# skhu101/TDNN-F_NAS

Measured on AMD Instinct MI355X. Metric: LF-MMI training frames/sec per node (SWBD 7q TDNN-F), higher is better.
Workload: dtype f32

## Files before the change

include/tdnnf_hip.h:

```cpp
#ifndef TDNNF_HIP_H_
#define TDNNF_HIP_H_

#include <stddef.h>
#include <stdint.h>

#ifdef __cplusplus
extern "C" {
#endif

#define TDNNF_OK 0
#define TDNNF_EINVAL 1
#define TDNNF_EHIP 2

#define TDNNF_MAX_OFFSETS 16

typedef struct {
  float *data;
  int rows, cols, stride;
} tdnnf_mat;

typedef void *tdnnf_stream;
typedef struct tdnnf_ng tdnnf_ng;

const char *tdnnf_last_error(void);
// ... 2 lines not shown
int tdnnf_get_option(const char *name, int *value_out);
int tdnnf_gemm_launch_forms(long long *counts, int capacity, int reset);
const char *tdnnf_gemm_launch_form_name(int index);

#define TDNNF_DARTS_USE_GUMBEL 1
#define TDNNF_DARTS_FREE_SELECT 2
#define TDNNF_DARTS_UNIFORM_SAMPLE 4
#define TDNNF_DARTS_USE_ENTROPY 8
#define TDNNF_DARTS_UPDATE_ALPHA 16

typedef struct {
  int row_stride;
  int num_offsets;
  int row_offsets[TDNNF_MAX_OFFSETS];
} tdnnf_tdnn_indexes;


int tdnnf_tdnn_darts_coef(const float *log_alpha_dev, int K, int flags, float temp_proportion,
                          const float *gumbel_u_dev, const float *sample_u_dev, int share_index,
                          float *coef_memo_dev, float *eff_coef_dev, tdnnf_stream stream);

int tdnnf_tdnn_propagate(const tdnnf_tdnn_indexes *indexes, const tdnnf_mat *in,
                         const float *linear_params_dev, int ldw, int Do, int Di,
                         const float *bias_dev, const float *eff_coef_dev, int init_mode,
                         tdnnf_mat *out, tdnnf_stream stream);

int tdnnf_tdnn_backprop_data(const tdnnf_tdnn_indexes *indexes, const tdnnf_mat *out_deriv,
                             const float *linear_params_dev, int ldw, int Do, int Di,
                             const float *eff_coef_dev, tdnnf_mat *in_deriv, tdnnf_stream stream);

size_t tdnnf_tdnn_update_workspace_bytes(int Do, int Di, int K, int num_rows);
int tdnnf_tdnn_update_simple(const tdnnf_tdnn_indexes *indexes, const tdnnf_mat *in_value,
                             const tdnnf_mat *out_deriv, int Do, int Di,
                             const float *eff_coef_dev, float lr, float *W_acc_dev, int ldw,
                             float *bias_acc_dev, void *workspace_dev, size_t workspace_bytes,
                             tdnnf_stream stream);

#define TDNNF_TAP_DOTS_SLABS 64
#define TDNNF_TAP_DOTS_DOUBLES(K) ((K) * (1 + TDNNF_TAP_DOTS_SLABS))

int tdnnf_tdnn_darts_alpha_update(const float *tap_grad_dev, int ldg, const float *linear_params_dev,
                                  int ldw, int Do, int Di, int K, const float *coef_memo_dev,
                                  int flags, int share_index, float temp_proportion, float lr,
                                  float *alpha_acc_dev, double *tap_dots_dev ,
                                  tdnnf_stream stream);

size_t tdnnf_tdnn_update_natural_gradient_workspace_bytes(int Do, int Di, int K, int num_rows, int has_bias);
int tdnnf_tdnn_update_natural_gradient(const tdnnf_tdnn_indexes *indexes, const tdnnf_mat *in_value,
                                       const tdnnf_mat *out_deriv, int Do, int Di,
                                       const float *linear_params_dev, int ldw_params,
                                       const float *coef_memo_dev, const float *eff_coef_dev, int flags,
                                       int share_index, float temp_proportion,
                                       tdnnf_ng *preconditioner_in, tdnnf_ng *preconditioner_out,
                                       float learning_rate, float *W_acc_dev, int ldw, float *bias_acc_dev,
                                       float *alpha_acc_dev, void *workspace_dev, size_t workspace_bytes,
                                       tdnnf_stream stream);


size_t tdnnf_colreduce_workspace_bytes(int rows, int cols);

int tdnnf_batchnorm_propagate(const tdnnf_mat *in, float epsilon, float target_rms, tdnnf_mat *out,
                              float *memo_dev, void *workspace_dev, size_t workspace_bytes, tdnnf_stream stream);
int tdnnf_batchnorm_backprop(const tdnnf_mat *out_value, const tdnnf_mat *out_deriv, float target_rms,
                             float *memo_dev, tdnnf_mat *in_deriv, void *workspace_dev, size_t workspace_bytes,
                             tdnnf_stream stream);
int tdnnf_batchnorm_store_stats(const float *memo_dev, int D, int num_frames, double *stats_dev,
                                tdnnf_stream stream);
int tdnnf_batchnorm_compute_derived(const double *stats_dev, int D, float epsilon, float target_rms,
                                    float *scale_dev, float *offset_dev, tdnnf_stream stream);
int tdnnf_batchnorm_test_propagate(const tdnnf_mat *in, const float *scale_dev, const float *offset_dev,
                                   tdnnf_mat *out, tdnnf_stream stream);
int tdnnf_batchnorm_test_backprop(const tdnnf_mat *out_deriv, const float *scale_dev, tdnnf_mat *in_deriv,
                                  tdnnf_stream stream);


int tdnnf_softmax_flops_propagate(const tdnnf_mat *in, const float *gumbel_u_dev, float temp_proportion,
                                  tdnnf_mat *out, tdnnf_stream stream);
int tdnnf_softmax_flops_backprop(const tdnnf_mat *out_value, tdnnf_mat *out_deriv, float scale,
                                 const float *flops_dev, int dim, float temp_proportion,
                                 tdnnf_mat *in_deriv, tdnnf_stream stream);
int tdnnf_onehot_propagate(const float *sample_u_dev, tdnnf_mat *out, tdnnf_stream stream);
int tdnnf_onehot_backprop(const tdnnf_mat *out_deriv, float lr, float *output_acc_dev, void *workspace_dev,
                          size_t workspace_bytes, tdnnf_stream stream);
int tdnnf_copyn_propagate(const tdnnf_mat *in, float scale, tdnnf_mat *out, tdnnf_stream stream);
int tdnnf_copyn_backprop(const tdnnf_mat *out_deriv, float scale, tdnnf_mat *in_deriv, tdnnf_stream stream);
int tdnnf_constant_function_propagate(const float *output_dev, tdnnf_mat *out, tdnnf_stream stream);
int tdnnf_constant_function_backprop(const tdnnf_mat *out_deriv, float lr, float *output_acc_dev,
                                     void *workspace_dev, size_t workspace_bytes, tdnnf_stream stream);
int tdnnf_flops_constraint_backprop(const float *flops_dev, float scale, int rows_in, int cols_in,
                                    tdnnf_mat *in_deriv, tdnnf_stream stream);

int tdnnf_elementwise_product_propagate(const tdnnf_mat *in, int output_dim, tdnnf_mat *out, tdnnf_stream);
int tdnnf_elementwise_product_backprop(const tdnnf_mat *in_value, const tdnnf_mat *out_deriv, int output_dim,
                                       tdnnf_mat *in_deriv, tdnnf_stream);
int tdnnf_relu_propagate(const tdnnf_mat *in, tdnnf_mat *out, tdnnf_stream);
int tdnnf_relu_backprop(const tdnnf_mat *out_value, const tdnnf_mat *out_deriv, tdnnf_mat *in_deriv, tdnnf_stream);
int tdnnf_relu_repair(const double *stats_dev, int dim, float self_repair_scale, float lower, float upper,
                      tdnnf_mat *in_deriv, tdnnf_stream);
int tdnnf_relu_store_stats(const tdnnf_mat *out_value, double *stats_dev, void *workspace_dev,
                           size_t workspace_bytes, tdnnf_stream);
int tdnnf_affine_propagate(const tdnnf_mat *in, const float *W_dev, int ldw, const float *bias_dev, int Do,
                           tdnnf_mat *out, tdnnf_stream);
int tdnnf_affine_backprop(const tdnnf_mat *out_deriv, const float *W_dev, int ldw, int Di, tdnnf_mat *in_deriv,
                          tdnnf_stream);
int tdnnf_affine_update_simple(const tdnnf_mat *in_value, const tdnnf_mat *out_deriv, float lr, float *W_acc_dev,
                               int ldw, float *bias_acc_dev, void *workspace_dev, size_t workspace_bytes,
                               tdnnf_stream);
size_t tdnnf_affine_update_natural_gradient_workspace_bytes(int Do, int Di, int num_rows, int has_bias);
int tdnnf_affine_update_natural_gradient(const tdnnf_mat *in_value, const tdnnf_mat *out_deriv,
                                         tdnnf_ng *preconditioner_in, tdnnf_ng *preconditioner_out,
                                         float learning_rate, float *W_acc_dev, int ldw, float *bias_acc_dev,
                                         void *workspace_dev, size_t workspace_bytes, tdnnf_stream);
int tdnnf_log_softmax_propagate(const tdnnf_mat *in, tdnnf_mat *out, tdnnf_stream);
int tdnnf_log_softmax_backprop(const tdnnf_mat *out_value, const tdnnf_mat *out_deriv, tdnnf_mat *in_deriv,
                               tdnnf_stream);
int tdnnf_sum_scaled(const tdnnf_mat *a, float sa, const tdnnf_mat *b, float sb, tdnnf_mat *out, tdnnf_stream);
int tdnnf_add_scaled(const tdnnf_mat *a, float s, tdnnf_mat *out, tdnnf_stream);
int tdnnf_general_dropout(const tdnnf_mat *in, const float *mask_dev, int num_seq, tdnnf_mat *out, tdnnf_stream);
int tdnnf_general_dropout_mask(const float *uniform_dev, long long n, float proportion, int continuous, float *mask_dev, tdnnf_stream);

typedef struct tdnnf_den_graph tdnnf_den_graph;
typedef struct tdnnf_supervision tdnnf_supervision;

int tdnnf_den_graph_create(int num_states, int num_arcs, int num_pdfs, const int *arc_src, const int *arc_dst,
                           const int *arc_pdf, const float *arc_prob, const float *initial_probs, int start_state,
                           tdnnf_den_graph **out);
void tdnnf_den_graph_destroy(tdnnf_den_graph *);
int tdnnf_supervision_create(int num_sequences, int frames_per_sequence, const int *seq_state_begin,
                             const int *seq_arc_begin, const int *state_time, const float *final_logprob,
                             const int *arc_src, const int *arc_dst, const int *arc_pdf, const float *arc_logprob,
                             float weight, tdnnf_supervision **out);
void tdnnf_supervision_destroy(tdnnf_supervision *);
int tdnnf_supervision_info(const tdnnf_supervision *, int *num_states, int *num_arcs, int *max_states_per_frame, int *wide);

int tdnnf_chain_set_denominator_mode(int mode);
int tdnnf_chain_den_mw_status(int *fallbacks, int *disabled, int reset);
size_t tdnnf_chain_workspace_bytes(const tdnnf_den_graph *, int num_sequences, int frames_per_sequence);
int tdnnf_chain_objf_and_deriv(const tdnnf_den_graph *, const tdnnf_supervision *, const tdnnf_mat *nnet_output,
                               const tdnnf_mat *xent_output , float leaky_hmm_coefficient,
                               float l2_regularize, float xent_regularize, double *results_dev,
                               tdnnf_mat *nnet_output_deriv, tdnnf_mat *xent_deriv, void *workspace_dev,
                               size_t workspace_bytes, tdnnf_stream);
int tdnnf_chain_numerator_part(const tdnnf_den_graph *, const tdnnf_supervision *, const tdnnf_mat *nnet_output, int part, double *results_dev,
                               tdnnf_mat *nnet_output_deriv, tdnnf_mat *xent_deriv, void *workspace_dev, size_t workspace_bytes, tdnnf_stream);

int tdnnf_ng_create(int rank, int update_period, float num_samples_history, float alpha, tdnnf_ng **out);
void tdnnf_ng_destroy(tdnnf_ng *);
int tdnnf_ng_freeze(tdnnf_ng *, int freeze);
int tdnnf_ng_precondition(tdnnf_ng *, tdnnf_mat *X, float *scale_host, tdnnf_stream);
size_t tdnnf_ng_stats_pass_workspace_bytes(int rank, int Di, int num_taps, int N);
int tdnnf_ng_stats_pass(const tdnnf_tdnn_indexes *ix, const tdnnf_mat *X, int Di, const float *eff_dev, const float *WT_dev,
                        const float *W_dev, int ldw, const float *bias_dev, tdnnf_mat *H, double *sumsq_dev, int sumsq_cap, int form,
                        void *workspace_dev, size_t workspace_bytes, tdnnf_stream);
const float *tdnnf_ng_scale_dev(const tdnnf_ng *);

size_t tdnnf_constrain_orthonormal_workspace_bytes(int rows, int cols);
int tdnnf_constrain_orthonormal(float scale, float *M_dev, int rows, int cols, int ld, void *workspace_dev,
                                size_t workspace_bytes, tdnnf_stream);
int tdnnf_axpy(const float *x_dev, float a, float *y_dev, size_t n, tdnnf_stream);
int tdnnf_dot(const float *x_dev, const float *y_dev, size_t n, double *result_host, tdnnf_stream);
size_t tdnnf_max_change_workspace_bytes(int num_comp);
int tdnnf_update_with_max_change(float *params_dev, float *delta_dev, int num_comp, const long long *comp_begin_host,
                                 const float *max_change_host, float max_param_change, float max_change_scale,
                                 float scale, int zero_delta, void *workspace_dev, size_t workspace_bytes,
                                 float *info_dev, tdnnf_stream);

int tdnnf_splice_input(const tdnnf_mat *feats, const tdnnf_mat *ivectors, int num_seq, int num_splice,
                       tdnnf_mat *out, tdnnf_stream);
int tdnnf_reorder_rows(const tdnnf_mat *in, int num_seq, int rho, int to_rho, tdnnf_mat *out, tdnnf_stream);

#define TDNNF_NET_MAX_LAYERS 32
typedef struct {
  int feat_dim, ivector_dim, num_pdfs;
  int hidden_dim, prefinal_small_dim;
  int num_layers;
  int bottleneck_dim[TDNNF_NET_MAX_LAYERS];
  int time_stride[TDNNF_NET_MAX_LAYERS];
  float bypass_scale;
  int frames_per_chunk, num_sequences;
  int frame_subsampling;
  float leaky_hmm, xent_regularize, chain_l2_regularize;
  float l2_hidden, l2_output;
  float max_change_hidden, max_change_output, max_param_change;
  float relu_self_repair_scale;
  float batchnorm_stats_scale;
  int darts_num_offsets;
  int darts_flags;
  float darts_temp_proportion;
  int use_natural_gradient;
  int bn_num_choices;
  int bn_choice_dims[8];
  int bn_mode;
  float bn_flops_scale;
  float bn_temp_proportion;
  int cv_update;
  int gemm_precision;
  int use_layer_offsets;
  int offset_left[TDNNF_NET_MAX_LAYERS];
  int offset_right[TDNNF_NET_MAX_LAYERS];
  int use_dropout;
} tdnnf_net_config;
typedef struct tdnnf_net tdnnf_net;

typedef struct tdnnf_egs_reader tdnnf_egs_reader;
typedef struct tdnnf_egs_writer tdnnf_egs_writer;
typedef struct tdnnf_eg tdnnf_eg;
int tdnnf_egs_reader_open(const char *path, tdnnf_egs_reader **out);
void tdnnf_egs_reader_close(tdnnf_egs_reader *);
int tdnnf_egs_reader_next(tdnnf_egs_reader *, tdnnf_eg **out);
void tdnnf_eg_destroy(tdnnf_eg *);
const char *tdnnf_eg_key(const tdnnf_eg *);
int tdnnf_eg_input_info(const tdnnf_eg *, const char *name, int *rows, int *cols, int *first_t);
int tdnnf_eg_input_copy(const tdnnf_eg *, const char *name, float *out);
int tdnnf_eg_supervision_info(const tdnnf_eg *, float *weight, int *num_sequences, int *frames_per_seq, int *label_dim, int *num_states,
                              int *num_arcs, int *first_t, int *t_step);
int tdnnf_egs_merge_sizes(const tdnnf_eg *const *egs, int n, int *num_states, int *num_arcs, int *frames_per_seq, int *feat_dim, int *ivector_dim);
int tdnnf_egs_merge(const tdnnf_eg *const *egs, int n, int first_t, int num_t, int frame_shift, float *feats, float *ivectors, int *seq_state_begin,
                    int *seq_arc_begin, int *state_time, float *final_logprob, int *arc_src, int *arc_dst, int *arc_pdf, float *arc_logprob,
                    float *weight_out);
int tdnnf_egs_writer_open(const char *path, tdnnf_egs_writer **out);
int tdnnf_egs_writer_close(tdnnf_egs_writer *);
int tdnnf_egs_writer_write(tdnnf_egs_writer *, const char *key, const float *feats, int rows, int feat_dim, int first_t, const float *ivector,
                           int ivector_dim, int compress, float weight, int frames, int t_step, int label_dim, int num_states, int num_arcs,
                           const float *final_logprob, const int *arc_src, const int *arc_dst, const int *arc_pdf, const float *arc_logprob);

int tdnnf_net_create(const tdnnf_net_config *cfg, tdnnf_net **out);
int tdnnf_net_create_shared(const tdnnf_net_config *cfg, const tdnnf_net *primary, tdnnf_net **out);
void tdnnf_net_destroy(tdnnf_net *);
long long tdnnf_net_num_params(const tdnnf_net *);
int tdnnf_net_num_components(const tdnnf_net *);
int tdnnf_net_component_info(const tdnnf_net *, int index, char *name_out, long long *begin, int *rows, int *cols,
                             int *has_bias, float *lr_factor, float *l2, float *max_change, float *orthonormal);
int tdnnf_net_component_num_alpha(const tdnnf_net *, int index);
int tdnnf_net_num_random_draws(const tdnnf_net *);
int tdnnf_net_set_random_draws(tdnnf_net *, const float *draws_dev);
int tdnnf_net_input_frames(const tdnnf_net *, int *num_t_in, int *first_t);
int tdnnf_net_set_buffers(tdnnf_net *, float *params_dev, float *grads_dev);
int tdnnf_net_forward_backward(tdnnf_net *, const tdnnf_mat *feats, const tdnnf_mat *ivectors, const tdnnf_den_graph *,
                               const tdnnf_supervision *, double *results_dev, long long step, tdnnf_stream);
int tdnnf_net_num_grad_buckets(const tdnnf_net *);
int tdnnf_net_grad_bucket(const tdnnf_net *, int index, long long *begin, long long *end);
int tdnnf_net_wait_grad_bucket(const tdnnf_net *, int index, tdnnf_stream stream);
int tdnnf_net_update(tdnnf_net *, float learning_rate, float l2_regularize_scale, long long step, tdnnf_stream);
int tdnnf_net_set_dropout_proportion(tdnnf_net *, float proportion);
int tdnnf_net_set_temperature_proportion(tdnnf_net *, float proportion);
size_t tdnnf_planes_bytes(int num_planes, long long rows_total, long long k_blocks);
size_t tdnnf_planes_split_workspace_bytes(void);
void tdnnf_planes_routed(long long *rows_gemms, long long *weight_gradients);
void tdnnf_planes_bound_checks(long long *checks, long long *violations);
int tdnnf_planes_split(int num_planes, const tdnnf_mat *x, int lead_rows, long long rows_total, void *planes, long long t_rows_total, void *planes_t,
                       float *scale_dev, void *workspace_dev, tdnnf_stream);
int tdnnf_planes_gemm(int num_planes, const void *a_planes, long long a_rows_total, const float *a_scale_dev, const void *b_planes, long long b_rows_total,
                      const float *b_scale_dev, int num_segments, const long long *a_row, const long long *b_row, const int *a_first_col,
                      const int *b_first_col, const int *seg_cols, const float *bias, int init_mode, int relu, tdnnf_mat *c, tdnnf_stream);
int tdnnf_planes_gemm_epilogue(int num_planes, const void *a_planes, long long a_rows_total, const float *a_scale_dev, const void *b_planes, long long b_rows_total,
                               const float *b_scale_dev, int num_segments, const long long *a_row, const long long *b_row, const int *a_first_col,
                               const int *b_first_col, const int *seg_cols, const float *bias, int init_mode, int relu, const tdnnf_mat *add, float add_scale,
                               int add_first_row, float *colstats, int *colstats_rows, tdnnf_mat *c, tdnnf_stream stream);
typedef int TDNNF_ALLREDUCE_FN(void *ctx, double *buf, long long count, tdnnf_stream stream);
int tdnnf_net_set_batchnorm_sync(tdnnf_net *, TDNNF_ALLREDUCE_FN *allreduce, void *ctx, int world_size);

int tdnnf_rccl_available(void);
int tdnnf_rccl_library_path(char *out, int out_bytes);
int tdnnf_rccl_unique_id(void *out_128_bytes);
int tdnnf_rccl_comm_create(const void *id_128_bytes, int world_size, int rank, void **comm_out);
void tdnnf_rccl_comm_destroy(void *comm);
int tdnnf_rccl_allreduce_sum(void *comm, void *buf_dev, long long count, int is_double, tdnnf_stream stream);
int tdnnf_net_set_batchnorm_sync_rccl(tdnnf_net *, void *comm, int world_size);
int tdnnf_net_allreduce_grads_rccl(tdnnf_net *, void *comm, tdnnf_stream comm_stream, tdnnf_stream stream);
int tdnnf_net_set_learning_rate_factor(tdnnf_net *, const char *name_pattern, float factor, int *num_set);
long long tdnnf_net_stats_size(const tdnnf_net *);
int tdnnf_net_get_stats(const tdnnf_net *, double *stats_host, tdnnf_stream);
int tdnnf_net_set_stats(tdnnf_net *, const double *stats_host, tdnnf_stream);
int tdnnf_net_write_model(const tdnnf_net *, const char *path, int binary, float learning_rate, tdnnf_stream);
int tdnnf_net_read_model(tdnnf_net *, const char *path, tdnnf_stream);
int tdnnf_net_config_from_model(const char *path, int frames_per_chunk, int num_sequences, tdnnf_net_config *out);
int tdnnf_net_config_text(const tdnnf_net_config *cfg, char *out, size_t capacity, size_t *needed);
int tdnnf_net_phase_times(tdnnf_net *, double *ms_out, int capacity, int *count);
int tdnnf_net_set_capture(tdnnf_net *, int on);
int tdnnf_net_get_activation(const tdnnf_net *, const char *name, tdnnf_mat *out, tdnnf_stream);
int tdnnf_net_activation_dims(const tdnnf_net *, const char *name, int *rows, int *cols);

typedef struct tdnnf_infer tdnnf_infer;
int tdnnf_infer_create(const tdnnf_net *model, int frames_per_chunk, int max_chunks, int which_output, tdnnf_infer **out);
void tdnnf_infer_destroy(tdnnf_infer *);
int tdnnf_infer_plan(const tdnnf_infer *, int num_utts, const int *frames_host, const int *ivector_rows_host, int ivector_period,
                     int *chunks_out, int capacity, int *num_chunks);
int tdnnf_chunk_plan(int frames_per_chunk, int frame_subsampling, int num_utts, const int *frames_host, const int *ivector_rows_host,
                     int ivector_period, int *chunks_out, int capacity, int *num_chunks);
int tdnnf_infer_compute(tdnnf_infer *, int num_utts, const int *frames_host, const tdnnf_mat *feats, const int *ivector_rows_host,
                        const tdnnf_mat *ivectors, int ivector_period, tdnnf_mat *out, tdnnf_stream);
int tdnnf_infer_counts(const tdnnf_infer *, int *fused_layers, int *fallback_passes);

int tdnnf_profile_enable(int on);
int tdnnf_profile_read(int kernel_class, double *launches, double *total_ms, double *total_flops);
int tdnnf_profile_read_bytes(int kernel_class, double *algorithmic_bytes);
const char *tdnnf_profile_class_name(int kernel_class);

#ifdef __cplusplus
}
#endif
#endif
```

tdnn-f_nas_amd/csrc/abi_ng.hip:

```cpp
#include <stdint.h>
#include <string.h>

#include <algorithm>

#include "gemm_f32.h"
#include "ng.h"

using namespace tdnnf;

extern "C" {

const float *tdnnf_ng_scale_dev(const tdnnf_ng *ng) { return ng && ng->dev ? ng->scale_f : nullptr; }

size_t tdnnf_ng_stats_pass_workspace_bytes(int rank, int Di, int num_taps, int N) { return ng_pform_ws_bytes(pad4(rank), Di, num_taps, N) + 64; }

int tdnnf_ng_stats_pass(const tdnnf_tdnn_indexes *ix, const tdnnf_mat *X, int Di, const float *eff, const float *WT, const float *W, int ldw,
                        const float *bias, tdnnf_mat *H, double *sumsq, int sumsq_cap, int use_valu, void *workspace, size_t workspace_bytes,
                        tdnnf_stream stream) {
  TDNNF_REQUIRE(ix && X && X->data && H && H->data && Di > 0 && ix->num_offsets >= 1 && ix->num_offsets <= kMaxSeg && ix->row_stride >= 1,
                "ng_stats_pass: bad arguments");
  const int K = ix->num_offsets, N = H->rows, Rp = H->cols;
  for (int i = 0; i < K; i++)
    TDNNF_REQUIRE(ix->row_offsets[i] >= 0 && (long long)(N - 1) * ix->row_stride + ix->row_offsets[i] < X->rows && Di <= X->cols,
                  "ng_stats_pass: tap %d reads outside X (%d x %d)", i, X->rows, X->cols);
  TDNNF_REQUIRE(!sumsq || sumsq_cap >= rows_gemm_sumsq_blocks(N), "ng_stats_pass: sumsq needs %d entries", rows_gemm_sumsq_blocks(N));
  hipStream_t s = (hipStream_t)stream;
  NgInput in;
  memset(&in, 0, sizeof(in));
  in.x = view(X); in.ix = *ix; in.Di = Di; in.ones = bias ? 1 : 0; in.N = N; in.eff = eff;
  if (use_valu == 2) {
    TDNNF_REQUIRE(W && ldw >= K * Di && sumsq && H->stride == Rp && workspace && ng_pform_ok(Rp, in, workspace_bytes),
                  "ng_stats_pass: the one-pass form takes >= 2 taps of one matrix whole 128-row tiles apart, N %% 128 == 0, N >= 32768, taps x rank <= 64, no coefficients");
    return ng_pform_pass(W, Rp, ldw, bias, in, H->data, sumsq, workspace, s);
  }
  if (use_valu) {
    const NgRowdotArgs v = ng_pass_rowdot_args(WT, Rp, bias, in, H->data, H->stride, sumsq, sumsq_cap);
    TDNNF_REQUIRE(WT && ng_rowdot_ok(v), "ng_stats_pass: the vector-ALU kernel takes rank 20 / 40 / 80 and 16-byte aligned rows");
    TDNNF_HIP(ng_rowdot(v, s));
    return TDNNF_OK;
  }
  TDNNF_REQUIRE(W && ldw >= K * Di, "ng_stats_pass: the MFMA form needs W (rank x ldw)");
  GemmPrecisionScope exact_f32(2);
  TDNNF_HIP(rows_gemm(ng_pass_gemm_args(W, ldw, Rp, bias, in, H->data, H->stride, sumsq), true, s));
  return TDNNF_OK;
}

int tdnnf_ng_create(int rank, int update_period, float num_samples_history, float alpha, tdnnf_ng **out) {
  TDNNF_REQUIRE(out && rank >= 0 && update_period >= 1 && num_samples_history > 0 && alpha >= 0, "ng_create: bad configuration");
  tdnnf_ng *ng = new tdnnf_ng();
  ng->rank = rank;
  ng->Rp = 0;
  ng->update_period = update_period;
  ng->t = 0;
  ng->D = ng->Dp = 0;
  ng->frozen = 0;
  ng->num_samples_history = num_samples_history;
  ng->alpha = alpha;
  ng->epsilon = 1.0e-10f;
  ng->delta = 5.0e-04f;
  ng->rho = 0;
  ng->dev = nullptr;
  ng->pin = nullptr;
  ng->scratch = nullptr;
  ng->scratch_floats = 0;
  ng->pending = 0;
  ng->job_done = 0;
  ng->ev_job = nullptr;
  ng->ev_wait = nullptr;
  ng->must_reorth = false;
  *out = ng;
  return TDNNF_OK;
}

int tdnnf_ng_freeze(tdnnf_ng *ng, int freeze) {
  TDNNF_REQUIRE(ng, "ng_freeze: null object");
  ng->frozen = freeze ? 1 : 0;
  return TDNNF_OK;
}

void tdnnf_ng_destroy(tdnnf_ng *ng) {
  if (!ng) return;
  if (ng->pending) ng_pool_wait(ng);
  hipFree(ng->dev);
  hipHostFree(ng->pin);
  hipFree(ng->scratch);
  if (ng->ev_job) hipEventDestroy(ng->ev_job);
  delete ng;
}

int tdnnf_ng_precondition(tdnnf_ng *ng, tdnnf_mat *X, float *scale_host, tdnnf_stream stream) {
  TDNNF_REQUIRE(ng && mat_ok(X) && X->rows > 0 && X->cols > 0, "ng_precondition: bad arguments");
  hipStream_t s = (hipStream_t)stream;
  NgCallScope scope;
  if (X->cols == 1) {
    if (scale_host) *scale_host = 1.0f;
    return TDNNF_OK;
  }
  const int N = X->rows, D = X->cols;
  const int Rp = pad4(std::max(1, std::min(ng->rank, D - 1)));
  const size_t ws_bytes = ng_stats_workspace_bytes(ng->rank, D, 1, N);
  const size_t need = (size_t)N * Rp + ws_bytes / sizeof(float) + 64;
  if (ng->scratch_floats < need) {
    if (ng->scratch) hipFree(ng->scratch);
    ng->scratch = nullptr;
    ng->scratch_floats = 0;
    TDNNF_HIP(hipMalloc((void **)&ng->scratch, sizeof(float) * need));
    ng->scratch_floats = need;
  }
  float *H = ng->scratch;
  void *ws = (void *)(((uintptr_t)(H + (size_t)N * Rp) + 63) & ~(uintptr_t)63);
  NgInput in;
  memset(&in, 0, sizeof(in));
  in.x = view(X);
  in.ix.row_stride = 1;
  in.ix.num_offsets = 1;
  in.Di = D;
  in.N = N;
  int rc = ng_stats_step(ng, in, H, ws, ws_bytes - 64, s);
  if (rc) return rc;
  if (ng->rank == 0) {
    if (scale_host) *scale_host = 1.0f;
    return TDNNF_OK;
  }
  TDNNF_HIP(rows_gemm_1seg(H, ng->Rp, ng->W, ng->Dp, false, X->data, X->stride, N, D, ng->Rp, 0, ng->neg_one, nullptr, s));
  if (scale_host) {
    TDNNF_HIP(hipMemcpyAsync(ng->h_scale, ng->scale_f, sizeof(float), hipMemcpyDeviceToHost, s));
    TDNNF_HIP(hipStreamSynchronize(s));
    *scale_host = *ng->h_scale;
  }
  return TDNNF_OK;
}

}
```

tdnn-f_nas_amd/csrc/abi_tdnn.hip:

```cpp
#include <dlfcn.h>
#include <stdlib.h>
#include <string.h>

#include <string>

#include "common.h"
#include "gemm_f32.h"
#include "planes_gemm.h"

namespace tdnnf {

static thread_local std::string g_last_error;

void set_error(const char *fmt, ...) {
  char buf[1024];
  va_list ap;
  va_start(ap, fmt);
  vsnprintf(buf, sizeof(buf), fmt, ap);
  va_end(ap);
  g_last_error = buf;
}
int hip_status(hipError_t e, const char *what) {
  set_error("HIP error %d (%s) in %s", (int)e, hipGetErrorString(e), what);
  return TDNNF_EHIP;
}

Options &options() {
  static Options o;
  return o;
}

namespace {
typedef int (*roctx_push_t)(const char *);
typedef int (*roctx_pop_t)();
roctx_push_t g_roctx_push = nullptr;
roctx_pop_t g_roctx_pop = nullptr;
bool roctx_ready() {
  static const bool ok = [] {
    const char *e = getenv("TDNNF_ROCTX");
    if (e && atoi(e) == 0) return false;
    for (const char *lib : {"librocprofiler-sdk-roctx.so", "librocprofiler-sdk-roctx.so.1", "libroctx64.so", "libroctx64.so.4"}) {
      void *h = dlopen(lib, RTLD_NOW | RTLD_GLOBAL);
      if (!h) continue;
      g_roctx_push = (roctx_push_t)dlsym(h, "roctxRangePushA");
      g_roctx_pop = (roctx_pop_t)dlsym(h, "roctxRangePop");
      if (g_roctx_push && g_roctx_pop) return true;
    }
    return false;
  }();
  return ok;
}
}
TraceRange::TraceRange(const char *name) : on(roctx_ready()) {
  if (on) g_roctx_push(name);
}
TraceRange::~TraceRange() {
  if (on) g_roctx_pop();
}

static bool tdnn_rows_ok(const tdnnf_tdnn_indexes *ix, int rows_in, int N) {
  if (!ix || ix->num_offsets < 1 || ix->num_offsets > TDNNF_MAX_OFFSETS || ix->row_stride < 1) return false;
  for (int i = 0; i < ix->num_offsets; i++) {
    const long long need = (long long)ix->row_offsets[i] + (long long)ix->row_stride * N - (ix->row_stride - 1);
    if (ix->row_offsets[i] < 0 || (N > 0 && rows_in < need)) return false;
  }
  return true;
}

}

using namespace tdnnf;

extern "C" {

const char *tdnnf_last_error(void) { return g_last_error.c_str(); }
int tdnnf_abi_version(void) { return 1; }

static int *option_slot(const char *name) {
  Options &o = options();
  if (!name) return nullptr;
  const struct { const char *n; int *p; } table[] = {{"ng_grouped", &o.ng_grouped}, {"ng_fuse", &o.ng_fuse}, {"ng_early_in", &o.ng_early_in},
                                                     {"wgrad_stream", &o.wgrad_stream}, {"gemm_ring", &o.gemm_ring}, {"planes", &o.planes}, {"den_split", &o.den_split}, {"phase_events", &o.phase_events}, {"wgrad_lag", &o.wgrad_lag}, {"ng_bk", &o.ng_bk}, {"ng_valu", &o.ng_valu}, {"ng_pform", &o.ng_pform}, {"planes_group", &o.planes_group}, {"xent_behind_den", &o.xent_behind_den}, {"ng_early_fork", &o.ng_early_fork}, {"ng_diag_skip", &o.ng_diag_skip}, {"wgrad_small", &o.wgrad_small}, {"splitk_per_cu", &o.splitk_per_cu}, {"gemm_alt_taps", &o.gemm_alt_taps}, {"reverse_passes", &o.reverse_passes}, {"splitk_partial_round", &o.splitk_partial_round}, {"wgrad_on_caller", &o.wgrad_on_caller}, {"den_mw_test_abort", &o.den_mw_test_abort}, {"planes_check_bound", &o.planes_check_bound}, {"den_gamma_pairs", &o.den_gamma_pairs}, {"num_form", &o.num_form}, {"num_frontier_cap", &o.num_frontier_cap}, {"gemm_arith_test", &o.gemm_arith_test}};
  for (auto &e : table)
    if (strcmp(e.n, name) == 0) return e.p;
  return nullptr;
}
int tdnnf_set_option(const char *name, int value) {
  int *p = option_slot(name);
  TDNNF_REQUIRE(p, "set_option: unknown option '%s' (ng_grouped, ng_fuse, ng_early_in, wgrad_stream, gemm_ring, planes, den_split)", name ? name : "(null)");
  *p = value;
  return TDNNF_OK;
}
int tdnnf_get_option(const char *name, int *value) {
  int *p = option_slot(name);
  TDNNF_REQUIRE(p && value, "get_option: unknown option '%s'", name ? name : "(null)");
  *value = *p;
  return TDNNF_OK;
}

}

namespace tdnnf {
int tdnn_propagate_impl(const tdnnf_tdnn_indexes *ix, const tdnnf_mat *in, const float *W, int ldw, int Do, int Di,
                        const float *bias, const float *eff_coef, int init_mode, int relu, tdnnf_mat *out, tdnnf_stream stream,
                        float *colstats, int *colstats_rows) {
  TDNNF_REQUIRE(mat_ok(in) && mat_ok(out) && W, "tdnn_propagate: bad matrices");
  TDNNF_REQUIRE(Do > 0 && Di > 0 && in->cols == Di && out->cols == Do, "tdnn_propagate: dims: in.cols=%d Di=%d out.cols=%d Do=%d",
                in ? in->cols : -1, Di, out ? out->cols : -1, Do);
  TDNNF_REQUIRE(tdnn_rows_ok(ix, in->rows, out->rows), "tdnn_propagate: input has too few rows for the time offsets");
  TDNNF_REQUIRE(ldw >= ix->num_offsets * Di, "tdnn_propagate: ldw < K*Di");
  TDNNF_REQUIRE(init_mode >= 0 && init_mode <= 2 && (init_mode != 1 || bias), "tdnn_propagate: init_mode 1 needs a bias");
  RowsGemmArgs a;
  memset(&a, 0, sizeof(a));
  a.A = in->data;
  a.lda = (long long)in->stride * ix->row_stride;
  a.B = W;
  a.ldb = ldw;
  a.C = out->data;
  a.ldc = out->stride;
  a.M = out->rows;
  a.N = Do;
  a.bias = bias;
  a.coef = eff_coef;
  a.init_mode = init_mode;
  a.relu = relu;
  a.colstats = colstats;
  a.colstats_rows = colstats_rows;
  a.nseg = ix->num_offsets;
  for (int i = 0; i < a.nseg; i++) {
    a.seg[i].a_off = (long long)ix->row_offsets[i] * in->stride;
    a.seg[i].b_off = (long long)i * Di;
    a.seg[i].klen = Di;
    a.seg[i].m_lo = 0;
    a.seg[i].m_hi = out->rows;
  }
  TDNNF_HIP(rows_gemm(a, true, (hipStream_t)stream));
  return TDNNF_OK;
}
}

extern "C" {

int tdnnf_tdnn_propagate(const tdnnf_tdnn_indexes *ix, const tdnnf_mat *in, const float *W, int ldw, int Do, int Di,
                         const float *bias, const float *eff_coef, int init_mode, tdnnf_mat *out, tdnnf_stream stream) {
  return tdnn_propagate_impl(ix, in, W, ldw, Do, Di, bias, eff_coef, init_mode, 0, out, stream);
}

}

namespace tdnnf {
int tdnn_backprop_data_impl(const tdnnf_tdnn_indexes *ix, const tdnnf_mat *out_deriv, const float *W, int ldw, int Do,
                            int Di, const float *eff_coef, int overwrite, const tdnnf_mat *add, float add_scale, int add_lo,
                            tdnnf_mat *in_deriv, tdnnf_stream stream) {
  TDNNF_REQUIRE(mat_ok(in_deriv) && mat_ok(out_deriv) && W, "tdnn_backprop_data: bad matrices");
  TDNNF_REQUIRE(Do > 0 && Di > 0 && in_deriv->cols == Di && out_deriv->cols == Do, "tdnn_backprop_data: bad dims");
  TDNNF_REQUIRE(tdnn_rows_ok(ix, in_deriv->rows, out_deriv->rows), "tdnn_backprop_data: in_deriv has too few rows for the time offsets");
  TDNNF_REQUIRE(ldw >= ix->num_offsets * Di, "tdnn_backprop_data: ldw < K*Di");
  const int rho = ix->row_stride, N = out_deriv->rows, K = ix->num_offsets;
  if (N == 0) return TDNNF_OK;
  for (int cls = 0; cls < rho; cls++) {
    RowsGemmArgs a;
    memset(&a, 0, sizeof(a));
    float cf_dummy = 0;
    (void)cf_dummy;
    int nseg = 0, u_max = 0;
    int seg_tap[kMaxSeg];
    for (int i = 0; i < K; i++) {
      if (ix->row_offsets[i] % rho != cls) continue;
      const int shift = (ix->row_offsets[i] - cls) / rho;
      a.seg[nseg].a_off = -(long long)shift * out_deriv->stride;
      a.seg[nseg].b_off = (long long)i * Di;
      a.seg[nseg].klen = Do;
      a.seg[nseg].m_lo = shift;
      a.seg[nseg].m_hi = shift + N;
      if (shift + N > u_max) u_max = shift + N;
      seg_tap[nseg] = i;
      nseg++;
    }
    if (nseg == 0) continue;
    bool contiguous = true;
    for (int s = 1; s < nseg; s++) contiguous = contiguous && seg_tap[s] == seg_tap[s - 1] + 1;
    a.A = out_deriv->data;
    a.lda = out_deriv->stride;
    a.B = W;
    a.ldb = ldw;
    const float *WT = (ldw == K * Di && !planes_hint_b()) ? transposed_weights(W) : nullptr;
    if (WT) {
      a.B = WT;
      a.ldb = Do;
      for (int sg = 0; sg < nseg; sg++) a.seg[sg].b_off = (long long)seg_tap[sg] * Di * Do;
    }
    a.C = in_deriv->data + (long long)cls * in_deriv->stride;
    a.ldc = (long long)in_deriv->stride * rho;
    a.M = u_max;
    a.N = Di;
    a.init_mode = 0;
    if (overwrite) {
      TDNNF_REQUIRE(rho == 1 && u_max == in_deriv->rows, "tdnn_backprop_data: overwrite needs row_stride 1 and full row coverage");
      a.init_mode = 2;
    }
    if (add) {
      TDNNF_REQUIRE(rho == 1 && add->cols == Di && add_lo >= 0 && add_lo + add->rows <= in_deriv->rows, "tdnn_backprop_data: bad addend");
      a.add = add->data;
      a.ldadd = add->stride;
      a.add_scale = add_scale;
      a.add_lo = add_lo;
      a.add_hi = add_lo + add->rows;
    }
    TDNNF_REQUIRE(!(overwrite || add) || !eff_coef || contiguous, "tdnn_backprop_data: fused overwrite/addend needs a single launch");
    if (!eff_coef || contiguous) {
      a.coef = eff_coef ? eff_coef + seg_tap[0] : nullptr;
      a.nseg = nseg;
      TDNNF_HIP(rows_gemm(a, WT != nullptr, (hipStream_t)stream));
    } else {
      for (int s = 0; s < nseg; s++) {
        RowsGemmArgs b = a;
        b.seg[0] = a.seg[s];
        b.nseg = 1;
        b.coef = eff_coef + seg_tap[s];
        b.M = a.seg[s].m_hi;
        TDNNF_HIP(rows_gemm(b, WT != nullptr, (hipStream_t)stream));
      }
    }
  }
  return TDNNF_OK;
}
}

extern "C" {

int tdnnf_tdnn_backprop_data(const tdnnf_tdnn_indexes *ix, const tdnnf_mat *out_deriv, const float *W, int ldw, int Do,
                             int Di, const float *eff_coef, tdnnf_mat *in_deriv, tdnnf_stream stream) {
  return tdnn_backprop_data_impl(ix, out_deriv, W, ldw, Do, Di, eff_coef, 0, nullptr, 0.f, 0, in_deriv, stream);
}

size_t tdnnf_tdnn_update_workspace_bytes(int Do, int Di, int K, int num_rows) {
  return wgrad_workspace_bytes(Do, Di, K, num_rows);
}

}

namespace tdnnf {
int tdnn_update_simple_impl(const tdnnf_tdnn_indexes *ix, const tdnnf_mat *in_value, const tdnnf_mat *out_deriv, int Do,
                            int Di, const float *eff_coef, float lr, float *W_acc, int ldw, float *bias_acc, void *ws,
                            size_t ws_bytes, const int *active_dev, int max_active, tdnnf_stream stream, bool overwrite) {
  TDNNF_REQUIRE(mat_ok(in_value) && mat_ok(out_deriv) && W_acc, "tdnn_update_simple: bad matrices");
  TDNNF_REQUIRE(Do > 0 && Di > 0 && in_value->cols == Di && out_deriv->cols == Do, "tdnn_update_simple: bad dims");
  TDNNF_REQUIRE(tdnn_rows_ok(ix, in_value->rows, out_deriv->rows), "tdnn_update_simple: in_value has too few rows for the time offsets");
  TDNNF_REQUIRE(ldw >= ix->num_offsets * Di, "tdnn_update_simple: ldw < K*Di");
  if (out_deriv->rows == 0) return TDNNF_OK;
  TDNNF_REQUIRE(ws && ws_bytes >= wgrad_workspace_bytes(Do, Di, ix->num_offsets, out_deriv->rows), "tdnn_update_simple: workspace too small");
  WgradArgs a;
  memset(&a, 0, sizeof(a));
  a.dY = out_deriv->data;
  a.lddy = out_deriv->stride;
  a.X = in_value->data;
  a.ldx = in_value->stride;
  a.Do = Do;
  a.Di = Di;
  a.K = ix->num_offsets;
  a.N = out_deriv->rows;
  a.row_stride = ix->row_stride;
  for (int i = 0; i < a.K; i++) a.row_offsets[i] = ix->row_offsets[i];
  a.coef = eff_coef;
  a.scale = lr;
  a.G = W_acc;
  a.ldg = ldw;
  a.accumulate = overwrite ? 0 : 1;
  a.bias_acc = bias_acc;
  a.active = active_dev;
  a.max_active = max_active;
  TDNNF_HIP(wgrad(a, ws, ws_bytes, (hipStream_t)stream));
  return TDNNF_OK;
}
}

extern "C" {

int tdnnf_tdnn_update_simple(const tdnnf_tdnn_indexes *ix, const tdnnf_mat *in_value, const tdnnf_mat *out_deriv, int Do,
                             int Di, const float *eff_coef, float lr, float *W_acc, int ldw, float *bias_acc, void *ws,
                             size_t ws_bytes, tdnnf_stream stream) {
  return tdnn_update_simple_impl(ix, in_value, out_deriv, Do, Di, eff_coef, lr, W_acc, ldw, bias_acc, ws, ws_bytes, nullptr, 0, stream);
}

int tdnnf_affine_propagate(const tdnnf_mat *in, const float *W, int ldw, const float *bias, int Do, tdnnf_mat *out,
                           tdnnf_stream stream) {
  TDNNF_REQUIRE(mat_ok(in) && mat_ok(out) && W && Do > 0 && out->cols == Do && in->rows == out->rows && ldw >= in->cols,
                "affine_propagate: bad arguments");
  tdnnf_tdnn_indexes ix;
  memset(&ix, 0, sizeof(ix));
  ix.row_stride = 1;
  ix.num_offsets = 1;
  return tdnnf_tdnn_propagate(&ix, in, W, ldw, Do, in->cols, bias, nullptr, bias ? 1 : 2, out, stream);
}

int tdnnf_affine_backprop(const tdnnf_mat *out_deriv, const float *W, int ldw, int Di, tdnnf_mat *in_deriv, tdnnf_stream stream) {
  TDNNF_REQUIRE(mat_ok(out_deriv) && mat_ok(in_deriv) && W && Di > 0 && in_deriv->cols == Di && in_deriv->rows == out_deriv->rows && ldw >= Di,
                "affine_backprop: bad arguments");
  if (out_deriv->rows == 0) return TDNNF_OK;
  RowsGemmArgs a;
  memset(&a, 0, sizeof(a));
  a.A = out_deriv->data;
  a.lda = out_deriv->stride;
  a.B = W;
  a.ldb = ldw;
  const float *WT = (ldw == Di && !planes_hint_b()) ? transposed_weights(W) : nullptr;
  if (WT) {
    a.B = WT;
    a.ldb = out_deriv->cols;
  }
  a.C = in_deriv->data;
  a.ldc = in_deriv->stride;
  a.M = out_deriv->rows;
  a.N = Di;
  a.init_mode = 2;
  a.nseg = 1;
  a.seg[0].klen = out_deriv->cols;
  a.seg[0].m_lo = 0;
  a.seg[0].m_hi = out_deriv->rows;
  TDNNF_HIP(rows_gemm(a, WT != nullptr, (hipStream_t)stream));
  return TDNNF_OK;
}

int tdnnf_affine_update_simple(const tdnnf_mat *in_value, const tdnnf_mat *out_deriv, float lr, float *W_acc, int ldw,
                               float *bias_acc, void *ws, size_t ws_bytes, tdnnf_stream stream) {
  TDNNF_REQUIRE(mat_ok(in_value) && mat_ok(out_deriv) && in_value->rows == out_deriv->rows, "affine_update_simple: bad matrices");
  tdnnf_tdnn_indexes ix;
  memset(&ix, 0, sizeof(ix));
  ix.row_stride = 1;
  ix.num_offsets = 1;
  return tdnnf_tdnn_update_simple(&ix, in_value, out_deriv, out_deriv->cols, in_value->cols, nullptr, lr, W_acc, ldw,
                                  bias_acc, ws, ws_bytes, stream);
}

}
```

tdnn-f_nas_amd/csrc/common.h:

```cpp
#pragma once
#include <hip/hip_runtime.h>
#include <stdarg.h>
#include <stdio.h>

#include "tdnnf_hip.h"

namespace tdnnf {

struct MatView {
  float *data;
  int rows, cols, stride;
};
inline MatView view(const tdnnf_mat *m) { return MatView{m->data, m->rows, m->cols, m->stride}; }

void set_error(const char *fmt, ...);
int hip_status(hipError_t e, const char *what);

inline bool mat_ok(const tdnnf_mat *m) {
  return m && m->rows >= 0 && m->cols >= 0 && m->stride >= m->cols && (m->data || m->rows * m->cols == 0);
}
inline bool same_dim(const tdnnf_mat *a, const tdnnf_mat *b) { return a->rows == b->rows && a->cols == b->cols; }

inline bool vec4_ok(const MatView &m) {
  return (reinterpret_cast<uintptr_t>(m.data) & 15) == 0 && m.stride % 4 == 0 && m.cols % 4 == 0;
}

#define TDNNF_REQUIRE(cond, ...)            \
  do {                                      \
    if (!(cond)) {                          \
      ::tdnnf::set_error(__VA_ARGS__);      \
      return TDNNF_EINVAL;                  \
    }                                       \
  } while (0)

#define TDNNF_HIP(expr)                                         \
  do {                                                          \
    hipError_t e__ = (expr);                                    \
    if (e__ != hipSuccess) return ::tdnnf::hip_status(e__, #expr); \
  } while (0)

#define TDNNF_LAUNCH_CHECK() TDNNF_HIP(hipGetLastError())

struct Options {
  int ng_grouped = 1;
  int ng_fuse = 1;
  int ng_early_in = 1;
  int wgrad_stream = -1;
  int gemm_ring = 1;
  int planes = 1;
  int den_mw_test_abort = 0;
  int planes_group = 1;
  int planes_check_bound = 0;
  int wgrad_lag = 3;
  int wgrad_on_caller = 0;
  int splitk_partial_round = 1;
  int reverse_passes = 0;
  int gemm_alt_taps = 1;
  int splitk_per_cu = 2;
  int wgrad_small = 0;
  int ng_bk = 0;
  int ng_early_fork = 1;
  int xent_behind_den = -1;
  int ng_pform = 1;
  int ng_valu = 0;
  int ng_diag_skip = 0;
  int phase_events = 0;
  int den_split = -1;
  int num_form = 0;
  int gemm_arith_test = 0;
  int num_frontier_cap = 0;
  int den_gamma_pairs = 0;
};
Options &options();

struct TraceRange {
  explicit TraceRange(const char *name);
  ~TraceRange();
  bool on;
};

__host__ __device__ inline float floor_keep_nan(float x, float f) { return x < f ? f : x; }

inline int grid_for(long long work, int block, int cap = 2048) {
  long long g = (work + block - 1) / block;
  if (g > cap) g = cap;
  if (g < 1) g = 1;
  return (int)g;
}
#ifdef __HIPCC__
template <class T>
struct as_given { typedef T type; };
template <class... P>
__attribute__((visibility("hidden"))) inline hipError_t launch_vec_or_scalar(bool vec, int rows, int cols, void (*k4)(P...), void (*k1)(P...), hipStream_t s, typename as_given<P>::type... args) {
  const long long work = (long long)rows * (vec ? cols / 4 : cols);
  void (*k)(P...) = vec ? k4 : k1;
  hipLaunchKernelGGL(k, dim3(grid_for(work, 256)), dim3(256), 0, s, args...);
  return hipGetLastError();
}
#endif

inline unsigned long long tdnnf_decision(unsigned long long step, unsigned long long k) {
  unsigned long long z = step * 0x9E3779B97F4A7C15ULL + k * 0xBF58476D1CE4E5B9ULL + 0x94D049BB133111EBULL;
  z = (z ^ (z >> 30)) * 0xBF58476D1CE4E5B9ULL;
  z = (z ^ (z >> 27)) * 0x94D049BB133111EBULL;
  return (z ^ (z >> 31)) >> 8;
}

bool log_softmax_propagate_with_aux(const tdnnf_mat *in, tdnnf_mat *out, tdnnf_mat *aux, float aux_scale, hipStream_t s);
float chain_supervision_weight(const tdnnf_supervision *sp);
size_t chain_split_region_bytes(const tdnnf_den_graph *g, int B, int T);
int chain_den(const tdnnf_den_graph *g, const tdnnf_supervision *sp, const tdnnf_mat *y, float leaky, tdnnf_mat *deriv, void *ws, hipStream_t s,
              bool beside_other_work = false, hipStream_t caller_aux = nullptr, hipEvent_t ev_recursions = nullptr, bool *ev_recorded = nullptr);
int chain_num_recursion(const tdnnf_supervision *sp, const tdnnf_den_graph *g, const tdnnf_mat *y, void *ws, hipStream_t s);
int chain_num_xent(const tdnnf_den_graph *g, const tdnnf_supervision *sp, const tdnnf_mat *y, const tdnnf_mat *xent_output, float xent_regularize,
                   tdnnf_mat *xent_deriv, void *ws, hipStream_t s, bool xent_deriv_initialised = false);
int chain_num(const tdnnf_den_graph *g, const tdnnf_supervision *sp, const tdnnf_mat *y, const tdnnf_mat *xent_output,
              float xent_regularize, tdnnf_mat *xent_deriv, void *ws, hipStream_t s, bool xent_deriv_initialised = false);
int chain_finish(const tdnnf_den_graph *g, const tdnnf_supervision *sp, const tdnnf_mat *y, float l2_regularize, double *results,
                 tdnnf_mat *deriv, tdnnf_mat *xent_deriv, void *ws, hipStream_t s);

int tdnn_propagate_impl(const tdnnf_tdnn_indexes *ix, const tdnnf_mat *in, const float *W, int ldw, int Do, int Di,
                        const float *bias, const float *eff_coef, int init_mode, int relu, tdnnf_mat *out, tdnnf_stream stream,
                        float *colstats = nullptr, int *colstats_rows = nullptr);
int tdnn_update_simple_impl(const tdnnf_tdnn_indexes *ix, const tdnnf_mat *in_value, const tdnnf_mat *out_deriv, int Do, int Di,
                            const float *eff_coef, float lr, float *W_acc, int ldw, float *bias_acc, void *ws, size_t ws_bytes,
                            const int *active_dev, int max_active, tdnnf_stream stream, bool overwrite = false);
int tdnn_backprop_data_impl(const tdnnf_tdnn_indexes *ix, const tdnnf_mat *out_deriv, const float *W, int ldw, int Do, int Di,
                            const float *eff_coef, int overwrite, const tdnnf_mat *add, float add_scale, int add_lo,
                            tdnnf_mat *in_deriv, tdnnf_stream stream);

}
```

tdnn-f_nas_amd/csrc/gemm_f32.h:

```cpp
#pragma once
#include <hip/hip_runtime.h>
#include <stddef.h>
#include <stdint.h>
#include <string.h>

#include <vector>

#include "prof.h"

namespace tdnnf {

constexpr int kMaxSeg = 16;

struct GemmSeg {
  long long a_off;
  long long b_off;
  int klen;
  int m_lo, m_hi;
};

struct RowsGemmArgs {
  const float *A;
  long long lda;
  const float *B;
  long long ldb;
  float *C;
  long long ldc;
  int M, N;
  const float *bias;
  const float *coef;
  int init_mode;
  int relu;
  int c_vec;
  const float *add;
  long long ldadd;
  float add_scale;
  int add_lo, add_hi;
  int ksplit;
  int kchunk;
  float *partial;
  double *sumsq;
  int sumsq_cap;
  float *colstats;
  int *colstats_rows;
  int colstats_stride;
  int prec;
  int serial_epilogue;
  int alt_seg_order;
  int nseg;
  GemmSeg seg[kMaxSeg];
  const float *col_scale;
  const float *col_offset;
  int post_add;
  const int *row_map;
};
inline bool rows_gemm_has_post(const RowsGemmArgs &a) { return a.col_scale || a.col_offset || a.post_add || a.row_map; }

struct SplitKScratchOverride {
  float *prev_buf;
  size_t prev_bytes;
  SplitKScratchOverride(float *buf, size_t bytes);
  ~SplitKScratchOverride();
};

struct GemmPrecisionScope {
  int prev;
  explicit GemmPrecisionScope(int prec);
  ~GemmPrecisionScope();
};
int gemm_precision_default();
struct TransposedWeightsScope {
  const float *prev_w, *prev_wt;
  long long prev_n;
  TransposedWeightsScope(const float *w_base, const float *wt_base, long long n);
  ~TransposedWeightsScope();
};
const float *transposed_weights(const float *W);

inline bool aligned16(const void *p) { return (reinterpret_cast<uintptr_t>(p) & 15) == 0; }

inline int rows_gemm_colstats_cap(int M) { return (M + 63) / 64 + 64; }
inline int rows_gemm_sumsq_blocks(int M) { return (M + 127) / 128 > 1024 ? (M + 127) / 128 : 1024; }

hipError_t rows_gemm(const RowsGemmArgs &args, bool b_kcontig, hipStream_t stream);
inline hipError_t rows_gemm_1seg(const float *A, long long lda, const float *B, long long ldb, bool b_kcontig, float *C, long long ldc, int M, int N, int K,
                                 int init_mode, const float *coef, double *sumsq, hipStream_t stream) {
  RowsGemmArgs a;
  memset(&a, 0, sizeof(a));
  a.A = A; a.lda = lda; a.B = B; a.ldb = ldb; a.C = C; a.ldc = ldc; a.M = M; a.N = N;
  a.init_mode = init_mode; a.coef = coef; a.sumsq = sumsq; a.nseg = 1;
  a.seg[0].klen = K; a.seg[0].m_lo = 0; a.seg[0].m_hi = M;
  return rows_gemm(a, b_kcontig, stream);
}

struct RowsGemmGroup;
bool rows_gemm_group_ok(const RowsGemmArgs &a);
hipError_t rows_gemm_group(const std::vector<RowsGemmArgs> &calls, RowsGemmGroup **cache, hipStream_t stream);
void rows_gemm_group_destroy(RowsGemmGroup *g);

struct WgradArgs {
  const float *dY;
  long long lddy;
  const float *X;
  long long ldx;
  int Do, Di, K, N;
  int row_stride;
  int row_offsets[kMaxSeg];
  const float *coef;
  float scale;
  float *G;
  long long ldg;
  int accumulate;
  float *bias_acc;
  const int *active;
  int max_active;
  int prec;
  int xcd_order;
};
size_t wgrad_workspace_bytes(int Do, int Di, int K, int N);
hipError_t wgrad(const WgradArgs &args, void *workspace, size_t workspace_bytes, hipStream_t stream);

}
```

tdnn-f_nas_amd/csrc/launch_forms.h:

```cpp
#pragma once
#include <atomic>

namespace tdnnf {

enum RowsForm {
  kFormPlain,
  kFormRing,
  kFormSplitK,
  kFormPartialS2,
  kFormPartialS8 = kFormPartialS2 + 6,
  kFormMainSplitTail,
  kFormMainPlainTail,
  kFormSumsqPlain,
  kFormSumsqSplitK,
  kFormPost,
  kFormGrouped,
  kRowsForms
};
constexpr int kRowsTiles = 9, kRowsAriths = 3;

template <int WM, int WN, int TM, int TN, int BK>
constexpr int rows_tile_index() {
  constexpr int BM = WM * TM * 32, BN = WN * TN * 32;
  constexpr int t = (BM == 128 && BN == 32 && BK == 32) ? 0 : (BM == 128 && BN == 32 && BK == 64) ? 1 : (BM == 128 && BN == 64 && BK == 32) ? 2
                  : (BM == 128 && BN == 96 && BK == 16) ? 3 : (BM == 128 && BN == 96 && BK == 32) ? 4 : (BM == 128 && BN == 160 && BK == 16) ? 5
                  : (BM == 64 && BN == 128 && BK == 16) ? 6 : (BM == 128 && BN == 128 && BK == 16) ? 7 : (BM == 128 && BN == 128 && BK == 32) ? 8 : -1;
  static_assert(t >= 0, "a rows GEMM tile without a counter: add it here and to kRowsTileNames (launch_forms.hip)");
  return t;
}
constexpr int rows_form_index(int tile, int arith, int form) { return (tile * kRowsAriths + arith) * kRowsForms + form; }

enum {
  kPlanesPlain = kRowsTiles * kRowsAriths * kRowsForms,
  kPlanesMainSplitTail,
  kPlanesMainPlainTail,
  kWgradFirst,
  kWgradPlanes = kWgradFirst + 5 * kRowsAriths,
  kWgradLastSlabs,
  kRowsLastSlices,
  kRowsVec4Launches,
  kRowsScalarLaunches,
  kPlanesAltChunked,
  kLaunchFormCounters
};

std::atomic<long long> *launch_form_counters();
inline void count_form(int index) { launch_form_counters()[index].fetch_add(1, std::memory_order_relaxed); }
inline void note_rows_slices(int ksplit) { launch_form_counters()[kRowsLastSlices].store(ksplit, std::memory_order_relaxed); }
inline void note_wgrad_slabs(int splits) { launch_form_counters()[kWgradLastSlabs].store(splits, std::memory_order_relaxed); }

}
```

tdnn-f_nas_amd/csrc/launch_forms.hip:

```cpp
#include "launch_forms.h"

#include <stdio.h>

#include "common.h"

namespace tdnnf {

std::atomic<long long> *launch_form_counters() {
  static std::atomic<long long> counters[kLaunchFormCounters];
  return counters;
}

namespace {
const char *const kRowsTileNames[kRowsTiles] = {"128x32k32", "128x32k64", "128x64k32", "128x96k16", "128x96k32", "128x160k16", "64x128k16", "128x128k16", "128x128k32"};
const char *const kArithNames[kRowsAriths] = {"f32", "bf16x3", "bf16x6"};
const char *const kRowsFormNames[kRowsForms] = {"plain", "ring", "splitk", "partial_s2", "partial_s3", "partial_s4", "partial_s5", "partial_s6", "partial_s7", "partial_s8",
                                                "main_split_tail", "main_plain_tail", "sumsq_plain", "sumsq_splitk", "post", "grouped"};
const char *const kWgradTileNames[5] = {"128x128", "160x128", "128x160", "32x128", "64x64"};
}

}

using namespace tdnnf;

extern "C" {

const char *tdnnf_gemm_launch_form_name(int index) {
  static thread_local char buf[64];
  if (index < 0 || index >= kLaunchFormCounters) return nullptr;
  if (index < kPlanesPlain) {
    const int form = index % kRowsForms, arith = (index / kRowsForms) % kRowsAriths, tile = index / (kRowsForms * kRowsAriths);
    snprintf(buf, sizeof(buf), "rows.%s.%s.%s", kRowsTileNames[tile], kArithNames[arith], kRowsFormNames[form]);
  } else if (index == kPlanesPlain) {
    snprintf(buf, sizeof(buf), "planes.plain");
  } else if (index == kPlanesMainSplitTail) {
    snprintf(buf, sizeof(buf), "planes.main_split_tail");
  } else if (index == kPlanesMainPlainTail) {
    snprintf(buf, sizeof(buf), "planes.main_plain_tail");
  } else if (index < kWgradPlanes) {
    const int i = index - kWgradFirst;
    snprintf(buf, sizeof(buf), "wgrad.%s.%s", kWgradTileNames[i / kRowsAriths], kArithNames[i % kRowsAriths]);
  } else if (index == kWgradPlanes) {
    snprintf(buf, sizeof(buf), "wgrad.planes");
  } else if (index == kWgradLastSlabs) {
    snprintf(buf, sizeof(buf), "wgrad.last_slabs");
  } else if (index == kRowsLastSlices) {
    snprintf(buf, sizeof(buf), "rows.last_slices");
  } else if (index == kRowsVec4Launches) {
    snprintf(buf, sizeof(buf), "rows.launches_vec4");
  } else if (index == kRowsScalarLaunches) {
    snprintf(buf, sizeof(buf), "rows.launches_scalar");
  } else {
    snprintf(buf, sizeof(buf), "planes.alt_chunked");
  }
  return buf;
}

int tdnnf_gemm_launch_forms(long long *counts, int capacity, int reset) {
  std::atomic<long long> *c = launch_form_counters();
  for (int i = 0; i < kLaunchFormCounters; i++) {
    if (counts && i < capacity) counts[i] = c[i].load(std::memory_order_relaxed);
    if (reset) c[i].store(0, std::memory_order_relaxed);
  }
  return kLaunchFormCounters;
}

}
```

tdnn-f_nas_amd/csrc/net_step.hip:

```cpp
#include <math.h>
#include <string.h>

#include <string>
#include <vector>

#include "batchnorm.h"
#include "common.h"
#include "fused.h"
#include "gemm_f32.h"
#include "net_model.h"
#include "ng.h"

namespace tdnnf {
namespace {

__global__ void add_scaled_taps_kernel(const float *G, const float *coef, float *acc, int Do, int KDi, int Di) {
  const long long total = (long long)Do * KDi;
  for (long long e = blockIdx.x * 256LL + threadIdx.x; e < total; e += gridDim.x * 256LL) acc[e] += coef[(e % KDi) / Di] * G[e];
}
__global__ void scaled_taps_to_kernel(const float *G, const float *coef, int Do, int KDi, int Di, float *T, int ldT) {
  const long long total = (long long)Do * KDi;
  for (long long e = blockIdx.x * 256LL + threadIdx.x; e < total; e += gridDim.x * 256LL) {
    const int o = (int)(e / KDi), c = (int)(e % KDi);
    T[(size_t)o * ldT + c] = (coef ? coef[c / Di] : 1.0f) * G[e];
// ... 551 lines not shown
        if (did) {
          TDNNF_HIP(hipEventRecord(n->ev_fin, n->s3));
          early_refresh = true;
        }
      }
    }
    if (early_refresh) TDNNF_HIP(hipStreamWaitEvent(s, n->ev_fin, 0));
    return TDNNF_OK;
  }
  bool is_head_comp(int comp) const {
    return comp == n->c_prefinal_l || comp == n->head[0].c_affine || comp == n->head[0].c_linear || comp == n->head[0].c_output ||
           comp == n->head[1].c_affine || comp == n->head[1].c_linear || comp == n->head[1].c_output;
  }
  bool early_eligible(int comp, int which) const {
    const auto &E = n->early[comp];
    if (E.done == n->fb_count || (which == 0 && is_head_comp(comp))) return false;
    if (E.recorded != n->fb_count - 1 || !n->ng_in[comp] || !n->ng_out[comp] || ng_dim(n->ng_in[comp]) == 0 || ng_dim(n->ng_out[comp]) == 0) return false;
    return n->comps[comp].lr_factor != 0.f && n->ngc[comp].H_in;
  }
  int launch_early_in(int which) {
    if (!(use_ng && n->early_on)) return TDNNF_OK;
    std::vector<int> who;
    for (int comp = (int)n->comps.size() - 1; comp >= 0; comp--)
      if (early_eligible(comp, which)) who.push_back(comp);
    if (who.empty()) return TDNNF_OK;
    TDNNF_HIP(hipEventRecord(n->ev_early_in, s));
    TDNNF_HIP(hipStreamWaitEvent(n->s4, n->ev_early_in, 0));
    if (early_refresh) TDNNF_HIP(hipStreamWaitEvent(n->s4, n->ev_fin, 0));
    NgInput xin;
    if (n->early_group) {
      std::vector<RowsGemmArgs> calls;
      std::vector<int> grouped;
      for (int comp : who) {
        memcpy(&xin, n->early[comp].xin, sizeof(xin));
        RowsGemmArgs a;
        CK(ng_stats_main_prepare(n->ng_in[comp], xin, n->ngc[comp].H_in, n->ngc[comp].part_in, n->s4, &a));
        if (!rows_gemm_group_ok(a)) continue;
        calls.push_back(a);
        grouped.push_back(comp);
      }
      if (calls.empty()) return TDNNF_OK;
      TDNNF_HIP(rows_gemm_group(calls, &n->early_launch, n->s4));
      for (int comp : grouped) n->early[comp].done = n->fb_count;
    } else {
      SplitKScratchOverride early_scratch(n->s4_scratch, n->s4_scratch_bytes);
      for (int comp : who) {
        memcpy(&xin, n->early[comp].xin, sizeof(xin));
        CK(ng_stats_main(n->ng_in[comp], xin, n->ngc[comp].H_in, n->ngc[comp].part_in, n->ws4, n->ws_bytes, n->s4));
        n->early[comp].done = n->fb_count;
      }
    }
    TDNNF_HIP(hipEventRecord(n->ev_early, n->s4));
    n->early_any = true;
    return TDNNF_OK;
  }

  int forward_heads_and_objective() {
    if (early_at_fork) {
      CK(finish_refreshes());
      CK(launch_early_in(0));
    }
    top = M(prev, No, Hd);
    if (po_next.base == top.data && po_next.rows == top.rows) po_top = po_next;
    else CK(split(top, 0, kP | kT, &po_top, s, fb_next));
    {
      PlanesHintScope ph(hint_of(po_top), wplanes(n->c_prefinal_l));
      CK(tdnnf_affine_propagate(&top, net_W(n, n->c_prefinal_l), Hd, nullptr, S, &pl, s));
    }
    CK(split(pl, 0, kP | kT, &po_pl, s));
    for (int h = 0; h < 2; h++) {
      CK(forward_head(h));
      if (h == 0) CK(fork_objective());
    }
    tdnnf_mat yx = M(n->head[1].y, No, P);
    const bool dense_first = log_softmax_propagate_with_aux(&yx, &lsm, &dx, -c.xent_regularize * chain_supervision_weight(sup), s);
    if (!dense_first) CK(tdnnf_log_softmax_propagate(&yx, &lsm, s));
    TDNNF_HIP(hipStreamWaitEvent(s, n->ev_num, 0));
    CK(chain_num_xent(den, sup, &y, &lsm, c.xent_regularize, &dx, n->chain_ws, s, dense_first));
    if (!dense_first) CK(tdnnf_log_softmax_backprop(&lsm, &dx, &dx, s));
    return phase_mark(n, 2, s);
  }
  int forward_head(int h) {
    auto &H = n->head[h];
    tdnnf_mat ar = M(H.aff_relu, No, Hd), lo = M(H.lin_out, No, S), b1 = M(H.bn1_out, No, Hd), b2 = M(H.bn2_out, No, S), yh = M(H.y, No, P);
    FroBound fb_b1;
    {
      PlanesHintScope ph(hint_of(po_pl), wplanes(H.c_affine));
      FroBoundScope fbs(pl_on ? n->fro_buf : nullptr, &fb_b1.blocks);
      CK(affine_relu_bn_stats(n, &ix1, &pl, net_W(n, H.c_affine), S, Hd, S, net_bias(n, H.c_affine), nullptr, &ar, H.bn1_memo, H.bn1_stats, s));
    }
    CK(bn_apply_planes(ar, H.bn1_memo, none, 0.f, b1, nullptr, fb_b1, &po_b1[h]));
    if (!po_b1[h].base) CK(split(b1, 0, kP | kT, &po_b1[h], s, fb_b1));
    {
      PlanesHintScope ph(hint_of(po_b1[h]), wplanes(H.c_linear));
      CK(tdnnf_affine_propagate(&b1, net_W(n, H.c_linear), Hd, nullptr, S, &lo, s));
    }
    CK(bn_fwd(n, H.lin_out, H.bn2_out, No, S, H.bn2_memo, H.bn2_stats, s));
    CK(split(b2, 0, kP | kT, &po_b2[h], s));
    PlanesHintScope ph(hint_of(po_b2[h]), wplanes(H.c_output));
    return tdnnf_affine_propagate(&b2, net_W(n, H.c_output), S, net_bias(n, H.c_output), P, &yh, s);
  }
  int fork_objective() {
    TraceRange trace_den("chain denominator forward-backward (second stream)");
    TDNNF_HIP(hipEventRecord(n->ev_fork, s));
    TDNNF_HIP(hipStreamWaitEvent(n->s2, n->ev_fork, 0));
    const bool den_split = n->den_split;
    TDNNF_HIP(hipStreamWaitEvent(n->s3, n->ev_fork, 0));
    const int xbd = options().xent_behind_den;
    const bool behind = den_split && (xbd > 0 || (xbd < 0 && !n->wg_on));
    if (behind && !n->ev_den_rec) TDNNF_HIP(hipEventCreateWithFlags(&n->ev_den_rec, hipEventDisableTiming));
    bool rec = false;
    CK(chain_den(den, sup, &y, c.leaky_hmm, &dy, n->chain_ws, n->s2, !den_split, n->s3, behind ? n->ev_den_rec : nullptr, &rec));
    if (rec) TDNNF_HIP(hipStreamWaitEvent(s, n->ev_den_rec, 0));
    TDNNF_HIP(hipEventRecord(n->ev_den, n->s2));
    hipStream_t sn = n->s3;
    if (n->wg_on && den_split) {
      sn = n->s4;
      TDNNF_HIP(hipStreamWaitEvent(sn, n->ev_fork, 0));
    }
    CK(chain_num_recursion(sup, den, &y, n->chain_ws, sn));
    TDNNF_HIP(hipEventRecord(n->ev_num, sn));
    return TDNNF_OK;
  }

  int capture(const std::string &name, const tdnnf_mat &m) {
    if (!n->capture_on) return TDNNF_OK;
    tdnnf_mat *dst = nullptr;
    for (auto &kv : n->named)
      if (kv.first == name) dst = &kv.second;
    if (!dst) {
      float *p = nullptr;
      TDNNF_HIP(hipMalloc((void **)&p, sizeof(float) * (size_t)std::max(1, m.rows) * ldpad(m.cols)));
      n->captured.push_back(p);
      n->named.push_back({name, M(p, m.rows, m.cols)});
      dst = &n->named.back().second;
    }
    TDNNF_REQUIRE(dst->rows == m.rows && dst->cols == m.cols, "net_forward_backward: captured %s changed shape", name.c_str());
    return tdnnf_sum_scaled(&m, 1.0f, nullptr, 0.f, dst, s);
  }
  int out_stats_fuse(int comp, MatView xv, MatView dzv, MatView dv, NgFuse &f) {
    fused_comp = -1;
    if (!c.use_natural_gradient || n->ng_out.empty() || !n->ng_out[comp] || n->comps[comp].lr_factor == 0.f) return 0;
    if (options().ng_fuse == 0) return 0;
    const bool fuse_always = options().ng_fuse == 2;
    auto &C = n->ngc[comp];
    const float *W = nullptr;
    int Rp = 0, ldw = 0;
    CK(ng_external_begin(n->ng_out[comp], dv.cols, &W, &Rp, &ldw, s));
    if (!W || !bn_relu_bwd_ng_ok(xv, dzv, dv, Rp) || !(fuse_always || bn_relu_bwd_ng_pays(dv.rows))) return 0;
    f.W = W; f.Rp = Rp; f.ldw = ldw; f.H = C.H_out; f.part = C.part_out; f.part_cap = rows_gemm_sumsq_blocks(dv.rows);
    fused_comp = comp;
    return 1;
  }
  double *oderiv_of(double *relu_stats, int relu_index) {
    std::vector<char> &nz = *n->oderiv_nonzero;
    if ((int)nz.size() < c.num_layers + 3) nz.resize(c.num_layers + 3, 0);
    const bool skip = nz[relu_index] && ::tdnnf::tdnnf_decision((unsigned long long)step, 2 * (4096 + relu_k)) % 4 == 0;
    relu_k++;
    if (!skip) nz[relu_index] = 1;
    return skip ? nullptr : relu_stats + relu_oderiv_at(Hd);
  }
  int bn_relu_backward(float *relu_out, const tdnnf_mat &d_in, const tdnnf_mat &d_out, int lead, float *memo, double *relu_stats, float *bias_acc, int comp,
                       int relu_index, const float *mask, FroBound *fb, PlanesOperand *po) {
    const bool store = coin() || step == 0;
    const bool repair = c.relu_self_repair_scale > 0.f && coin();
    tdnnf_mat x = M(relu_out, d_in.rows, Hd);
    NgFuse f;
    const int fuse = out_stats_fuse(comp, view(&x), view(&d_in), view(&d_out), f);
    if (fuse < 0) return TDNNF_EINVAL;
    FroBoundScope fbs(pl_on ? n->fro_buf : nullptr, &fb->blocks);
    BwdPlanes bp{nullptr, 0, 0, nullptr};
    PlanesOperand tmp;
    CK(bwd_planes(d_out, lead, &bp, &tmp));
    TDNNF_HIP(bn_relu_bwd(view(&x), view(&d_in), memo, 1.0f, cv, relu_stats, store, repair, c.relu_self_repair_scale, view(&d_out), bias_acc, 1.0f,
                          n->ws, n->ws_bytes, s, mask, B, fuse ? &f : nullptr, oderiv_of(relu_stats, relu_index), bp.P ? &bp : nullptr));
    if (bp.P) *po = tmp;
    if (bp.P && options().planes_check_bound) TDNNF_HIP(planes_check_bound(view(&d_out), bp.rec, n->planes_ws, s));
    return TDNNF_OK;
  }
  int close_bucket(int key) {
    if (use_ng) CK(ng_close(key));
    for (auto &gb : n->buckets) {
      if (gb.close_key != key) continue;
      hipStream_t cs = s;
      if (!use_ng && n->wg_on && n->pg_count > 0) CK(wait_last_wgrads(s, side_streams()));
      if (use_ng) {
        TDNNF_HIP(hipEventRecord(gb.handoff, s));
        TDNNF_HIP(hipStreamWaitEvent(n->s3, gb.handoff, 0));
        cs = n->s3;
      }
      const long long cnt = gb.end - gb.begin;
      if (cnt > 0)
        hipLaunchKernelGGL(commit_grads_kernel, dim3(grid_for(cnt, 256)), dim3(256), 0, cs, n->grads + gb.begin, n->gtmp + gb.begin, cnt, results);
      TDNNF_HIP(hipEventRecord(gb.ready, cs));
    }
    return TDNNF_OK;
  }
  float *bias_target(int comp) const {
    if (n->comps[comp].lr_factor == 0.f) return nullptr;
    if (!use_ng) return net_Bg(n, comp);
    return n->ngc[comp].bsum;
  }
  int handed_off(hipStream_t sw, bool on_caller) {
    if (!n->wg_on || on_caller) return TDNNF_OK;
    TDNNF_HIP(hipEventRecord(n->ev_pg[n->pg_count & 3], sw));
    const unsigned lag = lag3 ? 3u : 1u;
    if (n->pg_count >= lag) TDNNF_HIP(hipStreamWaitEvent(s, n->ev_pg[(n->pg_count - lag) & 3], 0));
    n->pg_count++;
    return TDNNF_OK;
  }
  int param_grad(int comp, const tdnnf_tdnn_indexes &ix, int K, int Di, int Do, tdnnf_mat *x, tdnnf_mat *dyv, const float *eff, bool bias_done,
                 const int *active, int max_active, bool from_tapgrad) {
    const int ldw = K * Di;
    float *bias_acc = net_Bg(n, comp);
    if (n->comps[comp].lr_factor == 0.f) return TDNNF_OK;
    hipStream_t sw = s;
    void *wsw = n->ws;
    const bool on_caller = n->wg_on && options().wgrad_on_caller != 0 && n->early_any && !den_joined;
    if (on_caller) caller_used = true;
    float *scr = nullptr;
    if (n->wg_on && !on_caller) {
      const int ns = (n->wg_two ? 2 : 1) + (n->s5 ? 1 : 0), k = (int)(n->pg_count % (unsigned)ns);
      const int which = k == 0 ? 0 : (k == 1 && n->wg_two) ? 1 : 2;
      sw = which == 0 ? n->s4 : which == 1 ? n->s2 : n->s5;
      wsw = which == 0 ? n->ws4 : which == 1 ? n->ws2 : n->ws5;
      scr = which == 0 ? n->s4_scratch : which == 1 ? n->s2_scratch : n->s5_scratch;
      TDNNF_HIP(hipEventRecord(n->ev_pg_in, s));
      TDNNF_HIP(hipStreamWaitEvent(sw, n->ev_pg_in, 0));
    }
    SplitKScratchOverride sw_scratch(scr, scr ? n->s4_scratch_bytes : 0);
    if (!use_ng) {
      CK(tdnn_update_simple_impl(&ix, x, dyv, Do, Di, eff, 1.0f, net_Wg(n, comp), ldw, bias_done ? nullptr : bias_acc, wsw, n->ws_bytes, active, max_active, sw));
      return handed_off(sw, on_caller);
    }
    const int N = dyv->rows, ones = bias_acc ? 1 : 0, Dx = ldw + ones, ldT = (Dx + 3) & ~3;
    auto &C = n->ngc[comp];
    TDNNF_REQUIRE(C.T && C.N == N, "net_forward_backward: component %s has no natural-gradient buffers for %d rows", n->comps[comp].name.c_str(), N);
    float *T = C.T;
    const bool grouped = n->ng_grouped && ng_dim(n->ng_in[comp]) != 0 && ng_dim(n->ng_out[comp]) != 0;
    const bool overwrite = !from_tapgrad && !active && eff == nullptr && (ones || ldT == ldw);
    if (!overwrite) TDNNF_HIP(hipMemsetAsync(T, 0, sizeof(float) * (size_t)Do * ldT, sw));
    if (from_tapgrad)
      hipLaunchKernelGGL(scaled_taps_to_kernel, dim3(grid_for((long long)Do * ldw, 256)), dim3(256), 0, sw, n->tapgrad, eff, Do, ldw, Di, T, ldT);
    else
      CK(tdnn_update_simple_impl(&ix, x, dyv, Do, Di, eff, 1.0f, T, ldT, nullptr, wsw, n->ws_bytes, active, max_active, sw, overwrite));
    if (ones) {
      if (!bias_done) TDNNF_HIP(colsum_add(view(dyv), 1.0f, C.bsum, wsw, sw));
      if (!grouped) ng_set_column(C.bsum, Do, T, ldT, ldw, sw);
    }
    NgInput xin;
    memset(&xin, 0, sizeof(xin));
    xin.x = view(x); xin.ix = ix; xin.Di = Di; xin.ones = ones; xin.N = N; xin.eff = eff; xin.active = active; xin.max_active = max_active;
    static_assert(sizeof(NgInput) <= sizeof(tdnnf_net::EarlyIn::xin), "EarlyIn::xin too small");
    if (n->early_on && n->early[comp].done == n->fb_count) {
      TDNNF_REQUIRE(memcmp(n->early[comp].xin, &xin, sizeof(xin)) == 0, "net_forward_backward: the input of component %s moved between minibatches",
                    n->comps[comp].name.c_str());
      if (n->early_group) {
        TDNNF_HIP(hipStreamWaitEvent(sw, n->ev_early, 0));
        CK(ng_stats_main_finish(n->ng_in[comp], xin, C.H_in, wsw, n->ws_bytes, sw));
      }
    } else {
      CK(ng_stats_main(n->ng_in[comp], xin, C.H_in, C.part_in, wsw, n->ws_bytes, sw));
    }
    if (n->early_on) {
      memcpy(n->early[comp].xin, &xin, sizeof(xin));
      n->early[comp].recorded = n->fb_count;
    }
    NgInput yin;
    memset(&yin, 0, sizeof(yin));
    yin.x = view(dyv); yin.ix.row_stride = 1; yin.ix.num_offsets = 1; yin.Di = Do; yin.N = N;
    if (fused_comp == comp) {
      fused_comp = -1;
      CK(ng_stats_main_finish(n->ng_out[comp], yin, C.H_out, wsw, n->ws_bytes, sw));
    } else {
      CK(ng_stats_main(n->ng_out[comp], yin, C.H_out, C.part_out, wsw, n->ws_bytes, sw));
    }
    if (grouped) {
      n->ng_cur.push_back(comp);
      CK(handed_off(sw, on_caller));
      if (from_tapgrad && n->wg_on) TDNNF_HIP(hipStreamWaitEvent(s, n->ev_pg[(n->pg_count - 1) & 3], 0));
      return TDNNF_OK;
    }
    TDNNF_HIP(hipEventRecord(n->ev_ngc, sw));
    TDNNF_HIP(hipStreamWaitEvent(n->s3, n->ev_ngc, 0));
    {
      SplitKScratchOverride side_scratch(n->s3_scratch, n->s3_scratch_bytes);
      CK(ng_chain_one(n->ng_in[comp], n->ng_out[comp], C.H_in, C.part_in, C.H_out, C.part_out, T, Do, Dx, ldT, ldw, net_Wg(n, comp), bias_acc,
                      n->ng_side_ws, n->ngset_ws_bytes, n->ngTmp, n->s3));
    }
    CK(handed_off(sw, on_caller));
    if (from_tapgrad && n->wg_on) TDNNF_HIP(hipStreamWaitEvent(s, n->ev_pg[(n->pg_count - 1) & 3], 0));
    return TDNNF_OK;
  }
  int ng_close(int key) {
    if (n->ng_cur.empty()) return TDNNF_OK;
    bool closes = false;
    for (auto &gb : n->buckets) closes = closes || gb.close_key == key;
    if (!closes) return TDNNF_OK;
    tdnnf_net::NgBucket *nb = nullptr;
    for (auto &b : n->ng_buckets)
      if (b.key == key) nb = &b;
    if (!nb) {
      std::vector<NgGroupComp> gc;
      for (int comp : n->ng_cur) {
        const CompDesc &cd = n->comps[comp];
        auto &C = n->ngc[comp];
        NgGroupComp g;
        g.in = n->ng_in[comp]; g.out = n->ng_out[comp];
        g.T = C.T; g.Do = cd.rows; g.ldw = cd.cols; g.Dx = cd.cols + (cd.has_bias ? 1 : 0); g.ldT = (g.Dx + 3) & ~3;
        g.bsum = cd.has_bias ? C.bsum : nullptr;
        g.H_in = C.H_in; g.H_out = C.H_out; g.part_in = C.part_in; g.part_out = C.part_out; g.N = C.N;
        g.W_acc = net_Wg(n, comp); g.bias_acc = net_Bg(n, comp);
        gc.push_back(g);
      }
      NgGroup *grp = nullptr;
      CK(ng_group_create(gc, &grp));
      n->ng_buckets.push_back(tdnnf_net::NgBucket{key, n->ng_cur, grp});
      nb = &n->ng_buckets.back();
    }
    TDNNF_REQUIRE(nb->comps == n->ng_cur, "net_forward_backward: the components of gradient bucket %d changed between minibatches", key);
    if (n->wg_on && n->pg_count > 0) {
      CK(wait_last_wgrads(n->s3, side_streams()));
      if (caller_used) {
        TDNNF_HIP(hipEventRecord(n->ev_ngc, s));
        TDNNF_HIP(hipStreamWaitEvent(n->s3, n->ev_ngc, 0));
        caller_used = false;
      }
    } else {
      TDNNF_HIP(hipEventRecord(n->ev_ngc, s));
      TDNNF_HIP(hipStreamWaitEvent(n->s3, n->ev_ngc, 0));
    }
    if (n->early_any) TDNNF_HIP(hipStreamWaitEvent(n->s3, n->ev_early, 0));
    CK(ng_group_run(nb->group, n->s3));
    n->ng_cur.clear();
    return TDNNF_OK;
  }
  int tdnn_wgrad(Tdnn &td, tdnnf_mat *x, tdnnf_mat *dyv, const float *eff, bool bias_done) {
    const int ldw = td.K * td.Di;
    bool tap_ready = false;
    if (td.darts && !(c.darts_flags & TDNNF_DARTS_UNIFORM_SAMPLE)) {
      tap_ready = true;
      TDNNF_HIP(hipMemsetAsync(n->tapgrad, 0, sizeof(float) * (size_t)td.Do * ldw, s));
      CK(tdnnf_tdnn_update_simple(&td.ix, x, dyv, td.Do, td.Di, nullptr, 1.0f, n->tapgrad, ldw, nullptr, n->ws, n->ws_bytes, s));
      CK(tdnnf_tdnn_darts_alpha_update(n->tapgrad, ldw, net_W(n, td.comp), ldw, td.Do, td.Di, td.K, td.memo, c.darts_flags, td.share,
                                       c.darts_temp_proportion, 1.0f, net_Ag(n, td.comp), n->tapdots, s));
      if (!use_ng) {
        hipLaunchKernelGGL(add_scaled_taps_kernel, dim3(grid_for((long long)td.Do * ldw, 256)), dim3(256), 0, s, n->tapgrad, eff,
                           net_Wg(n, td.comp), td.Do, ldw, td.Di);
        if (!bias_done) TDNNF_HIP(colsum_add(view(dyv), 1.0f, net_Bg(n, td.comp), n->ws, s));
        return TDNNF_OK;
      }
    }
    const bool compact = td.darts && (c.darts_flags & TDNNF_DARTS_UNIFORM_SAMPLE) && td.K > 2;
    return param_grad(td.comp, td.ix, td.K, td.Di, td.Do, x, dyv, eff, bias_done, compact ? td.active : nullptr, compact ? 2 : 0, tap_ready);
  }

  int backward_heads() {
    if (!early_at_fork) CK(finish_refreshes());
    if (n->wg_on) CK(launch_early_in(2));
    for (int h = 1; h >= 0; h--) CK(backward_head(h));
    CK(capture("prefinal-l.deriv", d_pl));
    CK(split(d_pl, 0, kP | kT, &po_dpl, s));
    {
      PlanesHintScope ph(hint_of(po_dpl), hint_of(po_top));
      CK(param_grad(n->c_prefinal_l, ix1, 1, Hd, S, &top, &d_pl, nullptr, false, nullptr, 0, false));
    }
    CK(close_bucket(-2));
    return phase_mark(n, 3, s);
  }
  int backward_head(int h) {
    auto &H = n->head[h];
    TraceRange trace_head(h == 0 ? "backward prefinal-chain / output" : "backward prefinal-xent / output-xent");
    if (h == 0) {
      TDNNF_HIP(hipStreamWaitEvent(s, n->ev_den, 0));
      den_joined = true;
      n->wg_two = n->wg_on && n->ws2 != nullptr;
      CK(chain_finish(den, sup, &y, c.chain_l2_regularize, results, &dy, nullptr, n->chain_ws, s));
    }
    tdnnf_mat dout = h == 0 ? dy : dx;
    tdnnf_mat b2 = M(H.bn2_out, No, S), b1 = M(H.bn1_out, No, Hd);
    float *d_b1_buf = !lag3 ? n->dA : dC_of(h == 1 ? Ltop : Ltop - 1), *d_b2_buf = !lag3 ? n->d_small2 : n->dS[h == 1 ? 0 : 1];
    tdnnf_mat d_b2 = M(d_b2_buf, No, S), d_b1 = M(d_b1_buf, No, Hd);
    const std::string hname = h == 0 ? "prefinal-chain" : "prefinal-xent";
    if (h == 1) CK(capture("output-xent.deriv", dout));
    PlanesOperand po_d;
    CK(split(dout, 0, kP | kT, &po_d, s));
    {
      PlanesHintScope ph(hint_of(po_d), hint_of(po_b2[h]));
      CK(param_grad(H.c_output, ix1, 1, S, P, &b2, &dout, nullptr, false, nullptr, 0, false));
    }
    {
      PlanesHintScope ph(hint_of(po_d), wplanes(H.c_output));
      CK(tdnnf_affine_backprop(&dout, net_W(n, H.c_output), S, S, &d_b2, s));
    }
    CK(capture(hname + ".batchnorm2.deriv", d_b2));
    if (cv) CK(tdnnf_batchnorm_test_backprop(&d_b2, H.bn2_memo + 2 * S, &d_b2, s));
    else CK(tdnnf_batchnorm_backprop(&b2, &d_b2, 1.0f, H.bn2_memo, &d_b2, n->ws, n->ws_bytes, s));
    CK(capture(hname + ".linear.deriv", d_b2));
    CK(split(d_b2, 0, kP | kT, &po_d, s));
    {
      PlanesHintScope ph(hint_of(po_d), hint_of(po_b1[h]));
      CK(param_grad(H.c_linear, ix1, 1, Hd, S, &b1, &d_b2, nullptr, false, nullptr, 0, false));
    }
    {
      PlanesHintScope ph(hint_of(po_d), wplanes(H.c_linear));
      CK(tdnnf_affine_backprop(&d_b2, net_W(n, H.c_linear), Hd, Hd, &d_b1, s));
    }
    CK(capture(hname + ".batchnorm1.deriv", d_b1));
    FroBound fb_d;
    CK(bn_relu_backward(H.aff_relu, d_b1, d_b1, 0, H.bn1_memo, H.relu_stats, bias_target(H.c_affine), H.c_affine, c.num_layers + 1 + h, nullptr, &fb_d,
                        &po_d));
    CK(capture(hname + ".affine.deriv", d_b1));
    if (!po_d.base || po_d.base != d_b1.data) CK(split(d_b1, 0, kP | kT, &po_d, s, fb_d));
    {
      PlanesHintScope ph(hint_of(po_d), hint_of(po_pl));
      CK(param_grad(H.c_affine, ix1, 1, S, Hd, &pl, &d_b1, nullptr, true, nullptr, 0, false));
    }
    PlanesHintScope ph_bp(hint_of(po_d), wplanes(H.c_affine));
    if (h == 1) {
      CK(tdnnf_affine_backprop(&d_b1, net_W(n, H.c_affine), S, S, &d_pl, s));
      if (!n->wg_on) CK(launch_early_in(early_at_fork ? 1 : 2));
    } else {
      tdnnf_mat tmp = M(!lag3 ? n->d_small2 : n->dS[0], No, S);
      CK(tdnnf_affine_backprop(&d_b1, net_W(n, H.c_affine), S, S, &tmp, s));
      CK(tdnnf_add_scaled(&tmp, 1.0f, &d_pl, s));
    }
    return TDNNF_OK;
  }
  int backward_trunk() {
    {
      tdnnf_mat d_top = M(d_cur, No, Hd);
      PlanesHintScope ph(hint_of(po_dpl), wplanes(n->c_prefinal_l));
      CK(tdnnf_affine_backprop(&d_pl, net_W(n, n->c_prefinal_l), Hd, Hd, &d_top, s));
    }
    for (int l = c.num_layers - 1; l >= 0; l--) CK(backward_layer(l));
    {
      FroBound fb_d;
      PlanesOperand po_d;
      tdnnf_mat d_aff = M(d_cur, N0, Hd);
      CK(bn_relu_backward(n->t1_relu, d_aff, d_aff, 0, n->t1_bn_memo, n->t1_relu_stats, bias_target(n->tdnn1.comp), n->tdnn1.comp, 0, mask_of(0), &fb_d, &po_d));
      if (!po_d.base) CK(split(d_aff, 0, kT, &po_d, s, fb_d));
      PlanesHintScope ph(hint_of(po_d), hint_of(po_lda));
      CK(param_grad(n->tdnn1.comp, ix1, 1, lda_dim, Hd, &lda_out, &d_aff, nullptr, true, nullptr, 0, false));
    }
    CK(close_bucket(-1));
    return phase_mark(n, 4, s);
  }
  int backward_layer(int l) {
    TdnnfLayer &L = n->layers[l];
    float *in_act = l > 0 ? n->layers[l - 1].noop_out : n->t1_bn;
    const int no = L.aff.rows_out, nl = L.lin.rows_out, ni = N_of(L.gin, B);
    tdnnf_mat d_out = M(d_cur, no, Hd), d_aff = M(dC_of(l), no, Hd);
    const std::string lname = "tdnnf" + std::to_string(l + 2);
    TraceRange trace_layer(("backward " + lname).c_str());
    CK(capture(lname + ".noop.deriv", d_out));
    FroBound fb_daff;
    PlanesOperand po_daff, po_dlin;
    CK(bn_relu_backward(L.relu_out, d_out, d_aff, max_off(L.aff), L.bn_memo, L.relu_stats, bias_target(L.aff.comp), L.aff.comp, 1 + l, mask_of(l + 1), &fb_daff,
                        &po_daff));
    CK(capture(lname + ".affine.deriv", d_aff));
    tdnnf_mat lin = M(L.lin_out, nl, L.bn);
    tdnnf_mat aff_in = L.perm ? M(L.lin_perm, nl, L.bn) : (L.c_arch >= 0 ? M(L.lin_masked, nl, L.bn) : lin);
    const float *lin_eff = L.lin.darts ? L.lin.memo + TDNNF_MAX_OFFSETS : nullptr;
    const float *aff_eff = L.aff.darts ? L.aff.memo + TDNNF_MAX_OFFSETS : nullptr;
    ProfFlopsScale taps_active(L.lin.darts && (c.darts_flags & TDNNF_DARTS_UNIFORM_SAMPLE) && L.lin.K > 2 ? 2.0 / L.lin.K : 1.0);
    if (pl_on && !po_daff.base) CK(split(d_aff, max_off(L.aff), kP | kT, &po_daff, s, fb_daff));
    {
      PlanesHintScope ph(hint_of(po_daff), hint_of(po_lin[l]));
      CK(tdnn_wgrad(L.aff, &aff_in, &d_aff, aff_eff, true));
    }
    PlanesHintScope ph_aff_bp(hint_of(po_daff), wplanes(L.aff.comp));
    tdnnf_mat d_lin = M(lag3 ? (L.perm ? n->d_small2 : dS_of(l)) : n->d_small, nl, L.bn);
    if (L.perm) {
      TDNNF_HIP(hipMemsetAsync(d_lin.data, 0, sizeof(float) * (size_t)nl * d_lin.stride, s));
      CK(tdnnf_tdnn_backprop_data(&L.aff.ix, &d_aff, net_W(n, L.aff.comp), L.aff.K * L.bn, Hd, L.bn, aff_eff, &d_lin, s));
      tdnnf_mat un = M(lag3 ? dS_of(l) : n->d_small2, nl, L.bn);
      CK(tdnnf_reorder_rows(&d_lin, B, L.aff.ix.row_stride, 0, &un, s));
      d_lin = un;
    } else {
      CK(tdnn_backprop_data_impl(&L.aff.ix, &d_aff, net_W(n, L.aff.comp), L.aff.K * L.bn, Hd, L.bn, aff_eff, 1, nullptr, 0.f, 0, &d_lin, s));
    }
    if (L.c_arch >= 0) {
      const int chunks = (nl + 511) / 512;
      hipLaunchKernelGGL(colsum_prod_partial_kernel, dim3((L.bn + 255) / 256, chunks), dim3(256), 0, s, view(&lin), view(&d_lin), 512, (float *)n->ws);
      hipLaunchKernelGGL(bn_choice_backward_kernel, dim3(1), dim3(256), 0, s, bn_choice(c), (const float *)n->ws, chunks, L.arch_p, net_Wg(n, L.c_arch));
      hipLaunchKernelGGL(col_scale_kernel, dim3(grid_for((long long)nl * L.bn, 256)), dim3(256), 0, s, view(&d_lin), L.arch_mask, view(&d_lin));
    }
    CK(capture(lname + ".linear.deriv", d_lin));
    tdnnf_mat in = M(in_act, ni, Hd);
    if (pl_on) CK(split(d_lin, max_off(L.lin), kP | kT, &po_dlin, s));
    {
      PlanesHintScope ph(hint_of(po_dlin), hint_of(po_in[l]));
      CK(tdnn_wgrad(L.lin, &in, &d_lin, lin_eff, false));
    }
    CK(close_bucket(l));
    PlanesHintScope ph_lin_bp(hint_of(po_dlin), wplanes(L.lin.comp));
    tdnnf_mat d_in = M(d_next, ni, Hd);
    tdnnf_mat d_byp = sub_grid_view(d_next, L.gin, L.gout, B, Hd);
    if (d_byp.rows == d_out.rows) {
      const int row0 = (int)((d_byp.data - d_in.data) / d_in.stride);
      CK(tdnn_backprop_data_impl(&L.lin.ix, &d_lin, net_W(n, L.lin.comp), L.lin.K * Hd, L.bn, Hd, lin_eff, 1, &d_out, c.bypass_scale, row0,
                                 &d_in, s));
    } else {
      CK(tdnn_backprop_data_impl(&L.lin.ix, &d_lin, net_W(n, L.lin.comp), L.lin.K * Hd, L.bn, Hd, lin_eff, 1, nullptr, 0.f, 0, &d_in, s));
      tdnnf_mat d_o = tdnnf_mat{d_cur, L.gout.n, d_byp.cols, B * ldpad(Hd)};
      CK(tdnnf_add_scaled(&d_o, c.bypass_scale, &d_byp, s));
    }
    std::swap(d_cur, d_next);
    return TDNNF_OK;
  }
  int join() {
    if (n->wg_on) CK(wait_last_wgrads(s, 3));
    n->wg_two = false;
    if (use_ng) {
      TDNNF_HIP(hipEventRecord(n->ev_s3, n->s3));
      TDNNF_HIP(hipStreamWaitEvent(s, n->ev_s3, 0));
    }
    CK(phase_mark(n, 5, s));
    TDNNF_LAUNCH_CHECK();
    return TDNNF_OK;
  }

  int run() {
    CK(begin());
    BnSyncScope bn_sync_scope(n->bn_sync.fn && !c.cv_update ? &n->bn_sync : nullptr);
    GemmPrecisionScope gemm_arith(c.gemm_precision == 2 ? 3 : c.gemm_precision == 3 ? 4 : c.gemm_precision);
    CK(weight_planes());
    TransposedWeightsScope gemm_wt(n->params, n->paramsT, n->paramsT ? n->num_params : 0);
    CK(transpose_weights());
    TraceRange trace_step("tdnnf_net_forward_backward");
    CK(forward_trunk());
    CK(forward_heads_and_objective());
    CK(backward_heads());
    CK(backward_trunk());
    return join();
  }
};

}

extern "C" {

int tdnnf_net_forward_backward(tdnnf_net *n, const tdnnf_mat *feats, const tdnnf_mat *ivectors, const tdnnf_den_graph *den,
                               const tdnnf_supervision *sup, double *results, long long step, tdnnf_stream stream) {
// ... 27 lines not shown
```

tdnn-f_nas_amd/csrc/rows_gemm.hip:

```cpp
#include <algorithm>
#include <cstring>
#include <vector>

#include "colreduce.h"
#include "common.h"
#include "device.h"
#include "gemm_f32.h"
#include "gemm_ring.h"
#include "launch_forms.h"
#include "planes_gemm.h"
#include "rows_gemm_kernels.h"

namespace tdnnf {
namespace {

float *g_scratch_override = nullptr;
size_t g_scratch_override_bytes = 0;
int g_gemm_prec = 0;
const float *g_tw_w = nullptr, *g_tw_wt = nullptr;
long long g_tw_n = 0;

struct KRange {
  long long ktot;
  bool k4;
};
KRange k_range(const RowsGemmArgs &a) {
  KRange k{0, true};
  for (int i = 0; i < a.nseg; i++) {
    k.ktot += a.seg[i].klen;
    k.k4 = k.k4 && (a.seg[i].klen % 4 == 0 || a.nseg == 1);
  }
  return k;
}
bool is_two_tap_shift(const RowsGemmArgs &a) {
  return a.nseg == 2 && a.seg[0].klen == a.seg[1].klen && a.lda > 0 && a.seg[0].a_off != a.seg[1].a_off && (a.seg[1].a_off - a.seg[0].a_off) % a.lda == 0;
}
int usable_rows(const GemmSeg &sg, int M) {
  const int lo = sg.m_lo > 0 ? sg.m_lo : 0, hi = sg.m_hi < M ? sg.m_hi : M;
  return hi > lo ? hi - lo : 0;
}
bool operands_vec4(const RowsGemmArgs &a) {
  bool vec = aligned16(a.A) && aligned16(a.B) && a.lda % 4 == 0 && a.ldb % 4 == 0;
  for (int i = 0; i < a.nseg; i++) vec = vec && a.seg[i].a_off % 4 == 0 && a.seg[i].b_off % 4 == 0;
  return vec;
}

template <int BM, int BN, int BK>
constexpr size_t rows_lds_bytes(bool b_kc) {
  return sizeof(float) * 2 * (BM * (BK + 4) + (b_kc ? BN * (BK + 4) : BK * (BN + 4)));
}
template <int BM, int BN, int BK, int NP>
constexpr size_t rows_x3_lds_bytes() {
  return sizeof(__bf16) * 2 * NP * (size_t)(BM + BN) * (BK + 8);
}

thread_local int t_launched_arith = 0;
inline void note_launch(int arith, bool vec) {
  t_launched_arith = arith;
  count_form(vec ? kRowsVec4Launches : kRowsScalarLaunches);
}
template <int WM, int WN, int TM, int TN, int BK>
void count_rows_form(int form) {
  count_form(rows_form_index(rows_tile_index<WM, WN, TM, TN, BK>(), t_launched_arith, form));
}

template <int WM, int WN, int TM, int TN, int BK, int NP, int TAG>
void launch_rows_x3_tagged(dim3 grid, const RowsGemmArgs &a, int ntm, int ntn, hipStream_t s) {
  constexpr int D = 1;
  constexpr size_t lds = rows_x3_lds_bytes<WM * TM * 32, WN * TN * 32, BK, NP>();
  static const bool opted = opt_in_lds(rows_gemm_x3_kernel<WM, WN, TM, TN, BK, NP, D, TAG>, lds);
  (void)opted;
  note_launch(NP - 1, true);
  hipLaunchKernelGGL((rows_gemm_x3_kernel<WM, WN, TM, TN, BK, NP, D, TAG>), grid, dim3(256), lds, s, a, ntm, ntn);
}

template <int WM, int WN, int TM, int TN, int BK, int TAG>
void launch_rows_kernel_tagged(dim3 grid, const RowsGemmArgs &a, int ntm, int ntn, bool b_kc, bool vec, hipStream_t s) {
  constexpr int BM = WM * TM * 32, BN = WN * TN * 32;
  constexpr size_t lds_kc = rows_lds_bytes<BM, BN, BK>(true), lds_nc = rows_lds_bytes<BM, BN, BK>(false);
  static const bool opted = opt_in_lds(rows_gemm_kernel<WM, WN, TM, TN, BK, true, 4, TAG>, lds_kc) && opt_in_lds(rows_gemm_kernel<WM, WN, TM, TN, BK, true, 1, TAG>, lds_kc) &&
                            opt_in_lds(rows_gemm_kernel<WM, WN, TM, TN, BK, false, 4, TAG>, lds_nc) && opt_in_lds(rows_gemm_kernel<WM, WN, TM, TN, BK, false, 1, TAG>, lds_nc);
  (void)opted;
  const dim3 block(256);
  note_launch(0, vec);
  if (b_kc) {
    if (vec) hipLaunchKernelGGL((rows_gemm_kernel<WM, WN, TM, TN, BK, true, 4, TAG>), grid, block, lds_kc, s, a, ntm, ntn);
    else hipLaunchKernelGGL((rows_gemm_kernel<WM, WN, TM, TN, BK, true, 1, TAG>), grid, block, lds_kc, s, a, ntm, ntn);
  } else {
    if (vec) hipLaunchKernelGGL((rows_gemm_kernel<WM, WN, TM, TN, BK, false, 4, TAG>), grid, block, lds_nc, s, a, ntm, ntn);
    else hipLaunchKernelGGL((rows_gemm_kernel<WM, WN, TM, TN, BK, false, 1, TAG>), grid, block, lds_nc, s, a, ntm, ntn);
  }
}
template <int WM, int WN, int TM, int TN, int BK>
void launch_rows_kernel(dim3 grid, const RowsGemmArgs &a, int ntm, int ntn, bool b_kc, bool vec, hipStream_t s) {
  const bool ng = prof_class_override() == 3;
  if (a.prec == 1 && b_kc && vec) {
    if (ng) launch_rows_x3_tagged<WM, WN, TM, TN, BK, 2, 1>(grid, a, ntm, ntn, s);
    else launch_rows_x3_tagged<WM, WN, TM, TN, BK, 2, 0>(grid, a, ntm, ntn, s);
    return;
  }
  if (a.prec == 3 && b_kc && vec) {
    if constexpr (BK == 16) {
      if (ng) launch_rows_x3_tagged<WM, WN, TM, TN, BK, 3, 1>(grid, a, ntm, ntn, s);
      else launch_rows_x3_tagged<WM, WN, TM, TN, BK, 3, 0>(grid, a, ntm, ntn, s);
      return;
    }
  }
  if (ng) launch_rows_kernel_tagged<WM, WN, TM, TN, BK, 1>(grid, a, ntm, ntn, b_kc, vec, s);
  else launch_rows_kernel_tagged<WM, WN, TM, TN, BK, 0>(grid, a, ntm, ntn, b_kc, vec, s);
}

template <int WM, int WN, int TM, int TN>
constexpr bool kRingTile = (WM == 2 && WN == 2 && TM == 2 && TN == 2) || (WM == 4 && WN == 1 && TM == 1 && TN == 5);
inline bool ring_applies(const RowsGemmArgs &a, bool b_kc, bool vec, int tile_cols) {
  return prof_class_override() != 3 && (tile_cols == 128 || rows_gemm_ring_mode() >= 2) && rows_gemm_ring_ok(a, b_kc, vec);
}

template <int WM, int WN, int TM, int TN, int BK>
hipError_t launch_rows(const RowsGemmArgs &a, bool b_kc, bool vec, hipStream_t s, int form = kFormPlain) {
  constexpr int BM = WM * TM * 32, BN = WN * TN * 32;
  const int ntm = (a.M + BM - 1) / BM, ntn = (a.N + BN - 1) / BN;
  if constexpr (kRingTile<WM, WN, TM, TN>) {
    if (ring_applies(a, b_kc, vec, BN)) {
      note_launch(0, true);
      count_rows_form<WM, WN, TM, TN, BK>(kFormRing);
      return rows_gemm_ring(a, b_kc, BN, s);
    }
  }
  launch_rows_kernel<WM, WN, TM, TN, BK>(dim3(ntm * ntn), a, ntm, ntn, b_kc, vec, s);
  count_rows_form<WM, WN, TM, TN, BK>(form);
  return hipGetLastError();
}

template <int WM, int WN, int TM, int TN, int BK>
void launch_split_k(RowsGemmArgs at, int ntm, int ntn, int S, long long ktot, float *scratch, bool b_kc, bool vec, hipStream_t s) {
  const long long kt = (ktot + BK - 1) / BK;
  at.kchunk = (int)(((kt + S - 1) / S) * BK);
  at.ksplit = (int)((ktot + at.kchunk - 1) / at.kchunk);
  at.partial = scratch;
  note_rows_slices(at.ksplit);
  launch_rows_kernel<WM, WN, TM, TN, BK>(dim3(ntm * ntn * at.ksplit), at, ntm, ntn, b_kc, vec, s);
  const long long total = (long long)at.M * at.N;
  hipLaunchKernelGGL(splitk_reduce_kernel, dim3((unsigned)std::min<long long>((total + 255) / 256, 2048)), dim3(256), 0, s, at);
}

template <int WM, int WN, int TM, int TN, int BK>
int rows_slots_per_cu(int prec) {
  int per_cu = (WM * TM == 4 && WN * TN == 4 && BK == 16 && prec == 0) ? 3 : 2;
  if (prec == 3 && WN * TN == 5) per_cu = 1;
  if (WM * TM == 2 && prec == 0) per_cu = 4;
  return per_cu;
}
template <int WM, int WN, int TM, int TN, int BK>
int rows_slots(int prec) {
  return rows_slots_per_cu<WM, WN, TM, TN, BK>(prec) * device_cus();
}

constexpr size_t kScratchDefaultBytes = 64u << 20;
float *splitk_scratch(size_t *bytes) {
  if (g_scratch_override) {
    *bytes = g_scratch_override_bytes;
    return g_scratch_override;
  }
  static float *buf = nullptr;
  static bool tried = false;
  if (!tried) {
    tried = true;
    if (hipMalloc((void **)&buf, kScratchDefaultBytes) != hipSuccess) buf = nullptr;
    (void)hipGetLastError();
  }
  *bytes = kScratchDefaultBytes;
  return buf;
}

template <int WM, int WN, int TM, int TN, int BK>
hipError_t launch_rows_balanced(const RowsGemmArgs &a, bool b_kc, bool vec, int cls, double flops, hipStream_t s) {
  constexpr int BM = WM * TM * 32, BN = WN * TN * 32;
  const int ntm = (a.M + BM - 1) / BM, ntn = (a.N + BN - 1) / BN;
  int slots = rows_slots<WM, WN, TM, TN, BK>((b_kc && vec) ? a.prec : 0);
  if constexpr (kRingTile<WM, WN, TM, TN>) {
    if (ring_applies(a, b_kc, vec, BN)) slots = rows_gemm_ring_slots(BN);
  }
  const int tiles = ntm * ntn;
  const int q = tiles / slots, r = tiles % slots;
  const bool stats = a.colstats != nullptr;
  const auto [ktot, k4] = k_range(a);
  const int main_mt = (q * slots) / ntn;
  float *scratch = nullptr;
  size_t scratch_bytes = 0;
  int S_partial = 0;
  if (!stats && q == 0 && tiles * 4 > slots && k4 && options().splitk_partial_round) {
    const int cus = device_cus();
    const long long kt = (ktot + BK - 1) / BK;
    double best = (double)((tiles + cus - 1) / cus);
    for (int S = 2; S <= 8; S++) {
      if (kt / S < 24) break;
      const double cost = (double)(((long long)tiles * S + cus - 1) / cus) / S + 0.02 * S;
      if (cost < best - 1e-9) {
        best = cost;
        S_partial = S;
      }
    }
  }
  if (!stats && (tiles * 4 <= slots || S_partial >= 2) && k4 && ktot >= 16 * BK && (scratch = splitk_scratch(&scratch_bytes))) {
    const long long kt = (ktot + BK - 1) / BK;
    int S = S_partial >= 2 ? S_partial : slots / tiles;
    if (S_partial < 2 && options().splitk_per_cu == 1) S = std::max(2, device_cus() / tiles);
    if (S > kt / 4) S = (int)(kt / 4);
    const size_t need = sizeof(float) * (size_t)S * a.M * ((a.N + 3) & ~3);
    if (S >= 2 && need <= scratch_bytes) {
      ProfScope ps(cls, flops, s);
      launch_split_k<WM, WN, TM, TN, BK>(a, ntm, ntn, S, ktot, scratch, b_kc, vec, s);
      count_rows_form<WM, WN, TM, TN, BK>(S_partial >= 2 ? kFormPartialS2 + S_partial - 2 : kFormSplitK);
      return hipGetLastError();
    }
  }
  if (q >= 1 && r > 0 && 2 * r <= slots && main_mt > 0 && main_mt < ntm && k4 && ktot >= 8 * BK && (scratch = splitk_scratch(&scratch_bytes))) {
    const int m_main = main_mt * BM;
    RowsGemmArgs am = a;
    am.M = m_main;
    const int tail_rows = a.M - m_main;
    const long long kt_tail = (ktot + BK - 1) / BK;
    const int tail_tiles0 = ((tail_rows + BM - 1) / BM) * ntn;
    int S_tail = slots / tail_tiles0;
    if (S_tail > kt_tail / 2) S_tail = (int)(kt_tail / 2);
    const bool tail_split = S_tail >= 2 && sizeof(float) * (size_t)S_tail * tail_rows * ((a.N + 3) & ~3) <= scratch_bytes;
    ColReducePlan tail_plan = colreduce_plan(tail_rows, a.N);
    if (stats) {
      am.colstats_stride = main_mt + (tail_split ? tail_plan.chunks : (tail_rows + BM - 1) / BM);
      *a.colstats_rows = am.colstats_stride;
    }
    {
      ProfScope ps(cls, flops * m_main / a.M, s);
      hipError_t e = launch_rows<WM, WN, TM, TN, BK>(am, b_kc, vec, s);
      if (e != hipSuccess) return e;
    }
    RowsGemmArgs at = a;
    at.M = a.M - m_main;
    at.A = a.A + (long long)m_main * a.lda;
    at.C = a.C + (long long)m_main * a.ldc;
    for (int i = 0; i < at.nseg; i++) {
      at.seg[i].m_lo -= m_main;
      at.seg[i].m_hi -= m_main;
    }
    at.add_lo -= m_main;
    at.add_hi -= m_main;
    if (stats) {
      at.colstats = a.colstats + (long long)main_mt * a.N;
      at.colstats_stride = am.colstats_stride;
    }
    if (tail_split) {
      {
        ProfScope ps(cls, flops * at.M / a.M, s);
        launch_split_k<WM, WN, TM, TN, BK>(at, (at.M + BM - 1) / BM, ntn, S_tail, ktot, scratch, b_kc, vec, s);
        count_rows_form<WM, WN, TM, TN, BK>(kFormMainSplitTail);
      }
      if (stats) {
        MatView ct{at.C, at.M, at.N, (int)at.ldc};
        hipError_t e = colreduce_partial_into(1, ct, ct, tail_plan.chunks, tail_plan.rows_per_chunk, am.colstats_stride, at.colstats, s);
        if (e != hipSuccess) return e;
      }
      return hipGetLastError();
    }
    ProfScope ps(cls, flops * at.M / a.M, s);
    const hipError_t e = launch_rows<WM, WN, TM, TN, BK>(at, b_kc, vec, s);
    count_rows_form<WM, WN, TM, TN, BK>(kFormMainPlainTail);
    return e;
  }
  ProfScope ps(cls, flops, s);
  if (stats) {
    RowsGemmArgs as = a;
    as.colstats_stride = ntm;
    *a.colstats_rows = ntm;
    return launch_rows<WM, WN, TM, TN, BK>(as, b_kc, vec, s);
  }
  return launch_rows<WM, WN, TM, TN, BK>(a, b_kc, vec, s);
}

template <int WM, int WN, int TM, int TN, int BK>
hipError_t launch_rows_sumsq(const RowsGemmArgs &a, bool b_kc, bool vec, hipStream_t s) {
  constexpr int BM = WM * TM * 32;
  const int tiles = (a.M + BM - 1) / BM, slots = rows_slots<WM, WN, TM, TN, BK>(0);
  const auto [ktot, k4] = k_range(a);
  float *scratch = nullptr;
  size_t scratch_bytes = 0;
  if (tiles * 4 <= slots && k4 && ktot >= 16 * BK && (scratch = splitk_scratch(&scratch_bytes))) {
    const long long kt = (ktot + BK - 1) / BK;
    int S = slots / tiles;
    if (S > kt / 4) S = (int)(kt / 4);
    if (S > 16) S = 16;
    const size_t need = sizeof(float) * (size_t)S * a.M * ((a.N + 3) & ~3);
    if (S >= 2 && need <= scratch_bytes && tiles * S <= a.sumsq_cap) {
      launch_split_k<WM, WN, TM, TN, BK>(a, tiles, 1, S, ktot, scratch, b_kc, vec, s);
      count_rows_form<WM, WN, TM, TN, BK>(kFormSumsqSplitK);
      return hipGetLastError();
    }
  }
  return launch_rows<WM, WN, TM, TN, BK>(a, b_kc, vec, s, kFormSumsqPlain);
}

template <int WM, int WN, int TM, int TN, int BK>
hipError_t launch_rows_post(const RowsGemmArgs &a, bool vec, int cls, double flops, hipStream_t s) {
  constexpr int BM = WM * TM * 32, BN = WN * TN * 32;
  const int ntm = (a.M + BM - 1) / BM, ntn = (a.N + BN - 1) / BN;
  constexpr size_t lds = rows_lds_bytes<BM, BN, BK>(true);
  static const bool opted = opt_in_lds(rows_gemm_post_kernel<WM, WN, TM, TN, BK, 4>, lds) && opt_in_lds(rows_gemm_post_kernel<WM, WN, TM, TN, BK, 1>, lds);
  (void)opted;
  ProfScope ps(cls, flops, s);
  note_launch(0, vec);
  count_rows_form<WM, WN, TM, TN, BK>(kFormPost);
  if (vec) hipLaunchKernelGGL((rows_gemm_post_kernel<WM, WN, TM, TN, BK, 4>), dim3(ntm * ntn), dim3(256), lds, s, a, ntm, ntn);
  else hipLaunchKernelGGL((rows_gemm_post_kernel<WM, WN, TM, TN, BK, 1>), dim3(ntm * ntn), dim3(256), lds, s, a, ntm, ntn);
  return hipGetLastError();
}

inline long long floordiv(long long a, long long b) { return a >= 0 ? a / b : -((-a + b - 1) / b); }

bool planes_try_rows(const RowsGemmArgs &a, bool b_kc, int np, double flops, hipStream_t s, hipError_t *err) {
  const PlanesOperand *ha = planes_hint_a(), *hb = planes_hint_b();
  if (!ha || !hb || ha->np != np || hb->np != np || !ha->P || a.sumsq || a.ksplit > 1 || a.nseg > 16) return false;
  if (ha->coef || (a.coef == nullptr) != (hb->coef == nullptr)) return false;
  long long coef_t0 = 0;
  if (a.coef) {
    coef_t0 = a.coef - hb->coef;
    if (coef_t0 < 0 || coef_t0 >= 16 || hb->coef_period <= 0) return false;
  }
  if (a.lda != ha->ld || a.A < ha->base || (a.A - ha->base) % ha->ld != 0) return false;
  const long long arow0 = (a.A - ha->base) / ha->ld;
  const int BM = planes_gemm_tile_rows(a.N), BN = planes_gemm_tile_cols(a.N);
  const long long m_pad = (long long)((a.M + BM - 1) / BM) * BM, n_pad = (long long)((a.N + BN - 1) / BN) * BN;
  PlanesGemmArgs g;
  memset(&g, 0, sizeof(g));
  g.np = np;
  g.A = ha->P; g.RA = ha->R; g.scale_a = ha->scale; g.scale_b = hb->scale;
  if (a.ldb != hb->ld || a.B < hb->base) return false;
  const long long boff0 = a.B - hb->base;
  if (b_kc) {
    if (!hb->P) return false;
    g.B = hb->P; g.RB = hb->R;
  } else {
    if (!hb->PT) return false;
    g.B = hb->PT; g.RB = hb->Rt;
  }
  for (int i = 0; i < a.nseg; i++) {
    const GemmSeg &sg = a.seg[i];
    const long long shift = floordiv(sg.a_off, ha->ld), c0 = sg.a_off - shift * ha->ld;
    if (c0 % 16 != 0 || c0 + sg.klen > ha->cols || sg.klen <= 0) return false;
    const long long first = arow0 + shift;
    const int lo = sg.m_lo > 0 ? sg.m_lo : 0, hi = sg.m_hi < a.M ? sg.m_hi : a.M;
    if (hi <= lo) return false;
    if (first + lo < 0 || first + hi > ha->rows) return false;
    if (lo > 0 && first + lo != 0) return false;
    if (hi < a.M && first + hi != ha->rows) return false;
    if (ha->lead + first < 0 || ha->lead + first + m_pad > ha->R) return false;
    g.seg[i].a_row = ha->lead + first;
    g.seg[i].a_kb0 = (int)(c0 / 16);
    g.seg[i].nkb = (sg.klen + 15) / 16;
    if (sg.klen % 16 != 0 && c0 + sg.klen != ha->cols) return false;
    const long long bo = boff0 + sg.b_off;
    if (b_kc) {
      const long long brow = bo / hb->ld, bc0 = bo % hb->ld;
      if (bo < 0 || bc0 % 16 != 0 || bc0 + sg.klen > hb->cols || brow + a.N > hb->rows || brow + n_pad > hb->R) return false;
      if (sg.klen % 16 != 0 && bc0 + sg.klen != hb->cols) return false;
      if (a.coef && (bc0 % hb->coef_period != 0 || bc0 / hb->coef_period != coef_t0 + i || sg.klen > hb->coef_period)) return false;
      g.seg[i].b_row = brow;
      g.seg[i].b_kb0 = (int)(bc0 / 16);
    } else {
      const long long krow = bo / hb->ld, ncol = bo % hb->ld;
      if (bo < 0 || krow % 16 != 0 || krow + sg.klen > hb->rows || ncol + a.N > hb->cols || ncol + n_pad > hb->Rt) return false;
      if (sg.klen % 16 != 0 && krow + sg.klen != hb->rows) return false;
      if (a.coef && (ncol % hb->coef_period != 0 || ncol / hb->coef_period != coef_t0 + i || a.N > hb->coef_period)) return false;
      g.seg[i].b_row = ncol;
      g.seg[i].b_kb0 = (int)(krow / 16);
    }
  }
  g.nseg = a.nseg;
  g.alt_seg_order = a.alt_seg_order && a.nseg == 2 && g.seg[0].nkb == g.seg[1].nkb && g.seg[0].a_kb0 == g.seg[1].a_kb0 && g.seg[0].a_row != g.seg[1].a_row;
  if (g.alt_seg_order && options().gemm_alt_taps == 2 && g.seg[0].nkb >= 24 && !a.coef) {
    const PlanesSeg s0 = g.seg[0], s1 = g.seg[1];
    const int nchunk = std::min(16, s0.nkb / 6), per = (s0.nkb + nchunk - 1) / nchunk;
    int n = 0;
    for (int c = 0; c < nchunk; c++) {
      const int k0 = c * per, kn = std::min(per, s0.nkb - k0);
      if (kn <= 0) break;
      for (const PlanesSeg *sp : {&s0, &s1}) {
        PlanesSeg q = *sp;
        q.a_kb0 += k0;
        q.b_kb0 += k0;
        q.nkb = kn;
        g.seg[n++] = q;
      }
    }
    g.nseg = n;
    g.alt_seg_order = 0;
    count_form(kPlanesAltChunked);
  }
  g.skip_coef = a.coef;
  g.C = a.C; g.ldc = a.ldc; g.M = a.M; g.N = a.N;
  g.bias = a.bias; g.init_mode = a.init_mode; g.relu = a.relu;
  g.add = a.add; g.ldadd = a.ldadd; g.add_scale = a.add_scale; g.add_lo = a.add_lo; g.add_hi = a.add_hi;
  ProfScope ps(BN == 160 ? 1 : 0, flops, s);
  g_planes_routed_rows++;
  {
    const int cus = device_cus();
    g.M = a.M;
    g.N = a.N;
    const int BMl = planes_gemm_launch_tile_rows(g);
    const int ntm = (a.M + BMl - 1) / BMl, ntn = (a.N + BN - 1) / BN, tiles = ntm * ntn, slots = cus * (BMl == 128 ? 2 : 1), q = tiles / slots, r = tiles % slots;
    int nkb = 0;
    for (int i = 0; i < g.nseg; i++) nkb += g.seg[i].nkb;
    const int main_mt = (q * slots) / ntn;
    const bool stats = a.colstats && a.colstats_rows && g.init_mode != 0;
    if (stats) {
      g.colstats = a.colstats;
      g.colstats_stride = ntm;
      *a.colstats_rows = ntm;
    }
    size_t scratch_bytes = 0;
    float *scratch = nullptr;
    if (q >= 1 && r > 0 && 2 * r <= slots && main_mt > 0 && main_mt < ntm && nkb >= 48 && BMl == BM && (scratch = splitk_scratch(&scratch_bytes))) {
      const int m_main = main_mt * BM, tail_rows = a.M - m_main, tail_tiles = ((tail_rows + BM - 1) / BM) * ntn;
      int S = std::min(cus / tail_tiles, nkb / 4);
      const long long ldp = (a.N + 3) & ~3;
      if (S >= 2 && sizeof(float) * (size_t)S * tail_rows * ldp <= scratch_bytes) {
        PlanesGemmArgs gm = g;
        gm.M = m_main;
        const ColReducePlan tail_plan = colreduce_plan(tail_rows, a.N);
        if (stats) {
          gm.colstats_stride = main_mt + tail_plan.chunks;
          *a.colstats_rows = gm.colstats_stride;
        }
        *err = planes_gemm(gm, s);
        if (*err != hipSuccess) return true;
        PlanesGemmArgs gt = g;
        gt.colstats = nullptr;
        gt.M = tail_rows;
        gt.C = g.C + (long long)m_main * g.ldc;
        for (int i = 0; i < gt.nseg; i++) gt.seg[i].a_row += m_main;
        if (gt.add) {
          gt.add_lo = g.add_lo - m_main;
          gt.add_hi = g.add_hi - m_main;
          gt.add = g.add;
        }
        const int kbps = (nkb + S - 1) / S;
        gt.ksplit = (nkb + kbps - 1) / kbps;
        gt.kb_per_split = kbps;
        gt.partial = scratch;
        gt.partial_stride = (long long)tail_rows * ldp;
        gt.ldp_m = ldp;
        gt.ldp_n = 1;
        count_form(gt.ksplit >= 2 ? kPlanesMainSplitTail : kPlanesMainPlainTail);
        if (gt.ksplit >= 2) {
          *err = planes_gemm(gt, s);
          if (*err == hipSuccess) *err = planes_splitk_finish(gt, s);
        } else {
          gt.ksplit = 0;
          gt.partial = nullptr;
          *err = planes_gemm(gt, s);
        }
        if (stats && *err == hipSuccess) {
          MatView ct{gt.C, tail_rows, a.N, (int)gt.ldc};
          *err = colreduce_partial_into(1, ct, ct, tail_plan.chunks, tail_plan.rows_per_chunk, gm.colstats_stride, a.colstats + (long long)main_mt * a.N, s);
        }
        return true;
      }
    }
  }
  count_form(kPlanesPlain);
  *err = planes_gemm(g, s);
  return true;
}

}

SplitKScratchOverride::SplitKScratchOverride(float *buf, size_t bytes) : prev_buf(g_scratch_override), prev_bytes(g_scratch_override_bytes) {
  g_scratch_override = buf;
  g_scratch_override_bytes = bytes;
}
SplitKScratchOverride::~SplitKScratchOverride() {
  g_scratch_override = prev_buf;
  g_scratch_override_bytes = prev_bytes;
}
GemmPrecisionScope::GemmPrecisionScope(int prec) : prev(g_gemm_prec) { g_gemm_prec = prec; }
GemmPrecisionScope::~GemmPrecisionScope() { g_gemm_prec = prev; }
int gemm_precision_default() { return g_gemm_prec; }
TransposedWeightsScope::TransposedWeightsScope(const float *w_base, const float *wt_base, long long n) : prev_w(g_tw_w), prev_wt(g_tw_wt), prev_n(g_tw_n) {
  g_tw_w = w_base;
  g_tw_wt = wt_base;
  g_tw_n = n;
}
TransposedWeightsScope::~TransposedWeightsScope() {
  g_tw_w = prev_w;
  g_tw_wt = prev_wt;
  g_tw_n = prev_n;
}
const float *transposed_weights(const float *W) {
  if (!g_tw_w || !g_tw_wt || W < g_tw_w || W >= g_tw_w + g_tw_n) return nullptr;
  return g_tw_wt + (W - g_tw_w);
}

hipError_t rows_gemm(const RowsGemmArgs &a_in, bool b_kc, hipStream_t s) {
  if (a_in.M <= 0 || a_in.N <= 0 || a_in.nseg <= 0) return hipSuccess;
  RowsGemmArgs a = a_in;
  a.c_vec = aligned16(a.C) && a.ldc % 4 == 0 && (a.init_mode != 1 || aligned16(a.bias)) && (!a.add || (aligned16(a.add) && a.ldadd % 4 == 0));
  const bool vec = operands_vec4(a);
  const int waste128 = ((a.N + 127) / 128) * 128 - a.N, waste160 = ((a.N + 159) / 160) * 160 - a.N;
  const long long ktot = k_range(a).ktot;
  double flops = 0;
  for (int i = 0; i < a.nseg; i++) flops += 2.0 * usable_rows(a.seg[i], a.M) * a.N * a.seg[i].klen;
  if (prof_on()) {
    double a_elems = 0, b_elems = 0;
    bool taps = true;
    for (int i = 1; i < a.nseg; i++)
      taps = taps && a.seg[i].klen == a.seg[0].klen && a.lda > 0 && (a.seg[i].a_off - a.seg[0].a_off) % a.lda == 0;
    if (taps) {
      long long lo = a.seg[0].a_off, hi = a.seg[0].a_off;
      for (int i = 1; i < a.nseg; i++) {
        lo = std::min(lo, a.seg[i].a_off);
        hi = std::max(hi, a.seg[i].a_off);
      }
      a_elems = ((double)a.M + (double)(hi - lo) / (double)a.lda) * a.seg[0].klen;
    }
    for (int i = 0; i < a.nseg; i++) {
      if (!taps) a_elems += (double)usable_rows(a.seg[i], a.M) * a.seg[i].klen;
      b_elems += (double)a.seg[i].klen * a.N;
    }
    double c_elems = (double)a.M * a.N * (a.init_mode == 0 ? 2.0 : 1.0);
    if (a.add) c_elems += (double)(std::min(a.add_hi, a.M) - std::max(a.add_lo, 0)) * a.N;
    prof_next_gemm(flops, 4.0 * (a_elems + b_elems + c_elems));
  }
  a.serial_epilogue = 0;
  a.alt_seg_order = options().gemm_alt_taps && is_two_tap_shift(a);
  if (rows_gemm_has_post(a)) {
    if (!b_kc || a.init_mode == 0 || a.sumsq || a.ksplit > 1 || (a.init_mode == 1 && !a.bias)) return hipErrorInvalidValue;
    a.prec = 0;
    a.colstats = nullptr;
    if (a.colstats_rows) *a.colstats_rows = 0;
    a.c_vec = a.c_vec && (!a.col_scale || aligned16(a.col_scale)) && (!a.col_offset || aligned16(a.col_offset));
    if (waste160 < waste128) return launch_rows_post<4, 1, 1, 5, 16>(a, vec, 1, flops, s);
    if ((long long)((a.M + 127) / 128) * ((a.N + 127) / 128) < 768) return launch_rows_post<2, 2, 1, 2, 16>(a, vec, 0, flops, s);
    if (ktot <= 512) return launch_rows_post<2, 2, 2, 2, 16>(a, vec, 0, flops, s);
    return launch_rows_post<2, 2, 2, 2, 32>(a, vec, 0, flops, s);
  }
  if (a.prec == 0) {
    a.prec = g_gemm_prec;
    if (a.prec == 0 && (options().gemm_arith_test == 1 || options().gemm_arith_test == 3)) a.prec = options().gemm_arith_test;
  }
  if (a.prec == 2) a.prec = 0;
  if (a.prec == 4 || (a.prec == 3 && options().planes)) {
    hipError_t pe = hipSuccess;
    if (planes_try_rows(a, b_kc, a.prec == 4 ? 2 : 3, flops, s, &pe)) return pe;
    if (a.prec == 4) a.prec = 0;
  }
  if (!(b_kc && vec)) a.prec = 0;
  if (a.colstats_rows) *a.colstats_rows = 0;
  if (!a.colstats_rows || a.prec != 0 || a.sumsq || a.N <= 32 || waste160 < waste128 || a.ksplit > 1) a.colstats = nullptr;
  if (a.sumsq) {
    if (a.N > 128) return hipErrorInvalidValue;
    a.sumsq_cap = rows_gemm_sumsq_blocks(a.M);
    ProfScope ps(0, flops, s);
    if (a.N <= 32) return (options().ng_bk & 1) ? launch_rows_sumsq<4, 1, 1, 1, 64>(a, b_kc, vec, s) : launch_rows_sumsq<4, 1, 1, 1, 32>(a, b_kc, vec, s);
    if (a.N <= 64 && a.N > 32 && (options().ng_bk & 8) == 0) return launch_rows_sumsq<4, 1, 1, 2, 32>(a, b_kc, vec, s);
    if (a.N <= 96 && a.N > 64 && ((options().ng_bk & 4) || ktot >= 2048)) return launch_rows_sumsq<2, 2, 2, 2, 32>(a, b_kc, vec, s);
    if (a.N <= 96) return (options().ng_bk & 2) ? launch_rows_sumsq<4, 1, 1, 3, 32>(a, b_kc, vec, s) : launch_rows_sumsq<4, 1, 1, 3, 16>(a, b_kc, vec, s);
    return launch_rows_sumsq<2, 2, 2, 2, 32>(a, b_kc, vec, s);
  }
  if (a.N <= 32 && a.M >= 1024) {
    ProfScope ps(0, flops, s);
    return (options().ng_bk & 1) ? launch_rows<4, 1, 1, 1, 64>(a, b_kc, vec, s) : launch_rows<4, 1, 1, 1, 32>(a, b_kc, vec, s);
  }
  if (waste160 < waste128) return launch_rows_balanced<4, 1, 1, 5, 16>(a, b_kc, vec, 1, flops, s);
  {
    const long long tiles128 = (long long)((a.M + 127) / 128) * ((a.N + 127) / 128);
    const bool small = tiles128 < 768;
    if (small && a.prec == 0 && !a.sumsq) return launch_rows_balanced<2, 2, 1, 2, 16>(a, b_kc, vec, 0, flops, s);
    if ((ktot <= 512 && a.prec == 0) || a.prec == 3) return launch_rows_balanced<2, 2, 2, 2, 16>(a, b_kc, vec, 0, flops, s);
  }
  return launch_rows_balanced<2, 2, 2, 2, 32>(a, b_kc, vec, 0, flops, s);
}

struct RowsGemmGroup {
  std::vector<RowsGemmArgs> args;
  std::vector<int> first;
  RowsGemmArgs *d_args = nullptr;
  int *d_first = nullptr;
  int capacity = 0;
};
void rows_gemm_group_destroy(RowsGemmGroup *g) {
  if (!g) return;
  if (g->d_args) hipFree(g->d_args);
  if (g->d_first) hipFree(g->d_first);
  delete g;
}
bool rows_gemm_group_ok(const RowsGemmArgs &a) {
  if (a.M <= 0 || a.N <= 0 || a.N > 32 || !a.sumsq || a.nseg <= 0 || a.ksplit > 1 || a.colstats || a.add) return false;
  return operands_vec4(a);
}
hipError_t rows_gemm_group(const std::vector<RowsGemmArgs> &calls, RowsGemmGroup **cache, hipStream_t s) {
  if (calls.empty()) return hipSuccess;
  if (!*cache) *cache = new RowsGemmGroup();
  RowsGemmGroup &g = **cache;
  std::vector<RowsGemmArgs> prep(calls.size());
  std::vector<int> first(calls.size() + 1, 0);
  double flops = 0, bytes = 0;
  for (size_t i = 0; i < calls.size(); i++) {
    RowsGemmArgs a = calls[i];
    if (!rows_gemm_group_ok(a)) return hipErrorInvalidValue;
    a.c_vec = aligned16(a.C) && a.ldc % 4 == 0 && (a.init_mode != 1 || aligned16(a.bias));
    a.sumsq_cap = rows_gemm_sumsq_blocks(a.M);
    a.serial_epilogue = 0;
    a.ksplit = 0;
    a.partial = nullptr;
    a.prec = 0;
    a.colstats = nullptr;
    a.colstats_rows = nullptr;
    a.alt_seg_order = options().gemm_alt_taps && is_two_tap_shift(a);
    prep[i] = a;
    first[i + 1] = first[i] + (a.M + 127) / 128;
    const double kt = (double)k_range(a).ktot;
    flops += 2.0 * a.M * a.N * kt;
    bytes += 4.0 * ((double)a.M * kt + kt * a.N + (double)a.M * a.N);
  }
  const bool same = g.args.size() == prep.size() && memcmp(g.args.data(), prep.data(), sizeof(RowsGemmArgs) * prep.size()) == 0 && g.first == first;
  if (!same) {
    if (g.capacity < (int)prep.size()) {
      if (g.d_args) hipFree(g.d_args);
      if (g.d_first) hipFree(g.d_first);
      hipError_t e = hipMalloc((void **)&g.d_args, sizeof(RowsGemmArgs) * prep.size());
      if (e != hipSuccess) return e;
      e = hipMalloc((void **)&g.d_first, sizeof(int) * (prep.size() + 1));
      if (e != hipSuccess) return e;
      g.capacity = (int)prep.size();
    }
    g.args = prep;
    g.first = first;
    hipError_t e = hipMemcpyAsync(g.d_args, g.args.data(), sizeof(RowsGemmArgs) * prep.size(), hipMemcpyHostToDevice, s);
    if (e != hipSuccess) return e;
    e = hipMemcpyAsync(g.d_first, g.first.data(), sizeof(int) * first.size(), hipMemcpyHostToDevice, s);
    if (e != hipSuccess) return e;
  }
  constexpr size_t lds = rows_lds_bytes<128, 32, 32>(true);
  ProfGemmRange prof(3, flops, bytes, s);
  RowsGemmTasks t{g.d_args, g.d_first, (int)prep.size()};
  note_launch(0, true);
  count_rows_form<4, 1, 1, 1, 32>(kFormGrouped);
  hipLaunchKernelGGL((rows_gemm_group_kernel<4, 1, 1, 1, 32, true, 4>), dim3(first.back()), dim3(256), lds, s, t);
  return hipGetLastError();
}

}
```

tdnn-f_nas_amd/csrc/rows_gemm_kernels.h:

```cpp
#pragma once
#include "common.h"
#include "gemm_dev.h"
#include "gemm_f32.h"

namespace tdnnf {
namespace {

__device__ __forceinline__ void post_store4(const RowsGemmArgs &p, int m, int n, float4 v, float4 pre, float4 addv) {
  v.x += pre.x; v.y += pre.y; v.z += pre.z; v.w += pre.w;
  if (!p.post_add) { v.x += p.add_scale * addv.x; v.y += p.add_scale * addv.y; v.z += p.add_scale * addv.z; v.w += p.add_scale * addv.w; }
  if (p.relu) { v.x = floor_keep_nan(v.x, 0.f); v.y = floor_keep_nan(v.y, 0.f); v.z = floor_keep_nan(v.z, 0.f); v.w = floor_keep_nan(v.w, 0.f); }
  const float4 sc = p.col_scale ? *reinterpret_cast<const float4 *>(p.col_scale + n) : make_float4(1.f, 1.f, 1.f, 1.f);
  const float4 of = p.col_offset ? *reinterpret_cast<const float4 *>(p.col_offset + n) : make_float4(0.f, 0.f, 0.f, 0.f);
  const float as = p.post_add ? p.add_scale : 0.f;
  v.x = sc.x * v.x + of.x + as * addv.x;
  v.y = sc.y * v.y + of.y + as * addv.y;
  v.z = sc.z * v.z + of.z + as * addv.z;
  v.w = sc.w * v.w + of.w + as * addv.w;
  const int mo = p.row_map ? p.row_map[m] : m;
  if (mo >= 0) *reinterpret_cast<float4 *>(p.C + (long long)mo * p.ldc + n) = v;
}
__device__ __forceinline__ void post_store1(const RowsGemmArgs &p, int m, int n, float x) {
  if (p.init_mode == 1) x += p.bias[n];
  const float a = (p.add && m >= p.add_lo && m < p.add_hi) ? p.add[(long long)(m - p.add_lo) * p.ldadd + n] : 0.f;
  if (!p.post_add) x += p.add_scale * a;
  if (p.relu) x = floor_keep_nan(x, 0.f);
  x = (p.col_scale ? p.col_scale[n] : 1.f) * x + (p.col_offset ? p.col_offset[n] : 0.f) + (p.post_add ? p.add_scale * a : 0.f);
  const int mo = p.row_map ? p.row_map[m] : m;
  if (mo >= 0) p.C[(long long)mo * p.ldc + n] = x;
}

template <int WM, int WN, int TM, int TN, int BK, bool B_KC, int VEC, bool POST = false>
__device__ __forceinline__ void rows_gemm_block(const RowsGemmArgs &p, int ntm, int ntn, int bx, int gx) {
  constexpr int BM = WM * TM * 32, BN = WN * TN * 32;
  constexpr int LDAS = BK + 4;
  constexpr int LDBS = B_KC ? BK + 4 : BN + 4;
  constexpr int A_TILE = BM * LDAS;
  constexpr int B_TILE = B_KC ? BN * LDBS : BK * LDBS;
  constexpr int A_F4 = (BM * BK / 4 + 255) / 256;
  constexpr int B_F4 = (BN * BK / 4 + 255) / 256;
  constexpr int KF4 = BK / 4;
  extern __shared__ __attribute__((aligned(16))) float smem[];
  float *As = smem;
  float *Bs = smem + 2 * A_TILE;

  const int nblk = ntm * ntn;
  int bid = bx;
  {
    const int q = nblk / 8, r = nblk % 8, xcd = bid % 8, j = bid / 8;
    bid = (xcd < r ? xcd * (q + 1) : r * (q + 1) + (xcd - r) * q) + j;
  }
  int sp = 0;
  if (p.ksplit > 1) {
    sp = bx % p.ksplit;
    bid = bx / p.ksplit;
  }
  const long long k_begin = (long long)sp * p.kchunk, k_end = p.ksplit > 1 ? k_begin + p.kchunk : (1LL << 60);
  const int tile_m = bid / ntn, tile_n = bid % ntn;
  const int m0 = tile_m * BM, n0 = tile_n * BN;
  const int t = threadIdx.x, lane = t & 63, wave = t >> 6;
  const int wm = wave / WN, wn = wave % WN;
  const int li = lane & 31, lh = lane >> 5;

  f32x16 acc[TM][TN];
#pragma unroll
  for (int a = 0; a < TM; a++)
#pragma unroll
    for (int b = 0; b < TN; b++)
#pragma unroll
      for (int r = 0; r < 16; r++) acc[a][b][r] = 0.f;

  const bool rev_seg = p.alt_seg_order && (tile_m & 1);
  int seg = -1, sgi = 0, kc = 0, klen = 0;
  long long seg_kstart = 0, seg_knext = 0;
  float cf = 1.f;
  auto next_seg = [&]() {
    for (++seg; seg < p.nseg; ++seg) {
      sgi = rev_seg ? p.nseg - 1 - seg : seg;
      seg_kstart = seg_knext;
      seg_knext += p.seg[sgi].klen;
      cf = p.coef ? p.coef[sgi] : 1.f;
      const long long lo = k_begin > seg_kstart ? k_begin - seg_kstart : 0;
      const long long hi = k_end < seg_knext ? k_end - seg_kstart : p.seg[sgi].klen;
      if (cf != 0.f && hi > lo) {
        kc = (int)lo;
        klen = (int)hi;
        return;
      }
    }
    kc = 0;
    klen = 0;
  };
  next_seg();

  float4 ra[A_F4], rb[B_F4];
  float cf_tile = 1.f;
  float ssq = 0.f;
  auto add_ssq = [&]() {
    float q0 = 0.f, q1 = 0.f;
#pragma unroll
    for (int j = 0; j < A_F4; j++) {
      asm volatile("v_fmac_f32 %0, %2, %2\n v_fmac_f32 %1, %3, %3\n v_fmac_f32 %0, %4, %4\n v_fmac_f32 %1, %5, %5"
                   : "+v"(q0), "+v"(q1)
                   : "v"(ra[j].x), "v"(ra[j].y), "v"(ra[j].z), "v"(ra[j].w));
    }
    ssq += cf_tile * cf_tile * (q0 + q1);
  };
  const float *aptr[A_F4], *bptr[B_F4];
  int astep[A_F4], bstep[B_F4];
  int ptr_seg = -1;
  auto setup_ptrs = [&]() {
    const GemmSeg sg = p.seg[sgi];
    const float *zero = reinterpret_cast<const float *>(&g_zero4);
#pragma unroll
    for (int j = 0; j < A_F4; j++) {
      const int idx = t + 256 * j, row = idx / KF4, m = m0 + row;
      const bool rv = (BM * BK / 4 % 256 == 0 || idx < BM * BK / 4) && m < p.M && m >= sg.m_lo && m < sg.m_hi;
      aptr[j] = rv ? p.A + sg.a_off + (long long)m * p.lda + (idx % KF4) * 4 : zero;
      astep[j] = rv ? 1 : 0;
    }
#pragma unroll
    for (int j = 0; j < B_F4; j++) {
      const int idx = t + 256 * j;
      bool rv;
      if (B_KC) {
        const int n = n0 + idx / KF4;
        rv = (BN * BK / 4 % 256 == 0 || idx < BN * BK / 4) && n < p.N;
        bptr[j] = rv ? p.B + sg.b_off + (long long)n * p.ldb + (idx % KF4) * 4 : zero;
        bstep[j] = rv ? 1 : 0;
      } else {
        const int kr = idx / (BN / 4), n = n0 + (idx % (BN / 4)) * 4;
        rv = (BN * BK / 4 % 256 == 0 || idx < BN * BK / 4) && n + 3 < p.N;
        bptr[j] = rv ? p.B + sg.b_off + (long long)kr * p.ldb + n : zero;
        bstep[j] = rv ? (int)p.ldb : 0;
      }
    }
    ptr_seg = seg;
  };
  const bool fast_ok = VEC == 4 && (B_KC || p.N % 4 == 0);
  auto load_tile = [&]() {
    if (fast_ok && kc + BK <= klen) {
      if (ptr_seg != seg) setup_ptrs();
#pragma unroll
      for (int j = 0; j < A_F4; j++) ra[j] = *reinterpret_cast<const float4 *>(aptr[j] + (long long)kc * astep[j]);
#pragma unroll
      for (int j = 0; j < B_F4; j++) rb[j] = *reinterpret_cast<const float4 *>(bptr[j] + (long long)kc * bstep[j]);
      cf_tile = cf;
      return;
    }
    const GemmSeg sg = p.seg[sgi];
    const float *Ab = p.A + sg.a_off;
    const float *Bb = p.B + sg.b_off;
#pragma unroll
    for (int j = 0; j < A_F4; j++) {
      const int idx = t + 256 * j;
      const int row = idx / KF4, k = kc + (idx % KF4) * 4;
      const int m = m0 + row;
      const bool rv = (BM * BK / 4 % 256 == 0 || idx < BM * BK / 4) && m < p.M && m >= sg.m_lo && m < sg.m_hi;
      const float *ptr = Ab + (long long)m * p.lda + k;
      ra[j] = ld4(ptr, rv && k < klen, rv && k + 1 < klen, rv && k + 2 < klen, rv && k + 3 < klen, VEC == 4);
    }
    if (B_KC) {
#pragma unroll
      for (int j = 0; j < B_F4; j++) {
        const int idx = t + 256 * j;
        const int row = idx / KF4, k = kc + (idx % KF4) * 4;
        const int n = n0 + row;
        const bool rv = (BN * BK / 4 % 256 == 0 || idx < BN * BK / 4) && n < p.N;
        const float *ptr = Bb + (long long)n * p.ldb + k;
        rb[j] = ld4(ptr, rv && k < klen, rv && k + 1 < klen, rv && k + 2 < klen, rv && k + 3 < klen, VEC == 4);
      }
    } else {
      constexpr int NF4 = BN / 4;
#pragma unroll
      for (int j = 0; j < B_F4; j++) {
        const int idx = t + 256 * j;
        const int kr = idx / NF4, n = n0 + (idx % NF4) * 4;
        const bool rv = (BN * BK / 4 % 256 == 0 || idx < BN * BK / 4) && kc + kr < klen;
        const float *ptr = Bb + (long long)(kc + kr) * p.ldb + n;
        rb[j] = ld4(ptr, rv && n < p.N, rv && n + 1 < p.N, rv && n + 2 < p.N, rv && n + 3 < p.N, VEC == 4);
      }
    }
    cf_tile = cf;
  };
  auto store_tile = [&](int buf) {
    float *as = As + buf * A_TILE, *bs = Bs + buf * B_TILE;
    if (p.sumsq) add_ssq();
    if (p.coef) {
#pragma unroll
      for (int j = 0; j < B_F4; j++) {
        rb[j].x *= cf_tile; rb[j].y *= cf_tile; rb[j].z *= cf_tile; rb[j].w *= cf_tile;
      }
    }
#pragma unroll
    for (int j = 0; j < A_F4; j++) {
      const int idx = t + 256 * j;
      if (BM * BK / 4 % 256 == 0 || idx < BM * BK / 4)
        *reinterpret_cast<float4 *>(as + (idx / KF4) * LDAS + (idx % KF4) * 4) = ra[j];
    }
#pragma unroll
    for (int j = 0; j < B_F4; j++) {
      const int idx = t + 256 * j;
      if (BN * BK / 4 % 256 == 0 || idx < BN * BK / 4) {
        if (B_KC)
          *reinterpret_cast<float4 *>(bs + (idx / KF4) * LDBS + (idx % KF4) * 4) = rb[j];
        else
          *reinterpret_cast<float4 *>(bs + (idx / (BN / 4)) * LDBS + (idx % (BN / 4)) * 4) = rb[j];
      }
    }
  };
  auto compute = [&](int buf) {
    const float *as = As + buf * A_TILE + (wm * TM * 32 + li) * LDAS + lh * 4;
    const float *bs = B_KC ? Bs + buf * B_TILE + (wn * TN * 32 + li) * LDBS + lh * 4
                           : Bs + buf * B_TILE + (lh * 4) * LDBS + wn * TN * 32 + li;
#pragma unroll
    for (int kg = 0; kg < BK / 8; kg++) {
      float4 a[TM], b[TN];
#pragma unroll
      for (int i = 0; i < TM; i++) a[i] = *reinterpret_cast<const float4 *>(as + i * 32 * LDAS + kg * 8);
#pragma unroll
      for (int i = 0; i < TN; i++) {
        if (B_KC) {
          b[i] = *reinterpret_cast<const float4 *>(bs + i * 32 * LDBS + kg * 8);
        } else {
          const float *q = bs + (kg * 8) * LDBS + i * 32;
          b[i] = make_float4(q[0], q[LDBS], q[2 * LDBS], q[3 * LDBS]);
        }
      }
#pragma unroll
      for (int i = 0; i < TM; i++)
#pragma unroll
        for (int j = 0; j < TN; j++) {
          acc[i][j] = __builtin_amdgcn_mfma_f32_32x32x2f32(a[i].x, b[j].x, acc[i][j], 0, 0, 0);
          acc[i][j] = __builtin_amdgcn_mfma_f32_32x32x2f32(a[i].y, b[j].y, acc[i][j], 0, 0, 0);
          acc[i][j] = __builtin_amdgcn_mfma_f32_32x32x2f32(a[i].z, b[j].z, acc[i][j], 0, 0, 0);
          acc[i][j] = __builtin_amdgcn_mfma_f32_32x32x2f32(a[i].w, b[j].w, acc[i][j], 0, 0, 0);
        }
    }
  };

  if (seg < p.nseg) {
    load_tile();
    store_tile(0);
    __syncthreads();
    int buf = 0;
    while (true) {
      kc += BK;
      if (kc >= klen) next_seg();
      const bool more = seg < p.nseg;
      if (more) load_tile();
      compute(buf);
      if (!more) break;
      store_tile(buf ^ 1);
      __syncthreads();
      buf ^= 1;
    }
  }

  constexpr int LDCS = BN + 4;
  constexpr int SMEM_FLOATS = 2 * (A_TILE + B_TILE);
  constexpr int HALF = (BM * LDCS <= SMEM_FLOATS) ? BM : ((BM / 2) * LDCS <= SMEM_FLOATS ? BM / 2 : BM / 4);
  static_assert(HALF * LDCS <= SMEM_FLOATS, "epilogue tile does not fit the staging LDS");
  static_assert(HALF % (TM * 32) == 0, "a wave's rows must not straddle epilogue passes");
  float *Cs = smem;
  const bool cvec = p.c_vec != 0;
  __syncthreads();
  if (p.sumsq) {
    double v = ssq;
    for (int o = 32; o > 0; o >>= 1) v += __shfl_xor(v, o, 64);
    double *red = reinterpret_cast<double *>(smem);
    if (lane == 0) red[wave] = v;
    __syncthreads();
    if (t == 0) p.sumsq[p.ksplit > 1 ? bx : bid] = (red[0] + red[1]) + (red[2] + red[3]);
    if (bx == 0)
      for (int i = gx + t; i < p.sumsq_cap; i += 256) p.sumsq[i] = 0.0;
    __syncthreads();
  }
  constexpr bool kColStats = 256 % (BN / 4) == 0 && (HALF * (BN / 4)) % 256 == 0;
  const bool colstats = kColStats && p.colstats && p.ksplit <= 1;
  float cs[4] = {0.f, 0.f, 0.f, 0.f}, cq[4] = {0.f, 0.f, 0.f, 0.f};
#pragma unroll
  for (int pass = 0; pass < BM / HALF; pass++) {
    if ((wm * TM * 32) / HALF == pass) {
#pragma unroll
      for (int i = 0; i < TM; i++)
#pragma unroll
        for (int j = 0; j < TN; j++)
#pragma unroll
          for (int r = 0; r < 16; r++) {
            const int row = (wm * TM + i) * 32 + (r & 3) + 8 * (r >> 2) + 4 * lh - pass * HALF;
            Cs[row * LDCS + (wn * TN + j) * 32 + li] = acc[i][j][r];
          }
    }
    constexpr int kSeg = HALF * (BN / 4) / 256;
    constexpr int kGrp = kSeg % 8 == 0 ? 8 : (kSeg % 5 == 0 ? 5 : (kSeg % 4 == 0 ? 4 : (kSeg % 2 == 0 ? 2 : 1)));
    constexpr bool kFastShape = (HALF * (BN / 4)) % 256 == 0;
    const bool fast_tile = kFastShape && cvec && p.ksplit <= 1 && !p.serial_epilogue && m0 + BM <= p.M && n0 + BN <= p.N;
    if (fast_tile) {
      __syncthreads();
#pragma unroll
      for (int g = 0; g < kSeg; g += kGrp) {
        float4 pre[kGrp], addv[kGrp];
        const float *zero = reinterpret_cast<const float *>(&g_zero4);
#pragma unroll
        for (int u = 0; u < kGrp; u++) {
          const int idx = t + 256 * (g + u), m = m0 + pass * HALF + idx / (BN / 4), n = n0 + (idx % (BN / 4)) * 4;
          const float *pp = p.init_mode == 0 ? p.C + (long long)m * p.ldc + n : (p.init_mode == 1 ? p.bias + n : zero);
          const float *pa = (p.add && m >= p.add_lo && m < p.add_hi) ? p.add + (long long)(m - p.add_lo) * p.ldadd + n : zero;
          pre[u] = *reinterpret_cast<const float4 *>(pp);
          addv[u] = *reinterpret_cast<const float4 *>(pa);
        }
#pragma unroll
        for (int u = 0; u < kGrp; u++) {
          const int idx = t + 256 * (g + u), row = idx / (BN / 4), c4 = (idx % (BN / 4)) * 4;
          const int m = m0 + pass * HALF + row, n = n0 + c4;
          float4 v = *reinterpret_cast<const float4 *>(Cs + row * LDCS + c4);
          if constexpr (POST) {
            post_store4(p, m, n, v, pre[u], addv[u]);
            continue;
          }
          v.x += pre[u].x + p.add_scale * addv[u].x;
          v.y += pre[u].y + p.add_scale * addv[u].y;
          v.z += pre[u].z + p.add_scale * addv[u].z;
          v.w += pre[u].w + p.add_scale * addv[u].w;
          if (p.relu) { v.x = floor_keep_nan(v.x, 0.f); v.y = floor_keep_nan(v.y, 0.f); v.z = floor_keep_nan(v.z, 0.f); v.w = floor_keep_nan(v.w, 0.f); }
          *reinterpret_cast<float4 *>(p.C + (long long)m * p.ldc + n) = v;
          if (kColStats && colstats) {
            cs[0] += v.x; cs[1] += v.y; cs[2] += v.z; cs[3] += v.w;
            cq[0] += v.x * v.x; cq[1] += v.y * v.y; cq[2] += v.z * v.z; cq[3] += v.w * v.w;
          }
        }
      }
      if (pass + 1 < BM / HALF) __syncthreads();
      continue;
    }
    __syncthreads();
    for (int idx = t; idx < HALF * (BN / 4); idx += 256) {
      const int row = idx / (BN / 4), c4 = (idx % (BN / 4)) * 4;
      const int m = m0 + pass * HALF + row, n = n0 + c4;
      if (m >= p.M || n >= p.N) continue;
      float4 v = *reinterpret_cast<const float4 *>(Cs + row * LDCS + c4);
      if (p.ksplit > 1) {
        const int ldp = (p.N + 3) & ~3;
        *reinterpret_cast<float4 *>(p.partial + ((long long)sp * p.M + m) * ldp + n) = v;
        continue;
      }
      if constexpr (POST) {
        if (cvec && n + 3 < p.N) {
          const float4 z = make_float4(0.f, 0.f, 0.f, 0.f);
          const float4 b = p.init_mode == 1 ? *reinterpret_cast<const float4 *>(p.bias + n) : z;
          const float4 o = (p.add && m >= p.add_lo && m < p.add_hi) ? *reinterpret_cast<const float4 *>(p.add + (long long)(m - p.add_lo) * p.ldadd + n) : z;
          post_store4(p, m, n, v, b, o);
        } else {
          const float vv[4] = {v.x, v.y, v.z, v.w};
#pragma unroll
          for (int e = 0; e < 4; e++)
            if (n + e < p.N) post_store1(p, m, n + e, vv[e]);
        }
        continue;
      }
      float *c = p.C + (long long)m * p.ldc + n;
      if (cvec && n + 3 < p.N) {
        if (p.init_mode == 1) {
          const float4 b = *reinterpret_cast<const float4 *>(p.bias + n);
          v.x += b.x; v.y += b.y; v.z += b.z; v.w += b.w;
        } else if (p.init_mode == 0) {
          const float4 o = *reinterpret_cast<const float4 *>(c);
          v.x += o.x; v.y += o.y; v.z += o.z; v.w += o.w;
        }
        if (p.add && m >= p.add_lo && m < p.add_hi) {
          const float4 o = *reinterpret_cast<const float4 *>(p.add + (long long)(m - p.add_lo) * p.ldadd + n);
          v.x += p.add_scale * o.x; v.y += p.add_scale * o.y; v.z += p.add_scale * o.z; v.w += p.add_scale * o.w;
        }
        if (p.relu) { v.x = floor_keep_nan(v.x, 0.f); v.y = floor_keep_nan(v.y, 0.f); v.z = floor_keep_nan(v.z, 0.f); v.w = floor_keep_nan(v.w, 0.f); }
        *reinterpret_cast<float4 *>(c) = v;
        if (colstats) {
          cs[0] += v.x; cs[1] += v.y; cs[2] += v.z; cs[3] += v.w;
          cq[0] += v.x * v.x; cq[1] += v.y * v.y; cq[2] += v.z * v.z; cq[3] += v.w * v.w;
        }
      } else {
        const float vv[4] = {v.x, v.y, v.z, v.w};
#pragma unroll
        for (int e = 0; e < 4; e++) {
          if (n + e < p.N) {
            float x = vv[e];
            if (p.init_mode == 1) x += p.bias[n + e];
            else if (p.init_mode == 0) x += c[e];
            if (p.add && m >= p.add_lo && m < p.add_hi) x += p.add_scale * p.add[(long long)(m - p.add_lo) * p.ldadd + n + e];
            if (p.relu) x = floor_keep_nan(x, 0.f);
            c[e] = x;
            if (colstats) { cs[e] += x; cq[e] += x * x; }
          }
        }
      }
    }
    if (pass + 1 < BM / HALF) __syncthreads();
  }
  if (kColStats && colstats) {
    constexpr int G = BN / 4;
    __syncthreads();
    float *red = smem;
#pragma unroll
    for (int e = 0; e < 4; e++) {
      red[((t / G) * BN + (t % G) * 4 + e) * 2] = cs[e];
      red[((t / G) * BN + (t % G) * 4 + e) * 2 + 1] = cq[e];
    }
    __syncthreads();
    if (t < BN && n0 + t < p.N) {
      float a0 = 0.f, a1 = 0.f;
#pragma unroll
      for (int g = 0; g < 256 / G; g++) {
        a0 += red[(g * BN + t) * 2];
        a1 += red[(g * BN + t) * 2 + 1];
      }
      p.colstats[(long long)tile_m * p.N + n0 + t] = a0;
      p.colstats[((long long)p.colstats_stride + tile_m) * p.N + n0 + t] = a1;
    }
  }
}

template <int WM, int WN, int TM, int TN, int BK, bool B_KC, int VEC, int TAG = 0>
__global__ __launch_bounds__(256) void rows_gemm_kernel(const RowsGemmArgs p, int ntm, int ntn) {
  rows_gemm_block<WM, WN, TM, TN, BK, B_KC, VEC>(p, ntm, ntn, (int)blockIdx.x, (int)gridDim.x);
}
template <int WM, int WN, int TM, int TN, int BK, int VEC>
__global__ __launch_bounds__(256) void rows_gemm_post_kernel(const RowsGemmArgs p, int ntm, int ntn) {
  rows_gemm_block<WM, WN, TM, TN, BK, true, VEC, true>(p, ntm, ntn, (int)blockIdx.x, (int)gridDim.x);
}
struct RowsGemmTasks {
  const RowsGemmArgs *args;
  const int *first;
  int ntasks;
};
template <int WM, int WN, int TM, int TN, int BK, bool B_KC, int VEC>
__global__ __launch_bounds__(256) void rows_gemm_group_kernel(RowsGemmTasks g) {
  int lo = 0, hi = g.ntasks;
  while (hi - lo > 1) {
    const int mid = (lo + hi) >> 1;
    if ((int)blockIdx.x >= g.first[mid]) lo = mid;
    else hi = mid;
  }
  const int b0 = g.first[lo], nb = g.first[lo + 1] - b0;
  rows_gemm_block<WM, WN, TM, TN, BK, B_KC, VEC>(g.args[lo], nb, 1, (int)blockIdx.x - b0, nb);
}

template <int WM, int WN, int TM, int TN, int BK, int NP, int D, int TAG = 0>
__global__ __launch_bounds__(256, 2) void rows_gemm_x3_kernel(const RowsGemmArgs p, int ntm, int ntn) {
  constexpr int VEC = 4;
  constexpr bool B_KC = true;
  constexpr int BM = WM * TM * 32, BN = WN * TN * 32;
  constexpr int LDH = BK + 8;
  constexpr int A_TILE = NP * BM * LDH / 2;
  constexpr int B_TILE = NP * BN * LDH / 2;
  constexpr int A_F4 = (BM * BK / 4 + 255) / 256;
  constexpr int B_F4 = (BN * BK / 4 + 255) / 256;
  constexpr int KF4 = BK / 4;
  extern __shared__ __attribute__((aligned(16))) float smem[];
  float *As = smem;
  float *Bs = smem + 2 * A_TILE;

  const int nblk = ntm * ntn;
  int bid = blockIdx.x;
  {
    const int q = nblk / 8, r = nblk % 8, xcd = bid % 8, j = bid / 8;
    bid = (xcd < r ? xcd * (q + 1) : r * (q + 1) + (xcd - r) * q) + j;
  }
  int sp = 0;
  if (p.ksplit > 1) {
    sp = blockIdx.x % p.ksplit;
    bid = blockIdx.x / p.ksplit;
  }
  const long long k_begin = (long long)sp * p.kchunk, k_end = p.ksplit > 1 ? k_begin + p.kchunk : (1LL << 60);
  const int tile_m = bid / ntn, tile_n = bid % ntn;
  const int m0 = tile_m * BM, n0 = tile_n * BN;
  const int t = threadIdx.x, lane = t & 63, wave = t >> 6;
  const int wm = wave / WN, wn = wave % WN;
  const int li = lane & 31, lh = lane >> 5;

  f32x16 acc[TM][TN];
#pragma unroll
  for (int a = 0; a < TM; a++)
#pragma unroll
    for (int b = 0; b < TN; b++)
#pragma unroll
      for (int r = 0; r < 16; r++) acc[a][b][r] = 0.f;

  int seg = -1, kc = 0, klen = 0;
  long long seg_kstart = 0, seg_knext = 0;
  float cf = 1.f;
  auto next_seg = [&]() {
    for (++seg; seg < p.nseg; ++seg) {
      seg_kstart = seg_knext;
      seg_knext += p.seg[seg].klen;
      cf = p.coef ? p.coef[seg] : 1.f;
      const long long lo = k_begin > seg_kstart ? k_begin - seg_kstart : 0;
      const long long hi = k_end < seg_knext ? k_end - seg_kstart : p.seg[seg].klen;
      if (cf != 0.f && hi > lo) {
        kc = (int)lo;
        klen = (int)hi;
        return;
      }
    }
    kc = 0;
    klen = 0;
  };
  next_seg();

  float4 ra[D][A_F4], rb[D][B_F4];
  float cf_tile[D];
  float ssq = 0.f;
  auto add_ssq = [&](const float4 (&xa)[A_F4], float c) {
    float q = 0.f;
#pragma unroll
    for (int j = 0; j < A_F4; j++) q += xa[j].x * xa[j].x + xa[j].y * xa[j].y + xa[j].z * xa[j].z + xa[j].w * xa[j].w;
    ssq += c * c * q;
  };
  const float *aptr[A_F4], *bptr[B_F4];
  int astep[A_F4], bstep[B_F4];
  int ptr_seg = -1;
  auto setup_ptrs = [&]() {
    const GemmSeg sg = p.seg[seg];
    const float *zero = reinterpret_cast<const float *>(&g_zero4);
#pragma unroll
    for (int j = 0; j < A_F4; j++) {
      const int idx = t + 256 * j, row = idx / KF4, m = m0 + row;
      const bool rv = (BM * BK / 4 % 256 == 0 || idx < BM * BK / 4) && m < p.M && m >= sg.m_lo && m < sg.m_hi;
      aptr[j] = rv ? p.A + sg.a_off + (long long)m * p.lda + (idx % KF4) * 4 : zero;
      astep[j] = rv ? 1 : 0;
    }
#pragma unroll
    for (int j = 0; j < B_F4; j++) {
      const int idx = t + 256 * j;
      bool rv;
      if (B_KC) {
        const int n = n0 + idx / KF4;
        rv = (BN * BK / 4 % 256 == 0 || idx < BN * BK / 4) && n < p.N;
        bptr[j] = rv ? p.B + sg.b_off + (long long)n * p.ldb + (idx % KF4) * 4 : zero;
        bstep[j] = rv ? 1 : 0;
      } else {
        const int kr = idx / (BN / 4), n = n0 + (idx % (BN / 4)) * 4;
        rv = (BN * BK / 4 % 256 == 0 || idx < BN * BK / 4) && n + 3 < p.N;
        bptr[j] = rv ? p.B + sg.b_off + (long long)kr * p.ldb + n : zero;
        bstep[j] = rv ? (int)p.ldb : 0;
      }
    }
    ptr_seg = seg;
  };
  const bool fast_ok = VEC == 4 && (B_KC || p.N % 4 == 0);
  auto load_tile = [&](float4 (&ra)[A_F4], float4 (&rb)[B_F4], float &cf_tile) {
    if (fast_ok && kc + BK <= klen) {
      if (ptr_seg != seg) setup_ptrs();
#pragma unroll
      for (int j = 0; j < A_F4; j++) ra[j] = *reinterpret_cast<const float4 *>(aptr[j] + (long long)kc * astep[j]);
#pragma unroll
      for (int j = 0; j < B_F4; j++) rb[j] = *reinterpret_cast<const float4 *>(bptr[j] + (long long)kc * bstep[j]);
      cf_tile = cf;
      return;
    }
    const GemmSeg sg = p.seg[seg];
    const float *Ab = p.A + sg.a_off;
    const float *Bb = p.B + sg.b_off;
#pragma unroll
    for (int j = 0; j < A_F4; j++) {
      const int idx = t + 256 * j;
      const int row = idx / KF4, k = kc + (idx % KF4) * 4;
      const int m = m0 + row;
      const bool rv = (BM * BK / 4 % 256 == 0 || idx < BM * BK / 4) && m < p.M && m >= sg.m_lo && m < sg.m_hi;
      const float *ptr = Ab + (long long)m * p.lda + k;
      ra[j] = ld4(ptr, rv && k < klen, rv && k + 1 < klen, rv && k + 2 < klen, rv && k + 3 < klen, VEC == 4);
    }
    if (B_KC) {
#pragma unroll
      for (int j = 0; j < B_F4; j++) {
        const int idx = t + 256 * j;
        const int row = idx / KF4, k = kc + (idx % KF4) * 4;
        const int n = n0 + row;
        const bool rv = (BN * BK / 4 % 256 == 0 || idx < BN * BK / 4) && n < p.N;
        const float *ptr = Bb + (long long)n * p.ldb + k;
        rb[j] = ld4(ptr, rv && k < klen, rv && k + 1 < klen, rv && k + 2 < klen, rv && k + 3 < klen, VEC == 4);
      }
// ... 222 lines not shown
```

Baseline: 1.640 million.

## Fuse output-layer NG stats GEMM into affine backprop as extra tile column

After: 1.645 million, median of 6. Within noise of the previous version (+0.3%).

```diff
diff --git a/include/tdnnf_hip.h b/include/tdnnf_hip.h
--- a/include/tdnnf_hip.h
+++ b/include/tdnnf_hip.h
@@ -178,6 +178,8 @@
 int tdnnf_ng_stats_pass(const tdnnf_tdnn_indexes *ix, const tdnnf_mat *X, int Di, const float *eff_dev, const float *WT_dev,
                         const float *W_dev, int ldw, const float *bias_dev, tdnnf_mat *H, double *sumsq_dev, int sumsq_cap, int form,
                         void *workspace_dev, size_t workspace_bytes, tdnnf_stream);
+int tdnnf_affine_backprop_ng_out(const tdnnf_mat *out_deriv, const float *W, int ldw, int Di, tdnnf_mat *in_deriv, const float *Wy_dev, int ldwy,
+                                 tdnnf_mat *H, double *sumsq_dev, int sumsq_cap, tdnnf_stream);
 const float *tdnnf_ng_scale_dev(const tdnnf_ng *);
 
 size_t tdnnf_constrain_orthonormal_workspace_bytes(int rows, int cols);
diff --git a/tdnn-f_nas_amd/csrc/abi_ng.hip b/tdnn-f_nas_amd/csrc/abi_ng.hip
--- a/tdnn-f_nas_amd/csrc/abi_ng.hip
+++ b/tdnn-f_nas_amd/csrc/abi_ng.hip
@@ -43,6 +43,26 @@
   GemmPrecisionScope exact_f32(2);
   TDNNF_HIP(rows_gemm(ng_pass_gemm_args(W, ldw, Rp, bias, in, H->data, H->stride, sumsq), true, s));
   return TDNNF_OK;
+}
+
+int tdnnf_affine_backprop_ng_out(const tdnnf_mat *out_deriv, const float *W, int ldw, int Di, tdnnf_mat *in_deriv, const float *Wy, int ldwy, tdnnf_mat *H,
+                                 double *sumsq, int sumsq_cap, tdnnf_stream stream) {
+  TDNNF_REQUIRE(mat_ok(out_deriv) && mat_ok(H) && H->data && Wy && sumsq && H->rows == out_deriv->rows && H->cols >= 1 && H->cols <= 128 && ldwy >= out_deriv->cols,
+                "affine_backprop_ng_out: bad arguments");
+  const int N = out_deriv->rows;
+  TDNNF_REQUIRE(sumsq_cap >= rows_gemm_sumsq_blocks(N), "affine_backprop_ng_out: sumsq needs %d entries", rows_gemm_sumsq_blocks(N));
+  if (N == 0) return TDNNF_OK;
+  if (options().ng_out_fused) {
+    const RowsGemmSide side{Wy, ldwy, H->data, H->stride, H->cols, sumsq};
+    return affine_backprop_impl(out_deriv, W, ldw, Di, in_deriv, &side, stream);
+  }
+  int rc = affine_backprop_impl(out_deriv, W, ldw, Di, in_deriv, nullptr, stream);
+  if (rc) return rc;
+  tdnnf_tdnn_indexes ix;
+  memset(&ix, 0, sizeof(ix));
+  ix.row_stride = 1;
+  ix.num_offsets = 1;
+  return tdnnf_ng_stats_pass(&ix, out_deriv, out_deriv->cols, nullptr, nullptr, Wy, ldwy, nullptr, H, sumsq, sumsq_cap, 0, nullptr, 0, stream);
 }
 
 int tdnnf_ng_create(int rank, int update_period, float num_samples_history, float alpha, tdnnf_ng **out) {
diff --git a/tdnn-f_nas_amd/csrc/abi_tdnn.hip b/tdnn-f_nas_amd/csrc/abi_tdnn.hip
--- a/tdnn-f_nas_amd/csrc/abi_tdnn.hip
+++ b/tdnn-f_nas_amd/csrc/abi_tdnn.hip
@@ -80,7 +80,7 @@
   Options &o = options();
   if (!name) return nullptr;
   const struct { const char *n; int *p; } table[] = {{"ng_grouped", &o.ng_grouped}, {"ng_fuse", &o.ng_fuse}, {"ng_early_in", &o.ng_early_in},
-                                                     {"wgrad_stream", &o.wgrad_stream}, {"gemm_ring", &o.gemm_ring}, {"planes", &o.planes}, {"den_split", &o.den_split}, {"phase_events", &o.phase_events}, {"wgrad_lag", &o.wgrad_lag}, {"ng_bk", &o.ng_bk}, {"ng_valu", &o.ng_valu}, {"ng_pform", &o.ng_pform}, {"planes_group", &o.planes_group}, {"xent_behind_den", &o.xent_behind_den}, {"ng_early_fork", &o.ng_early_fork}, {"ng_diag_skip", &o.ng_diag_skip}, {"wgrad_small", &o.wgrad_small}, {"splitk_per_cu", &o.splitk_per_cu}, {"gemm_alt_taps", &o.gemm_alt_taps}, {"reverse_passes", &o.reverse_passes}, {"splitk_partial_round", &o.splitk_partial_round}, {"wgrad_on_caller", &o.wgrad_on_caller}, {"den_mw_test_abort", &o.den_mw_test_abort}, {"planes_check_bound", &o.planes_check_bound}, {"den_gamma_pairs", &o.den_gamma_pairs}, {"num_form", &o.num_form}, {"num_frontier_cap", &o.num_frontier_cap}, {"gemm_arith_test", &o.gemm_arith_test}};
+                                                     {"wgrad_stream", &o.wgrad_stream}, {"gemm_ring", &o.gemm_ring}, {"planes", &o.planes}, {"den_split", &o.den_split}, {"phase_events", &o.phase_events}, {"wgrad_lag", &o.wgrad_lag}, {"ng_bk", &o.ng_bk}, {"ng_valu", &o.ng_valu}, {"ng_out_fused", &o.ng_out_fused}, {"ng_pform", &o.ng_pform}, {"planes_group", &o.planes_group}, {"xent_behind_den", &o.xent_behind_den}, {"ng_early_fork", &o.ng_early_fork}, {"ng_diag_skip", &o.ng_diag_skip}, {"wgrad_small", &o.wgrad_small}, {"splitk_per_cu", &o.splitk_per_cu}, {"gemm_alt_taps", &o.gemm_alt_taps}, {"reverse_passes", &o.reverse_passes}, {"splitk_partial_round", &o.splitk_partial_round}, {"wgrad_on_caller", &o.wgrad_on_caller}, {"den_mw_test_abort", &o.den_mw_test_abort}, {"planes_check_bound", &o.planes_check_bound}, {"den_gamma_pairs", &o.den_gamma_pairs}, {"num_form", &o.num_form}, {"num_frontier_cap", &o.num_frontier_cap}, {"gemm_arith_test", &o.gemm_arith_test}};
   for (auto &e : table)
     if (strcmp(e.n, name) == 0) return e.p;
   return nullptr;
@@ -295,9 +295,14 @@
 }
 
 int tdnnf_affine_backprop(const tdnnf_mat *out_deriv, const float *W, int ldw, int Di, tdnnf_mat *in_deriv, tdnnf_stream stream) {
-  TDNNF_REQUIRE(mat_ok(out_deriv) && mat_ok(in_deriv) && W && Di > 0 && in_deriv->cols == Di && in_deriv->rows == out_deriv->rows && ldw >= Di,
-                "affine_backprop: bad arguments");
-  if (out_deriv->rows == 0) return TDNNF_OK;
+  return affine_backprop_impl(out_deriv, W, ldw, Di, in_deriv, nullptr, stream);
+}
+
+}
+
+namespace tdnnf {
+namespace {
+RowsGemmArgs affine_backprop_args(const tdnnf_mat *out_deriv, const float *W, int ldw, int Di, const tdnnf_mat *in_deriv, bool *b_kc) {
   RowsGemmArgs a;
   memset(&a, 0, sizeof(a));
   a.A = out_deriv->data;
@@ -318,9 +323,32 @@
   a.seg[0].klen = out_deriv->cols;
   a.seg[0].m_lo = 0;
   a.seg[0].m_hi = out_deriv->rows;
-  TDNNF_HIP(rows_gemm(a, WT != nullptr, (hipStream_t)stream));
-  return TDNNF_OK;
-}
+  *b_kc = WT != nullptr;
+  return a;
+}
+bool affine_backprop_ok(const tdnnf_mat *out_deriv, const float *W, int ldw, int Di, const tdnnf_mat *in_deriv) {
+  return mat_ok(out_deriv) && mat_ok(in_deriv) && W && Di > 0 && in_deriv->cols == Di && in_deriv->rows == out_deriv->rows && ldw >= Di;
+}
+}
+
+int affine_backprop_impl(const tdnnf_mat *out_deriv, const float *W, int ldw, int Di, tdnnf_mat *in_deriv, const RowsGemmSide *side, tdnnf_stream stream) {
+  TDNNF_REQUIRE(affine_backprop_ok(out_deriv, W, ldw, Di, in_deriv), "affine_backprop: bad arguments");
+  if (out_deriv->rows == 0) return TDNNF_OK;
+  bool b_kc = false;
+  const RowsGemmArgs a = affine_backprop_args(out_deriv, W, ldw, Di, in_deriv, &b_kc);
+  if (side) TDNNF_HIP(rows_gemm_side(a, b_kc, *side, (hipStream_t)stream));
+  else TDNNF_HIP(rows_gemm(a, b_kc, (hipStream_t)stream));
+  return TDNNF_OK;
+}
+bool affine_backprop_side_fusable(const tdnnf_mat *out_deriv, const float *W, int ldw, int Di, const tdnnf_mat *in_deriv) {
+  if (!affine_backprop_ok(out_deriv, W, ldw, Di, in_deriv) || out_deriv->rows == 0) return false;
+  bool b_kc = false;
+  const RowsGemmArgs a = affine_backprop_args(out_deriv, W, ldw, Di, in_deriv, &b_kc);
+  return rows_gemm_side_fusable(a, b_kc);
+}
+}
+
+extern "C" {
 
 int tdnnf_affine_update_simple(const tdnnf_mat *in_value, const tdnnf_mat *out_deriv, float lr, float *W_acc, int ldw,
                                float *bias_acc, void *ws, size_t ws_bytes, tdnnf_stream stream) {
diff --git a/tdnn-f_nas_amd/csrc/common.h b/tdnn-f_nas_amd/csrc/common.h
--- a/tdnn-f_nas_amd/csrc/common.h
+++ b/tdnn-f_nas_amd/csrc/common.h
@@ -62,6 +62,7 @@
   int ng_early_fork = 1;
   int xent_behind_den = -1;
   int ng_pform = 1;
+  int ng_out_fused = 1;
   int ng_valu = 0;
   int ng_diag_skip = 0;
   int phase_events = 0;
@@ -128,5 +129,8 @@
 int tdnn_backprop_data_impl(const tdnnf_tdnn_indexes *ix, const tdnnf_mat *out_deriv, const float *W, int ldw, int Do, int Di,
                             const float *eff_coef, int overwrite, const tdnnf_mat *add, float add_scale, int add_lo,
                             tdnnf_mat *in_deriv, tdnnf_stream stream);
+struct RowsGemmSide;
+int affine_backprop_impl(const tdnnf_mat *out_deriv, const float *W, int ldw, int Di, tdnnf_mat *in_deriv, const RowsGemmSide *side, tdnnf_stream stream);
+bool affine_backprop_side_fusable(const tdnnf_mat *out_deriv, const float *W, int ldw, int Di, const tdnnf_mat *in_deriv);
 
 }
diff --git a/tdnn-f_nas_amd/csrc/gemm_f32.h b/tdnn-f_nas_amd/csrc/gemm_f32.h
--- a/tdnn-f_nas_amd/csrc/gemm_f32.h
+++ b/tdnn-f_nas_amd/csrc/gemm_f32.h
@@ -93,6 +93,17 @@
   return rows_gemm(a, b_kcontig, stream);
 }
 
+struct RowsGemmSide {
+  const float *B;
+  long long ldb;
+  float *C;
+  long long ldc;
+  int N;
+  double *sumsq;
+};
+bool rows_gemm_side_fusable(const RowsGemmArgs &args, bool b_kcontig);
+hipError_t rows_gemm_side(const RowsGemmArgs &args, bool b_kcontig, const RowsGemmSide &side, hipStream_t stream);
+
 struct RowsGemmGroup;
 bool rows_gemm_group_ok(const RowsGemmArgs &a);
 hipError_t rows_gemm_group(const std::vector<RowsGemmArgs> &calls, RowsGemmGroup **cache, hipStream_t stream);
diff --git a/tdnn-f_nas_amd/csrc/launch_forms.h b/tdnn-f_nas_amd/csrc/launch_forms.h
--- a/tdnn-f_nas_amd/csrc/launch_forms.h
+++ b/tdnn-f_nas_amd/csrc/launch_forms.h
@@ -15,6 +15,7 @@
   kFormSumsqSplitK,
   kFormPost,
   kFormGrouped,
+  kFormSide,
   kRowsForms
 };
 constexpr int kRowsTiles = 9, kRowsAriths = 3;
diff --git a/tdnn-f_nas_amd/csrc/launch_forms.hip b/tdnn-f_nas_amd/csrc/launch_forms.hip
--- a/tdnn-f_nas_amd/csrc/launch_forms.hip
+++ b/tdnn-f_nas_amd/csrc/launch_forms.hip
@@ -15,7 +15,7 @@
 const char *const kRowsTileNames[kRowsTiles] = {"128x32k32", "128x32k64", "128x64k32", "128x96k16", "128x96k32", "128x160k16", "64x128k16", "128x128k16", "128x128k32"};
 const char *const kArithNames[kRowsAriths] = {"f32", "bf16x3", "bf16x6"};
 const char *const kRowsFormNames[kRowsForms] = {"plain", "ring", "splitk", "partial_s2", "partial_s3", "partial_s4", "partial_s5", "partial_s6", "partial_s7", "partial_s8",
-                                                "main_split_tail", "main_plain_tail", "sumsq_plain", "sumsq_splitk", "post", "grouped"};
+                                                "main_split_tail", "main_plain_tail", "sumsq_plain", "sumsq_splitk", "post", "grouped", "side"};
 const char *const kWgradTileNames[5] = {"128x128", "160x128", "128x160", "32x128", "64x64"};
 }
 
diff --git a/tdnn-f_nas_amd/csrc/net_step.hip b/tdnn-f_nas_amd/csrc/net_step.hip
--- a/tdnn-f_nas_amd/csrc/net_step.hip
+++ b/tdnn-f_nas_amd/csrc/net_step.hip
@@ -727,6 +727,19 @@
     fused_comp = comp;
     return 1;
   }
+  int out_side_fuse(int comp, const tdnnf_mat &dv, const float *W, int ldw, const tdnnf_mat &d_in, RowsGemmSide *side) {
+    if (!use_ng || n->ng_out.empty() || !n->ng_out[comp] || n->comps[comp].lr_factor == 0.f || n->wg_on || options().ng_out_fused == 0) return 0;
+    if (!n->ng_grouped || ng_dim(n->ng_in[comp]) == 0 || ng_dim(n->ng_out[comp]) == 0) return 0;
+    if (!affine_backprop_side_fusable(&dv, W, ldw, d_in.cols, &d_in)) return 0;
+    auto &C = n->ngc[comp];
+    const float *Wy = nullptr;
+    int Rp = 0, ldwy = 0;
+    CK(ng_external_begin(n->ng_out[comp], dv.cols, &Wy, &Rp, &ldwy, s));
+    if (!Wy || Rp > 128) return 0;
+    *side = RowsGemmSide{Wy, ldwy, C.H_out, Rp, Rp, C.part_out};
+    fused_comp = comp;
+    return 1;
+  }
   double *oderiv_of(double *relu_stats, int relu_index) {
     std::vector<char> &nz = *n->oderiv_nonzero;
     if ((int)nz.size() < c.num_layers + 3) nz.resize(c.num_layers + 3, 0);
@@ -960,11 +973,18 @@
     if (h == 1) CK(capture("output-xent.deriv", dout));
     PlanesOperand po_d;
     CK(split(dout, 0, kP | kT, &po_d, s));
+    int side_fused = 0;
+    {
+      PlanesHintScope ph(hint_of(po_d), wplanes(H.c_output));
+      RowsGemmSide side;
+      if ((side_fused = out_side_fuse(H.c_output, dout, net_W(n, H.c_output), S, d_b2, &side)) < 0) return TDNNF_EINVAL;
+      if (side_fused) CK(affine_backprop_impl(&dout, net_W(n, H.c_output), S, S, &d_b2, &side, s));
+    }
     {
       PlanesHintScope ph(hint_of(po_d), hint_of(po_b2[h]));
       CK(param_grad(H.c_output, ix1, 1, S, P, &b2, &dout, nullptr, false, nullptr, 0, false));
     }
-    {
+    if (!side_fused) {
       PlanesHintScope ph(hint_of(po_d), wplanes(H.c_output));
       CK(tdnnf_affine_backprop(&dout, net_W(n, H.c_output), S, S, &d_b2, s));
     }
diff --git a/tdnn-f_nas_amd/csrc/rows_gemm.hip b/tdnn-f_nas_amd/csrc/rows_gemm.hip
--- a/tdnn-f_nas_amd/csrc/rows_gemm.hip
+++ b/tdnn-f_nas_amd/csrc/rows_gemm.hip
@@ -110,6 +110,18 @@
   else launch_rows_kernel_tagged<WM, WN, TM, TN, BK, 0>(grid, a, ntm, ntn, b_kc, vec, s);
 }
 
+template <int WM, int WN, int TM, int TN, int BK>
+void launch_rows_side_kernel(dim3 grid, const RowsGemmArgs &a, const RowsGemmArgs &sd, int ntm, int ntn, int ssq_zero_from, bool vec, hipStream_t s) {
+  constexpr int BM = WM * TM * 32, BN = WN * TN * 32;
+  constexpr size_t lds = std::max(rows_lds_bytes<BM, BN, BK>(true), rows_lds_bytes<BM, BN, BK>(false));
+  static const bool opted = opt_in_lds(rows_gemm_side_kernel<WM, WN, TM, TN, BK, false, 4>, lds) && opt_in_lds(rows_gemm_side_kernel<WM, WN, TM, TN, BK, false, 1>, lds);
+  (void)opted;
+  note_launch(0, vec);
+  count_rows_form<WM, WN, TM, TN, BK>(kFormSide);
+  if (vec) hipLaunchKernelGGL((rows_gemm_side_kernel<WM, WN, TM, TN, BK, false, 4>), grid, dim3(256), lds, s, a, sd, ntm, ntn, ssq_zero_from);
+  else hipLaunchKernelGGL((rows_gemm_side_kernel<WM, WN, TM, TN, BK, false, 1>), grid, dim3(256), lds, s, a, sd, ntm, ntn, ssq_zero_from);
+}
+
 template <int WM, int WN, int TM, int TN>
 constexpr bool kRingTile = (WM == 2 && WN == 2 && TM == 2 && TN == 2) || (WM == 4 && WN == 1 && TM == 1 && TN == 5);
 inline bool ring_applies(const RowsGemmArgs &a, bool b_kc, bool vec, int tile_cols) {
@@ -117,9 +129,16 @@
 }
 
 template <int WM, int WN, int TM, int TN, int BK>
-hipError_t launch_rows(const RowsGemmArgs &a, bool b_kc, bool vec, hipStream_t s, int form = kFormPlain) {
+hipError_t launch_rows(const RowsGemmArgs &a, bool b_kc, bool vec, hipStream_t s, int form = kFormPlain, const RowsGemmArgs *sd = nullptr, int ssq_zero_from = -1) {
   constexpr int BM = WM * TM * 32, BN = WN * TN * 32;
   const int ntm = (a.M + BM - 1) / BM, ntn = (a.N + BN - 1) / BN;
+  if constexpr (BN == 128) {
+    if (sd) {
+      launch_rows_side_kernel<WM, WN, TM, TN, BK>(dim3(ntm * (ntn + 1)), a, *sd, ntm, ntn, ssq_zero_from, vec, s);
+      count_rows_form<WM, WN, TM, TN, BK>(form);
+      return hipGetLastError();
+    }
+  }
   if constexpr (kRingTile<WM, WN, TM, TN>) {
     if (ring_applies(a, b_kc, vec, BN)) {
       note_launch(0, true);
@@ -132,16 +151,37 @@
   return hipGetLastError();
 }
 
-template <int WM, int WN, int TM, int TN, int BK>
-void launch_split_k(RowsGemmArgs at, int ntm, int ntn, int S, long long ktot, float *scratch, bool b_kc, bool vec, hipStream_t s) {
+inline size_t splitk_floats(int S, int M, int N) { return (size_t)S * M * ((N + 3) & ~3); }
+template <int BK>
+int splitk_slices(int S, long long ktot) {
+  const long long kt = (ktot + BK - 1) / BK, kchunk = ((kt + S - 1) / S) * BK;
+  return (int)((ktot + kchunk - 1) / kchunk);
+}
+template <int WM, int WN, int TM, int TN, int BK>
+void launch_split_k(RowsGemmArgs at, int ntm, int ntn, int S, long long ktot, float *scratch, bool b_kc, bool vec, hipStream_t s, const RowsGemmArgs *sd = nullptr,
+                    bool sd_clears = false) {
   const long long kt = (ktot + BK - 1) / BK;
   at.kchunk = (int)(((kt + S - 1) / S) * BK);
-  at.ksplit = (int)((ktot + at.kchunk - 1) / at.kchunk);
+  at.ksplit = splitk_slices<BK>(S, ktot);
   at.partial = scratch;
   note_rows_slices(at.ksplit);
-  launch_rows_kernel<WM, WN, TM, TN, BK>(dim3(ntm * ntn * at.ksplit), at, ntm, ntn, b_kc, vec, s);
+  RowsGemmArgs st;
+  if constexpr (WN * TN * 32 == 128) {
+    if (sd) {
+      st = *sd;
+      st.kchunk = at.kchunk;
+      st.ksplit = at.ksplit;
+      st.partial = scratch + splitk_floats(at.ksplit, at.M, at.N);
+      launch_rows_side_kernel<WM, WN, TM, TN, BK>(dim3(ntm * (ntn + 1) * at.ksplit), at, st, ntm, ntn, sd_clears ? ntm * at.ksplit : -1, vec, s);
+    }
+  }
+  if (!sd) launch_rows_kernel<WM, WN, TM, TN, BK>(dim3(ntm * ntn * at.ksplit), at, ntm, ntn, b_kc, vec, s);
   const long long total = (long long)at.M * at.N;
   hipLaunchKernelGGL(splitk_reduce_kernel, dim3((unsigned)std::min<long long>((total + 255) / 256, 2048)), dim3(256), 0, s, at);
+  if (sd) {
+    const long long stotal = (long long)st.M * st.N;
+    hipLaunchKernelGGL(splitk_reduce_kernel, dim3((unsigned)std::min<long long>((stotal + 255) / 256, 2048)), dim3(256), 0, s, st);
+  }
 }
 
 template <int WM, int WN, int TM, int TN, int BK>
@@ -173,8 +213,14 @@
   return buf;
 }
 
-template <int WM, int WN, int TM, int TN, int BK>
-hipError_t launch_rows_balanced(const RowsGemmArgs &a, bool b_kc, bool vec, int cls, double flops, hipStream_t s) {
+hipError_t side_by_itself(const RowsGemmArgs &sd, hipStream_t s) {
+  ProfClassOverride prof_as_ng(3);
+  GemmPrecisionScope exact_f32(2);
+  return rows_gemm(sd, true, s);
+}
+
+template <int WM, int WN, int TM, int TN, int BK>
+hipError_t launch_rows_balanced(const RowsGemmArgs &a, bool b_kc, bool vec, int cls, double flops, hipStream_t s, const RowsGemmArgs *sd = nullptr) {
   constexpr int BM = WM * TM * 32, BN = WN * TN * 32;
   const int ntm = (a.M + BM - 1) / BM, ntn = (a.N + BN - 1) / BN;
   int slots = rows_slots<WM, WN, TM, TN, BK>((b_kc && vec) ? a.prec : 0);
@@ -185,6 +231,7 @@
   const int q = tiles / slots, r = tiles % slots;
   const bool stats = a.colstats != nullptr;
   const auto [ktot, k4] = k_range(a);
+  const double sflops = sd ? 2.0 * a.M * sd->N * (double)ktot : 0.0;
   const int main_mt = (q * slots) / ntn;
   float *scratch = nullptr;
   size_t scratch_bytes = 0;
@@ -209,9 +256,13 @@
     if (S > kt / 4) S = (int)(kt / 4);
     const size_t need = sizeof(float) * (size_t)S * a.M * ((a.N + 3) & ~3);
     if (S >= 2 && need <= scratch_bytes) {
-      ProfScope ps(cls, flops, s);
-      launch_split_k<WM, WN, TM, TN, BK>(a, ntm, ntn, S, ktot, scratch, b_kc, vec, s);
-      count_rows_form<WM, WN, TM, TN, BK>(S_partial >= 2 ? kFormPartialS2 + S_partial - 2 : kFormSplitK);
+      const bool fuse = sd && need + sizeof(float) * splitk_floats(S, a.M, sd->N) <= scratch_bytes && (long long)ntm * S <= sd->sumsq_cap;
+      {
+        ProfScope ps(cls, flops + (fuse ? sflops : 0.0), s);
+        launch_split_k<WM, WN, TM, TN, BK>(a, ntm, ntn, S, ktot, scratch, b_kc, vec, s, fuse ? sd : nullptr, true);
+        count_rows_form<WM, WN, TM, TN, BK>(S_partial >= 2 ? kFormPartialS2 + S_partial - 2 : kFormSplitK);
+      }
+      if (sd && !fuse) return side_by_itself(*sd, s);
       return hipGetLastError();
     }
   }
@@ -230,9 +281,26 @@
       am.colstats_stride = main_mt + (tail_split ? tail_plan.chunks : (tail_rows + BM - 1) / BM);
       *a.colstats_rows = am.colstats_stride;
     }
+    const int tail_mt = (tail_rows + BM - 1) / BM;
+    const long long side_entries = main_mt + (long long)tail_mt * (tail_split ? splitk_slices<BK>(S_tail, ktot) : 1);
+    const bool fuse = sd && side_entries <= sd->sumsq_cap &&
+                      (!tail_split || sizeof(float) * (splitk_floats(S_tail, tail_rows, a.N) + splitk_floats(S_tail, tail_rows, sd->N)) <= scratch_bytes);
+    RowsGemmArgs sm, st;
+    if (fuse) {
+      sm = *sd;
+      sm.M = m_main;
+      st = *sd;
+      st.M = tail_rows;
+      st.A = sd->A + (long long)m_main * sd->lda;
+      st.C = sd->C + (long long)m_main * sd->ldc;
+      st.seg[0].m_lo -= m_main;
+      st.seg[0].m_hi -= m_main;
+      st.sumsq = sd->sumsq + main_mt;
+      st.sumsq_cap = 0;
+    }
     {
-      ProfScope ps(cls, flops * m_main / a.M, s);
-      hipError_t e = launch_rows<WM, WN, TM, TN, BK>(am, b_kc, vec, s);
+      ProfScope ps(cls, (flops + (fuse ? sflops : 0.0)) * m_main / a.M, s);
+      hipError_t e = launch_rows<WM, WN, TM, TN, BK>(am, b_kc, vec, s, kFormPlain, fuse ? &sm : nullptr, (int)side_entries);
       if (e != hipSuccess) return e;
     }
     RowsGemmArgs at = a;
@@ -251,8 +319,8 @@
     }
     if (tail_split) {
       {
-        ProfScope ps(cls, flops * at.M / a.M, s);
-        launch_split_k<WM, WN, TM, TN, BK>(at, (at.M + BM - 1) / BM, ntn, S_tail, ktot, scratch, b_kc, vec, s);
+        ProfScope ps(cls, (flops + (fuse ? sflops : 0.0)) * at.M / a.M, s);
+        launch_split_k<WM, WN, TM, TN, BK>(at, (at.M + BM - 1) / BM, ntn, S_tail, ktot, scratch, b_kc, vec, s, fuse ? &st : nullptr);
         count_rows_form<WM, WN, TM, TN, BK>(kFormMainSplitTail);
       }
       if (stats) {
@@ -260,21 +328,32 @@
         hipError_t e = colreduce_partial_into(1, ct, ct, tail_plan.chunks, tail_plan.rows_per_chunk, am.colstats_stride, at.colstats, s);
         if (e != hipSuccess) return e;
       }
+      if (sd && !fuse) return side_by_itself(*sd, s);
       return hipGetLastError();
     }
-    ProfScope ps(cls, flops * at.M / a.M, s);
-    const hipError_t e = launch_rows<WM, WN, TM, TN, BK>(at, b_kc, vec, s);
-    count_rows_form<WM, WN, TM, TN, BK>(kFormMainPlainTail);
-    return e;
-  }
-  ProfScope ps(cls, flops, s);
+    {
+      ProfScope ps(cls, (flops + (fuse ? sflops : 0.0)) * at.M / a.M, s);
+      const hipError_t e = launch_rows<WM, WN, TM, TN, BK>(at, b_kc, vec, s, kFormPlain, fuse ? &st : nullptr);
+      count_rows_form<WM, WN, TM, TN, BK>(kFormMainPlainTail);
+      if (e != hipSuccess) return e;
+    }
+    if (sd && !fuse) return side_by_itself(*sd, s);
+    return hipSuccess;
+  }
   if (stats) {
+    ProfScope ps(cls, flops, s);
     RowsGemmArgs as = a;
     as.colstats_stride = ntm;
     *a.colstats_rows = ntm;
     return launch_rows<WM, WN, TM, TN, BK>(as, b_kc, vec, s);
   }
-  return launch_rows<WM, WN, TM, TN, BK>(a, b_kc, vec, s);
+  const bool fuse = sd && ntm <= sd->sumsq_cap;
+  {
+    ProfScope ps(cls, flops + (fuse ? sflops : 0.0), s);
+    const hipError_t e = launch_rows<WM, WN, TM, TN, BK>(a, b_kc, vec, s, kFormPlain, fuse ? sd : nullptr, ntm);
+    if (e != hipSuccess || !sd || fuse) return e;
+  }
+  return side_by_itself(*sd, s);
 }
 
 template <int WM, int WN, int TM, int TN, int BK>
@@ -499,11 +578,59 @@
   return g_tw_wt + (W - g_tw_w);
 }
 
-hipError_t rows_gemm(const RowsGemmArgs &a_in, bool b_kc, hipStream_t s) {
+namespace {
+int resolved_prec(const RowsGemmArgs &a, bool b_kc, bool vec, int *planes) {
+  int prec = a.prec;
+  if (prec == 0) {
+    prec = g_gemm_prec;
+    if (prec == 0 && (options().gemm_arith_test == 1 || options().gemm_arith_test == 3)) prec = options().gemm_arith_test;
+  }
+  if (prec == 2) prec = 0;
+  *planes = (prec == 4 || (prec == 3 && options().planes)) ? (prec == 4 ? 2 : 3) : 0;
+  if (prec == 4) prec = 0;
+  if (!(b_kc && vec)) prec = 0;
+  return prec;
+}
+hipError_t rows_gemm_impl(const RowsGemmArgs &a_in, bool b_kc, const RowsGemmArgs *sd, hipStream_t s);
+}
+
+bool rows_gemm_side_fusable(const RowsGemmArgs &a, bool b_kc) {
+  if (b_kc || a.M <= 0 || a.N <= 0 || a.nseg != 1 || a.coef || a.sumsq || a.colstats || a.ksplit > 1 || rows_gemm_has_post(a)) return false;
+  if (a.seg[0].a_off != 0 || a.seg[0].m_lo > 0 || a.seg[0].m_hi < a.M || a.seg[0].klen <= 0) return false;
+  int planes = 0;
+  if (resolved_prec(a, b_kc, operands_vec4(a), &planes) != 0) return false;
+  if (planes && planes_hint_a() && planes_hint_b()) return false;
+  const int waste128 = ((a.N + 127) / 128) * 128 - a.N, waste160 = ((a.N + 159) / 160) * 160 - a.N;
+  return !(a.N <= 32 && a.M >= 1024) && waste160 >= waste128;
+}
+
+hipError_t rows_gemm_side(const RowsGemmArgs &a, bool b_kc, const RowsGemmSide &side, hipStream_t s) {
+  if (a.M <= 0 || a.N <= 0 || a.nseg != 1 || side.N <= 0 || side.N > 128 || !side.B || !side.C || !side.sumsq) return hipErrorInvalidValue;
+  RowsGemmArgs sd;
+  memset(&sd, 0, sizeof(sd));
+  sd.A = a.A; sd.lda = a.lda; sd.B = side.B; sd.ldb = side.ldb; sd.C = side.C; sd.ldc = side.ldc; sd.M = a.M; sd.N = side.N;
+  sd.init_mode = 2;
+  sd.sumsq = side.sumsq;
+  sd.nseg = 1;
+  sd.seg[0] = a.seg[0];
+  sd.seg[0].b_off = 0;
+  if (!rows_gemm_side_fusable(a, b_kc)) {
+    const hipError_t e = rows_gemm(a, b_kc, s);
+    return e != hipSuccess ? e : side_by_itself(sd, s);
+  }
+  sd.sumsq_cap = rows_gemm_sumsq_blocks(a.M);
+  sd.c_vec = aligned16(sd.C) && sd.ldc % 4 == 0;
+  return rows_gemm_impl(a, b_kc, &sd, s);
+}
+
+hipError_t rows_gemm(const RowsGemmArgs &a_in, bool b_kc, hipStream_t s) { return rows_gemm_impl(a_in, b_kc, nullptr, s); }
+
+namespace {
+hipError_t rows_gemm_impl(const RowsGemmArgs &a_in, bool b_kc, const RowsGemmArgs *sd, hipStream_t s) {
   if (a_in.M <= 0 || a_in.N <= 0 || a_in.nseg <= 0) return hipSuccess;
   RowsGemmArgs a = a_in;
   a.c_vec = aligned16(a.C) && a.ldc % 4 == 0 && (a.init_mode != 1 || aligned16(a.bias)) && (!a.add || (aligned16(a.add) && a.ldadd % 4 == 0));
-  const bool vec = operands_vec4(a);
+  const bool vec = operands_vec4(a) && (!sd || operands_vec4(*sd));
   const int waste128 = ((a.N + 127) / 128) * 128 - a.N, waste160 = ((a.N + 159) / 160) * 160 - a.N;
   const long long ktot = k_range(a).ktot;
   double flops = 0;
@@ -527,7 +654,13 @@
     }
     double c_elems = (double)a.M * a.N * (a.init_mode == 0 ? 2.0 : 1.0);
     if (a.add) c_elems += (double)(std::min(a.add_hi, a.M) - std::max(a.add_lo, 0)) * a.N;
-    prof_next_gemm(flops, 4.0 * (a_elems + b_elems + c_elems));
+    double side_flops = 0;
+    if (sd) {
+      side_flops = 2.0 * a.M * sd->N * (double)ktot;
+      b_elems += (double)ktot * sd->N;
+      c_elems += (double)a.M * sd->N;
+    }
+    prof_next_gemm(flops + side_flops, 4.0 * (a_elems + b_elems + c_elems));
   }
   a.serial_epilogue = 0;
   a.alt_seg_order = options().gemm_alt_taps && is_two_tap_shift(a);
@@ -542,17 +675,16 @@
     if (ktot <= 512) return launch_rows_post<2, 2, 2, 2, 16>(a, vec, 0, flops, s);
     return launch_rows_post<2, 2, 2, 2, 32>(a, vec, 0, flops, s);
   }
-  if (a.prec == 0) {
-    a.prec = g_gemm_prec;
-    if (a.prec == 0 && (options().gemm_arith_test == 1 || options().gemm_arith_test == 3)) a.prec = options().gemm_arith_test;
-  }
-  if (a.prec == 2) a.prec = 0;
-  if (a.prec == 4 || (a.prec == 3 && options().planes)) {
-    hipError_t pe = hipSuccess;
-    if (planes_try_rows(a, b_kc, a.prec == 4 ? 2 : 3, flops, s, &pe)) return pe;
-    if (a.prec == 4) a.prec = 0;
-  }
-  if (!(b_kc && vec)) a.prec = 0;
+  {
+    int planes = 0;
+    const int prec = resolved_prec(a, b_kc, vec, &planes);
+    if (planes && !sd) {
+      hipError_t pe = hipSuccess;
+      if (planes_try_rows(a, b_kc, planes, flops, s, &pe)) return pe;
+    }
+    a.prec = prec;
+  }
+  if (sd && (a.prec != 0 || a.sumsq || a.colstats || waste160 < waste128 || (a.N <= 32 && a.M >= 1024))) return hipErrorInvalidValue;
   if (a.colstats_rows) *a.colstats_rows = 0;
   if (!a.colstats_rows || a.prec != 0 || a.sumsq || a.N <= 32 || waste160 < waste128 || a.ksplit > 1) a.colstats = nullptr;
   if (a.sumsq) {
@@ -573,10 +705,11 @@
   {
     const long long tiles128 = (long long)((a.M + 127) / 128) * ((a.N + 127) / 128);
     const bool small = tiles128 < 768;
-    if (small && a.prec == 0 && !a.sumsq) return launch_rows_balanced<2, 2, 1, 2, 16>(a, b_kc, vec, 0, flops, s);
-    if ((ktot <= 512 && a.prec == 0) || a.prec == 3) return launch_rows_balanced<2, 2, 2, 2, 16>(a, b_kc, vec, 0, flops, s);
-  }
-  return launch_rows_balanced<2, 2, 2, 2, 32>(a, b_kc, vec, 0, flops, s);
+    if (small && a.prec == 0 && !a.sumsq) return launch_rows_balanced<2, 2, 1, 2, 16>(a, b_kc, vec, 0, flops, s, sd);
+    if ((ktot <= 512 && a.prec == 0) || a.prec == 3) return launch_rows_balanced<2, 2, 2, 2, 16>(a, b_kc, vec, 0, flops, s, sd);
+  }
+  return launch_rows_balanced<2, 2, 2, 2, 32>(a, b_kc, vec, 0, flops, s, sd);
+}
 }
 
 struct RowsGemmGroup {
diff --git a/tdnn-f_nas_amd/csrc/rows_gemm_kernels.h b/tdnn-f_nas_amd/csrc/rows_gemm_kernels.h
--- a/tdnn-f_nas_amd/csrc/rows_gemm_kernels.h
+++ b/tdnn-f_nas_amd/csrc/rows_gemm_kernels.h
@@ -31,7 +31,7 @@
 }
 
 template <int WM, int WN, int TM, int TN, int BK, bool B_KC, int VEC, bool POST = false>
-__device__ __forceinline__ void rows_gemm_block(const RowsGemmArgs &p, int ntm, int ntn, int bx, int gx) {
+__device__ __forceinline__ void rows_gemm_tile(const RowsGemmArgs &p, int tile_m, int tile_n, int sp, int ssq_at, bool ssq_zeroes, int ssq_zero_from) {
   constexpr int BM = WM * TM * 32, BN = WN * TN * 32;
   constexpr int LDAS = BK + 4;
   constexpr int LDBS = B_KC ? BK + 4 : BN + 4;
@@ -44,19 +44,7 @@
   float *As = smem;
   float *Bs = smem + 2 * A_TILE;
 
-  const int nblk = ntm * ntn;
-  int bid = bx;
-  {
-    const int q = nblk / 8, r = nblk % 8, xcd = bid % 8, j = bid / 8;
-    bid = (xcd < r ? xcd * (q + 1) : r * (q + 1) + (xcd - r) * q) + j;
-  }
-  int sp = 0;
-  if (p.ksplit > 1) {
-    sp = bx % p.ksplit;
-    bid = bx / p.ksplit;
-  }
   const long long k_begin = (long long)sp * p.kchunk, k_end = p.ksplit > 1 ? k_begin + p.kchunk : (1LL << 60);
-  const int tile_m = bid / ntn, tile_n = bid % ntn;
   const int m0 = tile_m * BM, n0 = tile_n * BN;
   const int t = threadIdx.x, lane = t & 63, wave = t >> 6;
   const int wm = wave / WN, wn = wave % WN;
@@ -271,9 +259,9 @@
     double *red = reinterpret_cast<double *>(smem);
     if (lane == 0) red[wave] = v;
     __syncthreads();
-    if (t == 0) p.sumsq[p.ksplit > 1 ? bx : bid] = (red[0] + red[1]) + (red[2] + red[3]);
-    if (bx == 0)
-      for (int i = gx + t; i < p.sumsq_cap; i += 256) p.sumsq[i] = 0.0;
+    if (t == 0) p.sumsq[ssq_at] = (red[0] + red[1]) + (red[2] + red[3]);
+    if (ssq_zeroes)
+      for (int i = ssq_zero_from + t; i < p.sumsq_cap; i += 256) p.sumsq[i] = 0.0;
     __syncthreads();
   }
   constexpr bool kColStats = 256 % (BN / 4) == 0 && (HALF * (BN / 4)) % 256 == 0;
@@ -419,6 +407,21 @@
   }
 }
 
+__device__ __forceinline__ int xcd_tile_id(int bx, int nblk) {
+  const int q = nblk / 8, r = nblk % 8, xcd = bx % 8, j = bx / 8;
+  return (xcd < r ? xcd * (q + 1) : r * (q + 1) + (xcd - r) * q) + j;
+}
+template <int WM, int WN, int TM, int TN, int BK, bool B_KC, int VEC, bool POST = false>
+__device__ __forceinline__ void rows_gemm_block(const RowsGemmArgs &p, int ntm, int ntn, int bx, int gx) {
+  int bid = xcd_tile_id(bx, ntm * ntn);
+  int sp = 0;
+  if (p.ksplit > 1) {
+    sp = bx % p.ksplit;
+    bid = bx / p.ksplit;
+  }
+  rows_gemm_tile<WM, WN, TM, TN, BK, B_KC, VEC, POST>(p, bid / ntn, bid % ntn, sp, p.ksplit > 1 ? bx : bid, bx == 0, gx);
+}
+
 template <int WM, int WN, int TM, int TN, int BK, bool B_KC, int VEC, int TAG = 0>
 __global__ __launch_bounds__(256) void rows_gemm_kernel(const RowsGemmArgs p, int ntm, int ntn) {
   rows_gemm_block<WM, WN, TM, TN, BK, B_KC, VEC>(p, ntm, ntn, (int)blockIdx.x, (int)gridDim.x);
@@ -426,6 +429,19 @@
 template <int WM, int WN, int TM, int TN, int BK, int VEC>
 __global__ __launch_bounds__(256) void rows_gemm_post_kernel(const RowsGemmArgs p, int ntm, int ntn) {
   rows_gemm_block<WM, WN, TM, TN, BK, true, VEC, true>(p, ntm, ntn, (int)blockIdx.x, (int)gridDim.x);
+}
+template <int WM, int WN, int TM, int TN, int BK, bool B_KC, int VEC>
+__global__ __launch_bounds__(256) void rows_gemm_side_kernel(const RowsGemmArgs p, const RowsGemmArgs sd, int ntm, int ntn, int ssq_zero_from) {
+  const int ntn1 = ntn + 1;
+  int bid = xcd_tile_id((int)blockIdx.x, ntm * ntn1);
+  int sp = 0;
+  if (p.ksplit > 1) {
+    sp = (int)blockIdx.x % p.ksplit;
+    bid = (int)blockIdx.x / p.ksplit;
+  }
+  const int tile_m = bid / ntn1, tile_n = bid % ntn1;
+  if (tile_n < ntn) rows_gemm_tile<WM, WN, TM, TN, BK, B_KC, VEC>(p, tile_m, tile_n, sp, 0, false, 0);
+  else rows_gemm_tile<WM, WN, TM, TN, BK, true, VEC>(sd, tile_m, 0, sp, sd.ksplit > 1 ? tile_m * sd.ksplit + sp : tile_m, ssq_zero_from >= 0 && tile_m == 0 && sp == 0, ssq_zero_from);
 }
 struct RowsGemmTasks {
   const RowsGemmArgs *args;
```
